# stevenlsw/reart

Hardware: AMD Instinct MI355X
Metric: relaxation-loop iterations/sec (higher is better)
Workload: dtype f32; 1 GPU; synthetic T=20 x N=4096, P=20, Chamfer+flow, full iteration, one instance/GPU; frames=20, points=4096, parts=20, flow=True, graph=True, steps_per_graph=20, graph_replays=1, eager_steps=0, parallelism=instances x1, instances_per_gpu=1

## Files before the change

include/reart_hip.h:

```cpp
#ifndef REART_HIP_H
#define REART_HIP_H

#include <stddef.h>
#include <stdint.h>

#ifdef __cplusplus
extern "C" {
#endif

typedef enum {
    REART_OK = 0,
    REART_ERR_INVALID_ARG = -1,
    REART_ERR_UNSUPPORTED = -2,
    REART_ERR_LAUNCH = -3,
    REART_ERR_NO_DEVICE = -4
} reart_status;

#define REART_MAX_K 16
#define REART_MAX_K_LIST 1024
#define REART_MAX_POSE_LEN 1024
#define REART_MAX_D 256

int reart_version(void);
int reart_device_count(void);
const char *reart_status_string(int status);


size_t reart_knn_points_workspace_bytes(int N, int P1, int P2, int K);
size_t reart_knn_points_workspace_bytes_d(int N, int P1, int P2, int D, int K);
int reart_knn_points_idx(const float *p1, const float *p2,
                         const int64_t *lengths1, const int64_t *lengths2,
                         int N, int P1, int P2, int D, int K,
                         float *dists, int64_t *idx,
                         void *workspace, size_t workspace_bytes, void *stream);

size_t reart_knn_points_workspace_bytes_f64(int N, int P1, int P2, int D, int K);
int reart_knn_points_idx_f64(const double *p1, const double *p2,
                             const int64_t *lengths1, const int64_t *lengths2,
                             int N, int P1, int P2, int D, int K,
                             double *dists, int64_t *idx,
                             void *workspace, size_t workspace_bytes, void *stream);

size_t reart_knn_points_backward_workspace_bytes(int N, int P1, int P2, int K);
int reart_knn_points_backward(const float *p1, const float *p2,
                              const int64_t *lengths1, const int64_t *lengths2,
                              const int64_t *idx, const float *grad_dists,
                              int N, int P1, int P2, int D, int K,
                              float *grad_p1, float *grad_p2,
                              void *workspace, size_t workspace_bytes, void *stream);

size_t reart_chamfer_bidir_workspace_bytes(int N, int P);
int reart_chamfer_bidir(const float *x, const float *y, int N, int P,
                        float *d_xy, int64_t *i_xy, float *d_yx, int64_t *i_yx,
                        void *workspace, size_t workspace_bytes, void *stream);

int reart_knn_cuda(const float *ref, const float *query, int B, int nr, int nq,
                   int D, int k, int euclidean, float *dist, int64_t *idx,
                   void *workspace, size_t workspace_bytes, void *stream);


size_t reart_blend_anchor_motion_workspace_bytes(int nq, int nr, int k);
int reart_blend_anchor_motion(const float *query, const float *ref, const float *ref_flow,
                              int nq, int nr, int k, int euclidean,
                              float *flow, uint8_t *mask,
                              void *workspace, size_t workspace_bytes, void *stream);

size_t reart_blend_anchor_motion_batch_workspace_bytes(int B, int nq, int nr_max, int k);
int reart_blend_anchor_motion_batch(const float *query, const float *ref, const float *ref_flow, const int64_t *ref_len,
                                    int B, int nq, int nr_max, int k, int euclidean, float *flow, uint8_t *mask,
                                    void *workspace, size_t workspace_bytes, void *stream);

size_t reart_kin_post_workspace_bytes(int B, int N, int nr_max, int k);
int reart_kin_post(const float *pc_trans, const float *cano, int B, int N, int cano_idx, const float *pc_src, const float *tgt,
                   const int32_t *cols, const int32_t *slot_of_point, int n, float lambda_assign, const float *ref,
                   const float *ref_flow, const int64_t *ref_len, int nr_max, int k, int euclidean, float lambda_flow, int robust,
                   float smooth_weight, float *G, float *matched, float *losses, void *workspace, size_t workspace_bytes,
                   void *stream);

size_t reart_flow_loss_workspace_bytes(void);
int reart_flow_loss(const float *gt, const float *pred, const uint8_t *mask, int B, int N,
                    int robust, float smooth_weight, float *loss, float *grad_pred,
                    void *workspace, size_t workspace_bytes, void *stream);


int reart_base_forward(const float *cano, int N, int P, int B,
                       const float *W1, const float *b1, const float *W2, int H,
                       const float *prop6d, const float *propt,
                       const float *gumbel, float tau,
                       float *out, int64_t *seg_part, float *trans_list,
                       float *yT, float *hT, int32_t *hard_idx, void *stream);

int reart_gumbel_noise(uint64_t seed, int64_t iter, int N, int P, float *out, void *stream);

size_t reart_base_backward_workspace_bytes(int N, int P, int B, int H);
int reart_base_path(int P, int B, int H, int backward);
int reart_base_backward(const float *cano, int N, int P, int B,
                        const float *W1, const float *b1, const float *W2, int H,
                        const float *prop6d, const float *propt,
                        const float *yT, const float *hT, const int32_t *hard_idx, float tau,
                        const float *G,
                        float *gW1, float *gb1, float *gW2, float *g6d, float *gt,
                        void *workspace, size_t workspace_bytes, void *stream);

int reart_compute_pc_transform(const float *cano, const float *pose, const int64_t *part,
                               int N, int P, int B, float *out, void *stream);

int reart_rotation_6d_to_matrix(const float *d6, int n, float *R, void *stream);

int reart_adam_step(float *param, const float *grad, float *exp_avg, float *exp_avg_sq,
                    int n, int step, float lr, float beta1, float beta2, float eps,
                    void *stream);

int reart_adam_step_multi(int count, float *const *param, const float *const *grad, float *const *exp_avg,
                          float *const *exp_avg_sq, const int *n, const float *lr, int step, float beta1, float beta2,
                          float eps, void *stream);


typedef struct reart_relax_config {
    int N, P, B, H;
    int cano_idx;
    int use_flow;
    int robust;
    int euclidean;
    int flow_k;
    int M_max;
    int M_total;
    int n_iter;
    int ring;
    float lambda_flow;
    float smooth_weight;
    float trans_lr, seg_lr;
    float beta1, beta2, eps;
    float start_tau, end_tau;
    float fixed_tau;
    uint64_t seed;
    int use_grid;
    int use_boxes;
    int use_assign;
    float lambda_assign;
    float weight_decay;
    int search_mode;
    int tune_slices;
    int tune_slices_flow;
    int tune_sparse;
    int tune_fwd_pts;
    int tune_bwd_pts;
    int tune_reorder;
    int tune_cloud;
    int tune_xcd;
    int profile;
    int tune_share;
    int tune_long;
} reart_relax_config;

typedef struct reart_relax_buffers {
    const float *cano;
    const float *pc_list;
    const float *ref_loc;
    const float *ref_flow;
    const int *ref_off;
    const float *gumbel;
    float *W1, *b1, *W2;
    float *p6d, *pt;
    float *adam_m, *adam_v;
    int64_t *iter;
    float *tau;
    float *losses;
    float *pc_trans;
    int64_t *seg_part;
    float *trans_list;
    void *aux_stream, *ev_fork, *ev_join;
    const int *assign_map;
} reart_relax_buffers;

size_t reart_relax_workspace_bytes(const reart_relax_config *cfg);
int reart_relax_prepare(const reart_relax_config *cfg, const reart_relax_buffers *bufs,
                        void *workspace, size_t workspace_bytes, void *stream);
int reart_relax_forward(const reart_relax_config *cfg, const reart_relax_buffers *bufs,
                        void *workspace, size_t workspace_bytes, void *stream);
int reart_relax_step(const reart_relax_config *cfg, const reart_relax_buffers *bufs,
                     void *workspace, size_t workspace_bytes, void *stream);
int reart_relax_step_batch(const reart_relax_config *cfgs, const reart_relax_buffers *bufs, void *const *workspaces,
                           size_t workspace_bytes, int K, void *stream);
#define REART_RELAX_PHASES 8
int reart_relax_step_timed(const reart_relax_config *cfg, const reart_relax_buffers *bufs,
                           void *workspace, size_t workspace_bytes, void *stream, float *h_ms);
int reart_relax_profile(const reart_relax_config *cfg, void *workspace, size_t workspace_bytes, void *stream,
                        double *h_out, int reset);


#define REART_FPS_MAX_N_LDS 12288
#define REART_FPS_MAX_N (1 << 21)
int reart_fps(const float *xyz, int B, int N, int npoint, const int32_t *start, int cuda_mode,
              int32_t *idx32, int64_t *idx64, void *stream);

int reart_fps_temp(const float *xyz, int B, int N, int npoint, const int32_t *start, int cuda_mode,
                   float *temp, int32_t *idx32, int64_t *idx64, void *stream);

int reart_ball_query(const float *xyz, const float *new_xyz, int B, int N, int S,
                     double radius, int nsample, int cuda_mode,
                     int32_t *idx32, int64_t *idx64, void *stream);

int reart_pn2_gather_points(const float *points, const int32_t *idx, int B, int C, int N, int M, float *out, void *stream);
int reart_pn2_gather_points_grad(const float *grad_out, const int32_t *idx, int B, int C, int N, int M, float *grad_points,
                                 void *stream);
int reart_pn2_three_interpolate(const float *points, const int32_t *idx, const float *weight, int B, int C, int M, int N,
                                float *out, void *stream);
int reart_pn2_three_interpolate_grad(const float *grad_out, const int32_t *idx, const float *weight, int B, int C, int N, int M,
                                     float *grad_points, void *stream);


int reart_fk_forward(const int32_t *parent, const int32_t *edge_of_part, const int32_t *order,
                     int P, const float *axis, const float *moment, const float *theta,
                     const float *distance, int B, int E, float *trans, void *stream);

size_t reart_fk_backward_workspace_bytes(int P, int B, int E);
int reart_fk_backward(const float *x, const int64_t *part, const float *G, int N,
                      const int32_t *parent, const int32_t *edge_of_part, const int32_t *order,
                      int P, const float *axis, const float *moment, const float *theta,
                      const float *distance, int B, int E, const float *trans,
                      float *g_axis, float *g_moment, float *g_theta, float *g_distance,
                      void *workspace, size_t workspace_bytes, void *stream);

#define REART_IK_MAX_POINTS 1024
int reart_ik_fit(const int32_t *parent, const int32_t *edge_of_part, const int32_t *order, int P,
                 const float *axis, const float *moment, int E, const float *src, const int64_t *part, int n,
                 const float *tgt, int M, const float *theta_init, int n_iter, float lr, float beta1, float beta2,
                 float eps, float *theta, float *loss, void *stream);


int reart_mlp_layer(const float *X, int ldx, const int64_t *gather_idx, int K, int S, int Npts,
                    const float *F, int D, const float *Q, const float *C, int xyz_first,
                    const float *Wt, const float *bias, int rows, int Cin, int Cout, int relu,
                    int pool_k, float *Y, int ldy, int ycol0, void *stream);

int reart_mlp_chain3(const int64_t *gather_idx, int K, int S, int Npts, const float *F, const float *Q, const float *C,
                     const float *W1t, const float *b1, int C1, const float *W2t, const float *b2, int C2,
                     const float *W3t, const float *b3, int C3, int rows, float *Y, int ldy, int ycol0, void *stream);

size_t reart_mlp_chain3_wide_workspace_bytes(int D, int C1, int C2, int C3);
int reart_mlp_chain3_wide(const int64_t *gather_idx, int K, int S, int Npts, const float *F, int D, const float *Q,
                          const float *C, const float *W1t, const float *b1, int C1, const float *W2t, const float *b2,
                          int C2, const float *W3t, const float *b3, int C3, int rows, float *Y, int ldy, int ycol0,
                          void *workspace, size_t workspace_bytes, void *stream);

int reart_mlp_chain_serves(int D, int K, int C1, int C2, int C3, int rows, int xyz_first);
size_t reart_mlp_chain_workspace_bytes(int D, int C1, int C2, int C3);
int reart_mlp_chain(const int64_t *gather_idx, int K, int S, int Npts, const float *F, int D, const float *Q, const float *C,
                    int xyz_first, const float *W1t, const float *b1, int C1, const float *W2t, const float *b2, int C2,
                    const float *W3t, const float *b3, int C3, int rows, float *Y, int ldy, int ycol0, void *workspace,
                    size_t workspace_bytes, void *stream);

int reart_square_distance(const float *src, const float *dst, int B, int N, int M, float *out, void *stream);

int reart_three_nn(const float *xyz1, const float *xyz2, int B, int N, int S2, float *dist3,
                   int64_t *idx3, void *stream);
size_t reart_three_interpolate_workspace_bytes(int B, int N, int S2);
int reart_three_interpolate(const float *xyz1, const float *xyz2, const float *points2, int B,
                            int N, int S2, int D, float *out, int ldo, int col0,
                            void *workspace, size_t workspace_bytes, void *stream);


size_t reart_grid_knn_workspace_bytes(int E, int Nt_max);
int reart_grid_knn(const float *targets, const int32_t *offsets, int E, int Nt_max,
                   const float *queries, int nq, int K, float *dists, int32_t *idx,
                   void *workspace, size_t workspace_bytes, void *stream);

size_t reart_knn_points_warm_workspace_bytes(int N, int P1, int P2, int K);
int reart_knn_points_idx_warm(const float *p1, const float *p2, int N, int P1, int P2, int K,
                              int32_t *seed, float *dists, int64_t *idx, void *workspace,
                              size_t workspace_bytes, void *stream);

size_t reart_chamfer_loss_workspace_bytes(int N, int P1, int P2);
int reart_chamfer_loss(const float *x, const float *y, int N, int P1, int P2, int32_t *seed_xy, int32_t *seed_yx,
                       int y_unchanged, float *d_xy, int64_t *i_xy, float *d_yx, int64_t *i_yx, float *loss,
                       float *grad_x, float *grad_y, int32_t *fx_bits, void *workspace, size_t workspace_bytes,
                       void *stream);

size_t reart_flow_term_workspace_bytes(int B, int N, int nr_max);
int reart_flow_term_prepare(const float *ref, const float *ref_flow, const int64_t *ref_len, int B, int nr_max, void *workspace,
                            size_t workspace_bytes, void *stream);
int reart_flow_term(const float *pc_trans, const float *cano, const int32_t *order, int B, int N, int cano_idx, int euclidean,
                    int robust, float smooth_weight, float weight, int32_t *seed, float *gt_flow, uint8_t *mask, float *dists,
                    int64_t *idx, float *loss, float *G, int accumulate, void *workspace, size_t workspace_bytes, void *stream);


size_t reart_lap_workspace_bytes(int B, int n);
int reart_lap_auction(const float *cost, int B, int n, int32_t *col4row, int32_t *certified,
                      const double *price_in, double *price_out, void *workspace, size_t workspace_bytes,
                      void *stream);

int reart_lap_auction_points(const float *cost, const float *src, const float *tgt, int B, int n, int32_t *col4row,
                             int32_t *certified, const double *price_in, double *price_out, void *workspace,
                             size_t workspace_bytes, void *stream);

size_t reart_lap_race_workspace_bytes(int B, int n, int racers);
int reart_lap_auction_race(const float *cost, const float *src, const float *tgt, int B, int n, int racers,
                           int32_t *col4row, int32_t *certified, double *price_out, void *workspace,
                           size_t workspace_bytes, void *stream);

int reart_lap_auction_race_warm(const float *cost, const float *src, const float *tgt, int B, int n, int racers,
                                const int32_t *col4row_in, const double *price_in, int32_t *col4row, int32_t *certified,
                                double *price_out, void *workspace, size_t workspace_bytes, void *stream);

#define REART_LAP_LARGE_MAX_N 8192
size_t reart_lap_large_workspace_bytes(int B, int n);
int reart_lap_auction_large(const float *cost, const float *src, const float *tgt, int B, int n,
                            int32_t *col4row, int32_t *certified, double *price_out,
                            void *workspace, size_t workspace_bytes, void *stream);

int reart_lap_auction_warm(const float *cost, int B, int n, int32_t *col4row, int32_t *certified,
                           const double *price_in, double *price_out, void *workspace, size_t workspace_bytes,
                           void *stream);

int reart_lap_resolve(const float *cost, int B, int n, int32_t *col4row, int32_t *certified,
                      const double *price_in, double *price_out, void *workspace, size_t workspace_bytes,
                      void *stream);

size_t reart_lap_resolve_large_workspace_bytes(int B, int n);
int reart_lap_resolve_large(const float *cost, int B, int n, int max_steps, int32_t *col4row, int32_t *certified,
                            const double *price_in, double *price_out, void *workspace, size_t workspace_bytes,
                            void *stream);

int reart_lap_step_floor(int B, int n, int steps, void *workspace, size_t workspace_bytes, double *h_us_per_step, void *stream);

int reart_relax_step_floor(const int *shape, int nk, int iters, void *workspace, size_t workspace_bytes, void *stream);

int reart_lap_resolve_points(const float *src, const float *tgt, int B, int n, int32_t *col4row,
                             int32_t *certified, const double *price_in, double *price_out, void *workspace,
                             size_t workspace_bytes, void *stream);
// ... 53 lines not shown
```

reart_amd/_lib.py:

```python
import ctypes
import os
import threading

import torch

_HERE = os.path.dirname(os.path.abspath(__file__))
LIB_PATH = os.environ.get("REART_LIB") or os.path.join(_HERE, "csrc", "libreart_hip.so")

c_int, c_float, c_size_t, c_void_p = ctypes.c_int, ctypes.c_float, ctypes.c_size_t, ctypes.c_void_p
P = c_void_p

MAX_K = 16
MAX_K_LIST = 1024
MAX_D = 256
MAX_POSE_LEN = 1024
IK_MAX_POINTS = 1024
LAP_LARGE_MAX_N = 8192
FPS_MAX_N_LDS = 12288
FPS_MAX_N = 1 << 21

PROTOTYPES = {
    "reart_version": (c_int, []),
    "reart_device_count": (c_int, []),
    "reart_status_string": (ctypes.c_char_p, [c_int]),
    "reart_knn_points_workspace_bytes": (c_size_t, [c_int] * 4),
    "reart_knn_points_workspace_bytes_d": (c_size_t, [c_int] * 5),
    "reart_knn_points_idx": (c_int, [P, P, P, P, c_int, c_int, c_int, c_int, c_int, P, P, P, c_size_t, P]),
    "reart_knn_points_workspace_bytes_f64": (c_size_t, [c_int] * 5),
    "reart_knn_points_idx_f64": (c_int, [P, P, P, P, c_int, c_int, c_int, c_int, c_int, P, P, P, c_size_t, P]),
    "reart_knn_points_backward_workspace_bytes": (c_size_t, [c_int] * 4),
    "reart_knn_points_backward": (c_int, [P, P, P, P, P, P, c_int, c_int, c_int, c_int, c_int, P, P, P, c_size_t, P]),
    "reart_chamfer_bidir_workspace_bytes": (c_size_t, [c_int] * 2),
    "reart_chamfer_bidir": (c_int, [P, P, c_int, c_int, P, P, P, P, P, c_size_t, P]),
    "reart_knn_cuda": (c_int, [P, P, c_int, c_int, c_int, c_int, c_int, c_int, P, P, P, c_size_t, P]),
    "reart_blend_anchor_motion_workspace_bytes": (c_size_t, [c_int] * 3),
    "reart_blend_anchor_motion": (c_int, [P, P, P, c_int, c_int, c_int, c_int, P, P, P, c_size_t, P]),
    "reart_kin_post_workspace_bytes": (c_size_t, [c_int] * 4),
    "reart_kin_post": (c_int, [P, P, c_int, c_int, c_int, P, P, P, P, c_int, c_float, P, P, P, c_int, c_int, c_int, c_float, c_int, c_float,
                               P, P, P, P, c_size_t, P]),
    "reart_blend_anchor_motion_batch_workspace_bytes": (c_size_t, [c_int] * 4),
    "reart_blend_anchor_motion_batch": (c_int, [P, P, P, P, c_int, c_int, c_int, c_int, c_int, P, P, P, c_size_t, P]),
    "reart_flow_loss_workspace_bytes": (c_size_t, []),
    "reart_flow_loss": (c_int, [P, P, P, c_int, c_int, c_int, c_float, P, P, P, c_size_t, P]),
    "reart_base_forward": (c_int, [P, c_int, c_int, c_int, P, P, P, c_int, P, P, P, c_float, P, P, P, P, P, P, P]),
    "reart_gumbel_noise": (c_int, [ctypes.c_uint64, ctypes.c_int64, c_int, c_int, P, P]),
    "reart_base_backward_workspace_bytes": (c_size_t, [c_int] * 4),
    "reart_base_path": (c_int, [c_int] * 4),
    "reart_base_backward": (c_int, [P, c_int, c_int, c_int, P, P, P, c_int, P, P, P, P, P, c_float, P,
                                    P, P, P, P, P, P, c_size_t, P]),
    "reart_compute_pc_transform": (c_int, [P, P, P, c_int, c_int, c_int, P, P]),
    "reart_rotation_6d_to_matrix": (c_int, [P, c_int, P, P]),
    "reart_adam_step": (c_int, [P, P, P, P, c_int, c_int, c_float, c_float, c_float, c_float, P]),
    "reart_adam_step_multi": (c_int, [c_int, P, P, P, P, P, P, c_int, c_float, c_float, c_float, P]),
    "reart_fps": (c_int, [P, c_int, c_int, c_int, P, c_int, P, P, P]),
    "reart_fps_temp": (c_int, [P, c_int, c_int, c_int, P, c_int, P, P, P, P]),
    "reart_ball_query": (c_int, [P, P, c_int, c_int, c_int, ctypes.c_double, c_int, c_int, P, P, P]),
    "reart_pn2_gather_points": (c_int, [P, P, c_int, c_int, c_int, c_int, P, P]),
    "reart_pn2_gather_points_grad": (c_int, [P, P, c_int, c_int, c_int, c_int, P, P]),
    "reart_pn2_three_interpolate": (c_int, [P, P, P, c_int, c_int, c_int, c_int, P, P]),
    "reart_pn2_three_interpolate_grad": (c_int, [P, P, P, c_int, c_int, c_int, c_int, P, P]),
    "reart_fk_forward": (c_int, [P, P, P, c_int, P, P, P, P, c_int, c_int, P, P]),
    "reart_fk_backward_workspace_bytes": (c_size_t, [c_int] * 3),
    "reart_fk_backward": (c_int, [P, P, P, c_int, P, P, P, c_int, P, P, P, P, c_int, c_int, P, P, P, P, P, P,
                                  c_size_t, P]),
    "reart_ik_fit": (c_int, [P, P, P, c_int, P, P, c_int, P, P, c_int, P, c_int, P, c_int, c_float, c_float, c_float, c_float, P, P, P]),
    "reart_mlp_layer": (c_int, [P, c_int, P, c_int, c_int, c_int, P, c_int, P, P, c_int, P, P, c_int, c_int, c_int,
                                c_int, c_int, P, c_int, c_int, P]),
    "reart_mlp_chain3": (c_int, [P, c_int, c_int, c_int, P, P, P, P, P, c_int, P, P, c_int, P, P, c_int, c_int, P, c_int, c_int, P]),
    "reart_mlp_chain3_wide_workspace_bytes": (c_size_t, [c_int] * 4),
    "reart_mlp_chain3_wide": (c_int, [P, c_int, c_int, c_int, P, c_int, P, P, P, P, c_int, P, P, c_int, P, P, c_int, c_int, P, c_int,
                                      c_int, P, c_size_t, P]),
    "reart_mlp_chain_serves": (c_int, [c_int] * 7),
    "reart_mlp_chain_workspace_bytes": (c_size_t, [c_int] * 4),
    "reart_mlp_chain": (c_int, [P, c_int, c_int, c_int, P, c_int, P, P, c_int, P, P, c_int, P, P, c_int, P, P, c_int, c_int, P, c_int,
                                c_int, P, c_size_t, P]),
    "reart_square_distance": (c_int, [P, P, c_int, c_int, c_int, P, P]),
    "reart_three_nn": (c_int, [P, P, c_int, c_int, c_int, P, P, P]),
    "reart_three_interpolate_workspace_bytes": (c_size_t, [c_int] * 3),
    "reart_three_interpolate": (c_int, [P, P, P, c_int, c_int, c_int, c_int, P, c_int, c_int, P, c_size_t, P]),
    "reart_grid_knn_workspace_bytes": (c_size_t, [c_int] * 2),
    "reart_grid_knn": (c_int, [P, P, c_int, c_int, P, c_int, c_int, P, P, P, c_size_t, P]),
    "reart_knn_points_warm_workspace_bytes": (c_size_t, [c_int] * 4),
    "reart_knn_points_idx_warm": (c_int, [P, P, c_int, c_int, c_int, c_int, P, P, P, P, c_size_t, P]),
    "reart_chamfer_loss_workspace_bytes": (c_size_t, [c_int] * 3),
    "reart_chamfer_loss": (c_int, [P, P, c_int, c_int, c_int, P, P, c_int, P, P, P, P, P, P, P, P, P, c_size_t, P]),
    "reart_flow_term_workspace_bytes": (c_size_t, [c_int] * 3),
    "reart_flow_term_prepare": (c_int, [P, P, P, c_int, c_int, P, c_size_t, P]),
    "reart_flow_term": (c_int, [P, P, P, c_int, c_int, c_int, c_int, c_int, c_float, c_float, P, P, P, P, P, P, P, c_int, P, c_size_t, P]),
    "reart_lap_workspace_bytes": (c_size_t, [c_int] * 2),
    "reart_lap_auction": (c_int, [P, c_int, c_int, P, P, P, P, P, c_size_t, P]),
    "reart_lap_auction_warm": (c_int, [P, c_int, c_int, P, P, P, P, P, c_size_t, P]),
    "reart_lap_auction_points": (c_int, [P, P, P, c_int, c_int, P, P, P, P, P, c_size_t, P]),
    "reart_lap_race_workspace_bytes": (c_size_t, [c_int] * 3),
    "reart_lap_auction_race": (c_int, [P, P, P, c_int, c_int, c_int, P, P, P, P, c_size_t, P]),
    "reart_lap_auction_race_warm": (c_int, [P, P, P, c_int, c_int, c_int, P, P, P, P, P, P, c_size_t, P]),
    "reart_lap_large_workspace_bytes": (c_size_t, [c_int] * 2),
    "reart_lap_auction_large": (c_int, [P, P, P, c_int, c_int, P, P, P, P, c_size_t, P]),
    "reart_lap_resolve": (c_int, [P, c_int, c_int, P, P, P, P, P, c_size_t, P]),
    "reart_lap_resolve_large_workspace_bytes": (c_size_t, [c_int] * 2),
    "reart_lap_resolve_large": (c_int, [P, c_int, c_int, c_int, P, P, P, P, P, c_size_t, P]),
    "reart_lap_resolve_points": (c_int, [P, P, c_int, c_int, P, P, P, P, P, c_size_t, P]),
    "reart_lap_resolve_points_race": (c_int, [P, P, c_int, c_int, c_int, P, P, P, P, P, c_size_t, P]),
    "reart_lap_resolve_points_mw": (c_int, [P, P, c_int, c_int, c_int, P, P, P, P, P, c_size_t, P]),
    "reart_lap_mc_workspace_bytes": (c_size_t, [c_int] * 3),
    "reart_lap_resolve_points_mc": (c_int, [P, P, c_int, c_int, c_int, c_int, P, P, P, P, P, c_size_t, P]),
    "reart_gather_points": (c_int, [P, P, c_int, c_int, c_int, P, P]),
    "reart_publish_words": (c_int, [P, c_int, P, c_int, P, c_int, P, P]),
    "reart_assign_pairs": (c_int, [P, P, P, c_int, c_int, c_int, P, P]),
    "reart_lap_ties": (c_int, [P, P, c_int, c_int, P, P, P, P, P, c_int, P]),
    "reart_lap_resolve_points_mc_ties": (c_int, [P, P, c_int, c_int, c_int, c_int, P, P, P, P, P, P, P, c_int, P, c_size_t, P]),
    "reart_lap_step_floor": (c_int, [c_int, c_int, c_int, P, c_size_t, ctypes.POINTER(ctypes.c_double), P]),
    "reart_relax_step_floor": (c_int, [ctypes.POINTER(c_int), c_int, c_int, P, c_size_t, P]),
    "reart_cdist": (c_int, [P, P, c_int, c_int, c_int, P, P]),
    "reart_match_smnn_workspace_bytes": (c_size_t, [c_int] * 3),
    "reart_match_smnn": (c_int, [P, P, c_int, c_int, c_int, c_int, c_float, P, P, P, c_size_t, P]),
    "reart_screw_fit_workspace_bytes": (c_size_t, [c_int] * 2),
    "reart_screw_fit": (c_int, [P, c_int, c_int, P, c_int, c_int, P, P, P, P, P, P, P, c_size_t, P]),
    "reart_part_fps": (c_int, [P, P, c_int, P, c_int, c_int, c_int, P, P, P]),
    "reart_part_pair_cost": (c_int, [P, P, c_int, c_int, c_int, P, P, P, P]),
    "reart_group_temporal_err": (c_int, [P, c_int, c_int, P, P, c_int, P, P, P]),
    "reart_relax_workspace_bytes": (c_size_t, None),
    "reart_relax_prepare": (c_int, None),
    "reart_relax_step": (c_int, None),
    "reart_relax_step_batch": (c_int, None),
    "reart_relax_forward": (c_int, None),
    "reart_relax_step_timed": (c_int, None),
    "reart_relax_profile": (c_int, None),
}

_lib = None
_lock = threading.Lock()


class ReartHipError(RuntimeError):
    """A libreart_hip.so entry point returned a negative reart_status."""


def lib():
    global _lib
    if _lib is None:
        with _lock:
            if _lib is None:
                if not os.path.exists(LIB_PATH):
                    raise ImportError(
                        f"{LIB_PATH} is missing: build it with `make -C reart_amd/csrc -j8` "
                        "(or `python -c 'import __graft_entry__ as g; g.build()'`). "
                        "reart_amd has no CPU / PyTorch fallback."
                    )
                handle = ctypes.CDLL(LIB_PATH)
                for name, (res, args) in PROTOTYPES.items():
                    fn = getattr(handle, name)
                    fn.restype = res
                    if args is not None:
                        fn.argtypes = args
                _lib = handle
    return _lib


def check(rc, what):
    if rc != 0:
        msg = lib().reart_status_string(rc).decode()
        raise ReartHipError(f"{what} failed: {msg} (status {rc})")


def require_gpu(*tensors):
    for t in tensors:
        if t is not None and not t.is_cuda:
            raise RuntimeError(
                "reart_amd operators run on an AMD GPU only (tensor is on "
                f"{t.device}); there is no CPU fallback."
            )


def ptr(t):
    return None if t is None else c_void_p(t.data_ptr())


def stream():
    return c_void_p(torch.cuda.current_stream().cuda_stream)


_ws_cache = {}


def workspace(nbytes, device):
    key = (device.index if device.index is not None else torch.cuda.current_device(),
           torch.cuda.current_stream(device).cuda_stream)
    buf = _ws_cache.get(key)
    if buf is None or buf.numel() < nbytes:
        buf = torch.empty(max(int(nbytes), 1 << 20), dtype=torch.uint8, device=device)
        _ws_cache[key] = buf
    return buf
```

reart_amd/csrc/internal.h:

```cpp
#pragma once
#include "common.h"

struct BaseFwdArgs {
    const float *cano;
    const float *W1, *b1, *W2, *p6d, *pt;
    const float *gumbel;
    const float *tau_ptr;
    const int64_t *iter_ptr;
    uint64_t seed;
    float tau;
    int N, P, B, H, Npad;
    float *out;
    float *out_soa;
    int64_t *seg_part;
    float *trans_list;
    float *yT;
    float *hT;
    int *hard_idx;
    float *rt_table;
    float *boxes;
    int pts;
};

struct BaseBwdArgs {
    const float *cano, *W2, *p6d, *pt;
    const float *yT, *hT;
    const int *hard_idx;
    const float *tau_ptr;
    float tau;
    const float *G;
    const float *rt_table;
    const float *gpf;
    int cano_idx;
    int N, P, B, H;
    int nchunk;
    int cpts;
    int dp_sep;
    float *partial;
    float *gW1, *gb1, *gW2, *g6d, *gt;
};

struct AdamSeg { float *p; const float *g; float *m; float *v; int n; float lr; };
struct AdamArgs { AdamSeg seg[8]; int nseg; float beta1, beta2, eps; const int64_t *step_ptr; int step; };

#define REART_BATCH_MAX 6
template <class A>
struct Batched { A a[REART_BATCH_MAX]; };
template <class A>
static inline Batched<A> reart_batched(const A *a, int K) {
    Batched<A> b = {};
    for (int k = 0; k < K && k < REART_BATCH_MAX; ++k) b.a[k] = a[k];
    return b;
}
int reart_base_forward_launch(const BaseFwdArgs *a, int K, hipStream_t st, int force_long);
struct FinalizeAdam {
    int enabled;
    float *W1, *b1, *W2, *p6d, *pt;
    float *m, *v;
    float seg_lr, trans_lr, beta1, beta2, eps;
    float weight_decay;
    const int64_t *step_ptr;
    const double *bias_corr;
};

struct StepBook {
    int enabled;
    const double *frame_loss; int n_frame_part;
    const double *flow_part; int n_flow_part;
    int64_t *iter; float *tau; float *losses; double *bias_corr;
    unsigned int *ticket;
    int ring, n_iter;
    float lambda_flow, fixed_tau, end_tau, start_tau, beta1, beta2;
};
int reart_base_backward_launch(const BaseBwdArgs *args, const FinalizeAdam *adam, const StepBook *book, void *const *workspaces,
                               size_t workspace_bytes, int K, hipStream_t st, int force_long);
int reart_base_forward_long_launch(const BaseFwdArgs *a, int K, hipStream_t st);
int reart_base_backward_long_launch(const BaseBwdArgs *a, int K, hipStream_t st);
int reart_base_bwd_long_tile(int P, int B, int H, int cpts, int *dp_sep, size_t *lds);
#ifdef __HIPCC__
__device__ __forceinline__ float reart_tau_schedule(long cur_iter, int n_iter, float end_t, float start_t) {
    const double c = cos(3.14159265358979323846 * (double)cur_iter / (double)n_iter);
    return (float)((double)end_t + ((double)start_t - (double)end_t) * (c + 1.0) * 0.5);
}
#endif
int reart_adam_ex(const AdamArgs &a, hipStream_t st);

int reart_knn_run(int njobs, const float *const *q, const float *const *t,
                  const int64_t *const *lenq, const int64_t *const *lent, int N, const int *P1,
                  const int *P2, int K, int euclidean, float *const *dists, int64_t *const *idx,
                  void *workspace, size_t workspace_bytes, hipStream_t st);

#define NN_BS 64
#define NN_UB 16
struct SoaJob {
    const float *src;
    const int64_t *len;
    float *dst;
    int P, Ppad;
};
struct SoaArgs {
    SoaJob job[2];
};

struct KnnJob {
    const float *q;
    const float *tsoa;
    const int64_t *lenq;
    const int64_t *lent;
    const float *q_alt;
    const int *qmap;
    const int *tlen;
    const float *boxes;
    const int *seed;
    const int *border;
    unsigned int *cost;
    int P1, P2, Ppad, L;
    int nqg;
    float *pd;
    int *pi;
    float *dists;
    int64_t *idx;
};
struct KnnArgs {
    KnnJob job[2];
    int N, S, K, euclidean;
    int items0;
    int items;
};

int reart_knn_launch_slices(const KnnArgs &a, int KK, hipStream_t st);
int reart_soa_launch(const SoaArgs &sa, int maxPpad, int N, int njobs, hipStream_t st);
int reart_knn_pick_split(long waves, int P2, int K);

size_t reart_knn_list_workspace_bytes(int N, int P1, int P2, int K);
int reart_knn_list_run(const float *q, const float *t, const int64_t *lenq, const int64_t *lent, int N, int P1,
                       int P2, int K, int euclidean, float *dists, int64_t *idx, void *workspace,
                       size_t workspace_bytes, hipStream_t st);
template <class T>
int reart_knn_anyd_run(const T *q, const T *t, const int64_t *lenq, const int64_t *lent, int N, int P1, int P2, int D,
                       int K, int euclidean, T *dists, int64_t *idx, void *workspace, size_t workspace_bytes,
                       hipStream_t st);
#ifndef NN_BOX
#define NN_BOX 16
#endif
int reart_boxes_launch(const float *soa, int N, int Ppad, float *boxes, hipStream_t st);
struct SearchArgs {
    KnnJob k1[2]; int n1;
    KnnJob k3;    int n3;
    int G;
    int per;
    int S1, S3;
    int sparse;
    int share;
    int interleave;
    int cloud_resident;
    int cloud_slices;
    int k_nqg;
    unsigned long long *prof;
    unsigned int *prof_pairs;
};
int reart_search_launch(const SearchArgs &a, hipStream_t st);
int reart_search_launch_batch(const SearchArgs *a, int K, hipStream_t st);
int reart_search_grid(int n1, int n3, int G);
int reart_search_grid_cloud(int n1, int n3, int G, int nqg, int slices);
int reart_search_workgroups(const SearchArgs &a);

#ifdef __HIPCC__
__device__ __forceinline__ void reart_top3_insert(float (&kd)[3], int (&ki)[3], float d, int j) {
    const bool l0 = (d < kd[0]) | ((d == kd[0]) & (j < ki[0]));
    const bool l1 = (d < kd[1]) | ((d == kd[1]) & (j < ki[1]));
    const bool l2 = (d < kd[2]) | ((d == kd[2]) & (j < ki[2]));
    kd[2] = l1 ? kd[1] : (l2 ? d : kd[2]);
    ki[2] = l1 ? ki[1] : (l2 ? j : ki[2]);
    kd[1] = l0 ? kd[0] : (l1 ? d : kd[1]);
    ki[1] = l0 ? ki[0] : (l1 ? j : ki[1]);
    kd[0] = l0 ? d : kd[0];
    ki[0] = l0 ? j : ki[0];
}
#endif

struct GridBuildArgs {
    const float *pts;
    const int *offsets;
    int N;
    int stride;
    float *gx, *gy, *gz;
    int *gorig;
    int *cell_start;
    float *meta;
    int *scratch;
};

struct GridQueryArgs {
    const float *q;
    const float *q_alt;
    const int *qmap;
    int nq, E, stride, euclid_unused;
    const float *gx, *gy, *gz;
    const int *gorig, *cell_start;
    const float *meta;
    float *od;
    int *oi;
};

size_t reart_grid_bytes(int E, int stride);
void reart_grid_layout(void *mem, int E, int stride, GridBuildArgs *b);
int reart_grid_build_launch(const GridBuildArgs &b, int E, hipStream_t st);
int reart_grid_query_launch(const GridQueryArgs &q, int K, hipStream_t st);
```

reart_amd/csrc/model.hip:

```cpp
#include "common.h"
#include "internal.h"
#include "model_dev.h"
#include <math.h>


#ifdef REART_PHASE_CLOCK
__device__ unsigned long long g_phase_ts[2][16];
extern "C" int reart_debug_phase_clock(unsigned long long *out) {
    return hipMemcpyFromSymbol(out, HIP_SYMBOL(g_phase_ts), sizeof(g_phase_ts)) == hipSuccess ? REART_OK : REART_ERR_LAUNCH;
}
#define PHASE_TS(which, k) do { if (blockIdx.x == 1 && threadIdx.x == 0) { g_phase_ts[which][k] = __builtin_amdgcn_s_memtime(); \
    g_phase_ts[which][(k) == 0 ? 12 : 13] = wall_clock64(); } } while (0)
#else
#define PHASE_TS(which, k) do { } while (0)
#endif
#ifdef REART_PHASE_CLOCK
#define PHASE_SYNC_TS(which, k) do { __syncthreads(); PHASE_TS(which, k); } while (0)
#else
#define PHASE_SYNC_TS(which, k) do { } while (0)
#endif


template <int PP, bool HALF, bool BATCH>
__global__ __launch_bounds__(64 * (HALF ? (((PP > 0 ? PP : 32) + 2 * FW_PG - 1) / (2 * FW_PG)) : (((PP > 0 ? PP : 32) + FW_PG - 1) / FW_PG)))
void base_fwd_kernel(Batched<BaseFwdArgs> ab) {
    const BaseFwdArgs &a = ab.a[BATCH ? blockIdx.y : 0];
    extern __shared__ __attribute__((aligned(16))) float smem[];
    constexpr int PMAX = (PP > 0) ? PP : 32;
    constexpr int W = HALF ? (PMAX + 2 * FW_PG - 1) / (2 * FW_PG) : (PMAX + FW_PG - 1) / FW_PG;
    constexpr int NS = HALF ? 2 * W : W;
    constexpr int PTS = HALF ? FW_PTS / 2 : FW_PTS;
    constexpr int BS = 64 * W;
    float *s_rt = smem;
    float *s_wb = s_rt + 12 * (size_t)a.B * a.P;
    float *s_w2T = s_wb + 4 * (size_t)a.H;
    float *s_a = s_w2T + (size_t)a.H * PMAX;
    float *s_e = s_a + PMAX * PTS;
    float *s_hh = s_e + PMAX * PTS;
    const int HS = a.H + 4;
    const int tid = threadIdx.x, lane = tid & 63, grp = tid >> 6;
    const int pl = HALF ? (lane & 31) : lane;
    const int sid = HALF ? 2 * grp + (lane >> 5) : grp;
    PHASE_TS(0, 0);
    const int P = (PP > 0) ? PP : a.P;
    const int nRT = a.B * a.P;
    auto put_rt = [&](int e, const float (&d6)[6], const float (&tv)[3]) {
        float R[9];
        r6d_to_matrix(d6, R);
#pragma unroll
        for (int c = 0; c < 9; ++c) s_rt[12 * e + c] = R[c];
#pragma unroll
        for (int c = 0; c < 3; ++c) s_rt[12 * e + 9 + c] = tv[c];
        if (blockIdx.x == 0) {
            if (a.trans_list) {
                float *T = a.trans_list + 16 * (size_t)e;
#pragma unroll
                for (int r = 0; r < 3; ++r) {
#pragma unroll
                    for (int c = 0; c < 3; ++c) T[4 * r + c] = R[3 * r + c];
                    T[4 * r + 3] = tv[r];
                }
                T[12] = 0.f; T[13] = 0.f; T[14] = 0.f; T[15] = 1.f;
            }
            if (a.rt_table) {
#pragma unroll
                for (int c = 0; c < 9; ++c) a.rt_table[12 * (size_t)e + c] = R[c];
#pragma unroll
                for (int c = 0; c < 3; ++c) a.rt_table[12 * (size_t)e + 9 + c] = tv[c];
            }
        }
    };
    {
        float d6[6], tv[3], vw[PMAX];
        const int e0 = tid < nRT ? tid : 0;
#pragma unroll
        for (int c = 0; c < 6; ++c) d6[c] = a.p6d[6 * (size_t)e0 + c];
#pragma unroll
        for (int c = 0; c < 3; ++c) tv[c] = a.pt[3 * (size_t)e0 + c];
        const int ew = tid < 4 * a.H ? tid : 0;
        const float wbv = (ew & 3) < 3 ? a.W1[3 * (ew >> 2) + (ew & 3)] : a.b1[ew >> 2];
        const int jw = tid < a.H ? tid : 0;
#pragma unroll
        for (int p = 0; p < PMAX; ++p) vw[p] = a.W2[(size_t)(p < P ? p : 0) * a.H + jw];
        if (tid < nRT) put_rt(tid, d6, tv);
        if (tid < 4 * a.H) s_wb[tid] = wbv;
        if (tid < a.H) {
#pragma unroll
            for (int p = 0; p < PMAX; ++p) s_w2T[((p >> 1) * a.H + tid) * 2 + (p & 1)] = p < P ? vw[p] : 0.f;
        }
    }
    for (int e = tid + BS; e < nRT; e += BS) {
        float d6[6], tv[3];
#pragma unroll
        for (int c = 0; c < 6; ++c) d6[c] = a.p6d[6 * (size_t)e + c];
#pragma unroll
        for (int c = 0; c < 3; ++c) tv[c] = a.pt[3 * (size_t)e + c];
        put_rt(e, d6, tv);
    }
    for (int e = tid + BS; e < 4 * a.H; e += BS) {
        const int j = e >> 2, c = e & 3;
        s_wb[e] = c < 3 ? a.W1[3 * j + c] : a.b1[j];
    }
    for (int j = tid + BS; j < a.H; j += BS)
        for (int p = 0; p < PMAX; ++p) s_w2T[((p >> 1) * a.H + j) * 2 + (p & 1)] = p < P ? a.W2[(size_t)p * a.H + j] : 0.f;

    const int n = blockIdx.x * PTS + pl;
    const bool live = n < a.N;
    const int nc = live ? n : a.N - 1;
    const float x0 = a.cano[3 * (size_t)nc], x1 = a.cano[3 * (size_t)nc + 1], x2 = a.cano[3 * (size_t)nc + 2];
    const int p0 = sid * FW_PG;
    const bool has1 = p0 + 1 < P;
    const float tau = a.tau_ptr ? a.tau_ptr[0] : a.tau;
    float g0, g1 = 0.f;
    if (a.gumbel) {
        g0 = a.gumbel[(size_t)nc * P + (p0 < P ? p0 : 0)];
        if (has1) g1 = a.gumbel[(size_t)nc * P + p0 + 1];
    } else {
        const uint64_t it = a.iter_ptr ? (uint64_t)a.iter_ptr[0] : 0ull;
        uint32_t r[4];
        philox4x32((uint32_t)n, (uint32_t)(p0 >> 2), (uint32_t)it, (uint32_t)(it >> 32), (uint32_t)a.seed,
                   (uint32_t)(a.seed >> 32), r);
        g0 = gumbel_from_bits(r[p0 & 3]);
        g1 = gumbel_from_bits(r[(p0 & 3) + 1]);
    }
    __syncthreads();
    PHASE_TS(0, 1);
    {
        const int jq = (a.H + NS - 1) / NS, j0 = sid * jq, j1 = (j0 + jq < a.H) ? j0 + jq : a.H;
        for (int j = j0; j < j1; ++j) {
            const float4 wb = *(const float4 *)(s_wb + 4 * j);
            float acc = wb.x * x0;
            acc = fmaf(wb.y, x1, acc);
            acc = fmaf(wb.z, x2, acc);
            acc = acc + wb.w;
            const float h = acc > 0.f ? acc : 0.f;
            s_hh[pl * HS + j] = h;
            if (a.hT && live) a.hT[(size_t)j * a.N + n] = h;
        }
    }
    __syncthreads();
    float sp0 = 0.f, sp1 = 0.f;
    {
        const float *hrow = s_hh + pl * HS, *wrow = s_w2T + (size_t)(sid < PMAX / 2 ? sid : PMAX / 2 - 1) * a.H * 2;
        int j = 0;
        const int H4 = (a.H & 3) == 0 ? a.H : 0;
#pragma unroll 2
        for (; j + 4 <= H4; j += 4) {
            const float4 h4 = *(const float4 *)(hrow + j);
            const float4 wa = *(const float4 *)(wrow + 2 * j), wb2 = *(const float4 *)(wrow + 2 * j + 4);
            sp0 = fmaf(wa.x, h4.x, sp0); sp1 = fmaf(wa.y, h4.x, sp1);
            sp0 = fmaf(wa.z, h4.y, sp0); sp1 = fmaf(wa.w, h4.y, sp1);
            sp0 = fmaf(wb2.x, h4.z, sp0); sp1 = fmaf(wb2.y, h4.z, sp1);
            sp0 = fmaf(wb2.z, h4.w, sp0); sp1 = fmaf(wb2.w, h4.w, sp1);
        }
        for (; j < a.H; ++j) {
            const float h = hrow[j];
            sp0 = fmaf(wrow[2 * j], h, sp0);
            sp1 = fmaf(wrow[2 * j + 1], h, sp1);
        }
    }
    PHASE_TS(0, 2);
    const float z0 = (sp0 + g0) / tau, z1 = has1 ? (sp1 + g1) / tau : -INFINITY;
    if (p0 < P) { s_a[p0 * PTS + pl] = sp0; s_e[p0 * PTS + pl] = z0; }
    if (has1) { s_a[(p0 + 1) * PTS + pl] = sp1; s_e[(p0 + 1) * PTS + pl] = z1; }
    __syncthreads();
    float m = -INFINITY;
    int am = 0;
    float sm = -INFINITY;
#pragma unroll
    for (int p = 0; p < PMAX; ++p)
        if (PP > 0 || p < P) {
            m = fmaxf(m, s_e[p * PTS + pl]);
            if (sid == 0) {
                const float sv = s_a[p * PTS + pl];
                if (sv > sm) { sm = sv; am = p; }
            }
        }
    __syncthreads();
    const float e0 = expf(z0 - m), e1 = has1 ? expf(z1 - m) : 0.f;
    if (p0 < P) s_e[p0 * PTS + pl] = e0;
    if (has1) s_e[(p0 + 1) * PTS + pl] = e1;
    __syncthreads();
    float sum = 0.f;
#pragma unroll
    for (int p = 0; p < PMAX; ++p)
        if (PP > 0 || p < P) sum += s_e[p * PTS + pl];
    const float y0 = e0 / sum, y1 = e1 / sum;
    if (p0 < P) { s_a[p0 * PTS + pl] = y0; if (a.yT && live) a.yT[(size_t)p0 * a.N + n] = y0; }
    if (has1) { s_a[(p0 + 1) * PTS + pl] = y1; if (a.yT && live) a.yT[(size_t)(p0 + 1) * a.N + n] = y1; }
    __syncthreads();
    PHASE_TS(0, 3);
    int k = 0;
    float yk = -1.f;
#pragma unroll
    for (int p = 0; p < PMAX; ++p)
        if (PP > 0 || p < P) {
            const float yv = s_a[p * PTS + pl];
            if (yv > yk) { yk = yv; k = p; }
        }
    const float w = (1.0f - yk) + yk;
    if (live && sid == 0) {
        if (a.seg_part) a.seg_part[n] = am;
        if (a.hard_idx) a.hard_idx[n] = k;
    }
    PHASE_TS(0, 4);
    for (int t = sid; t < a.B; t += NS) {
        float v[3];
        apply_rt(s_rt + 12 * (t * a.P + k), x0, x1, x2, v);
        v[0] = w * v[0]; v[1] = w * v[1]; v[2] = w * v[2];
        if (live) {
            float *o = a.out + 3 * ((size_t)t * a.N + n);
            o[0] = v[0]; o[1] = v[1]; o[2] = v[2];
        }
        if (a.out_soa && n < a.Npad) {
            float *o = a.out_soa + (size_t)t * 3 * a.Npad;
            o[n] = live ? v[0] : INFINITY;
            o[a.Npad + n] = live ? v[1] : INFINITY;
            o[2 * (size_t)a.Npad + n] = live ? v[2] : INFINITY;
        }
        if (a.boxes && blockIdx.x * PTS < a.Npad) {
            float lo[3], hi[3];
#pragma unroll
            for (int c = 0; c < 3; ++c) {
                static_assert(NN_BOX == 16, "a box is one DPP row");
                lo[c] = reart_row16_min(live ? v[c] : INFINITY);
                hi[c] = reart_row16_max(live ? v[c] : -INFINITY);
                if (hi[c] == -INFINITY) hi[c] = INFINITY;
            }
            const int pos = blockIdx.x * PTS + pl;
            if ((pl & (NN_BOX - 1)) == 0 && pos < a.Npad) {
                float *o = a.boxes + ((size_t)t * (a.Npad / NN_BOX) + pos / NN_BOX) * 8;
                o[0] = lo[0]; o[1] = lo[1]; o[2] = lo[2]; o[3] = hi[0]; o[4] = hi[1]; o[5] = hi[2];
            }
        }
    }
    PHASE_TS(0, 5);
}

template <int PP, bool HALF>
static void launch_base_fwd_t(const BaseFwdArgs *ak, int K, hipStream_t st) {
    const BaseFwdArgs &a = ak[0];
    constexpr int PMAX = (PP > 0) ? PP : 32;
    constexpr int W = HALF ? (PMAX + 2 * FW_PG - 1) / (2 * FW_PG) : (PMAX + FW_PG - 1) / FW_PG;
    constexpr int PTS = HALF ? FW_PTS / 2 : FW_PTS;
    const int cover = a.out_soa ? (a.Npad > a.N ? a.Npad : a.N) : a.N;
    const size_t lds = sizeof(float) * (12 * (size_t)a.B * a.P + (size_t)a.H * (4 + PMAX) + 2 * (size_t)PTS * PMAX +
                                        (size_t)(a.H + 4) * PTS);
    if (lds > REART_LDS_DEFAULT_CAP) {
        (void)hipFuncSetAttribute((const void *)base_fwd_kernel<PP, HALF, false>, hipFuncAttributeMaxDynamicSharedMemorySize, 152 * 1024);
        (void)hipFuncSetAttribute((const void *)base_fwd_kernel<PP, HALF, true>, hipFuncAttributeMaxDynamicSharedMemorySize, 152 * 1024);
    }
    if (K == 1) hipLaunchKernelGGL((base_fwd_kernel<PP, HALF, false>), dim3(reart_div_up(cover, PTS)), dim3(64 * W), lds, st, reart_batched(ak, 1));
    else hipLaunchKernelGGL((base_fwd_kernel<PP, HALF, true>), dim3(reart_div_up(cover, PTS), K), dim3(64 * W), lds, st, reart_batched(ak, K));
}
template <int PP>
static void launch_base_fwd(const BaseFwdArgs *a, int K, hipStream_t st) {
    if (a[0].pts == 64) launch_base_fwd_t<PP, false>(a, K, st);
    else launch_base_fwd_t<PP, true>(a, K, st);
}

static size_t base_fwd_lds_bound(int P, int B, int H) {
    return ((size_t)B * P * 12 + 2 * FW_PTS * 32 + (size_t)H * (36 + FW_PTS) + 4 * FW_PTS) * sizeof(float);
}
static size_t base_bwd_lds(int P, int B, int H) {
    const int PMAX = (P == 20 || P == 10 || P == 8) ? P : 32;
    return sizeof(float) * ((size_t)(H + PMAX) * BW_LD + RED_CHUNK * 5 + PMAX + 4 +
                            (size_t)B * RED_CHUNK * 3 + (size_t)H * PMAX + 12 * (size_t)B * P +
                            (size_t)PMAX * BW_LD);
}

extern "C" int reart_base_path(int P, int B, int H, int backward) {
    if (P < 1 || B < 1 || H < 1) return REART_ERR_INVALID_ARG;
    if (P > 32) return REART_ERR_UNSUPPORTED;
    if ((backward ? base_bwd_lds(P, B, H) : base_fwd_lds_bound(P, B, H)) <= REART_MODEL_LDS_CAP) return 0;
    if (B > REART_MAX_POSE_LEN) return REART_ERR_UNSUPPORTED;
    if (backward) return reart_base_bwd_long_tile(P, B, H, 0, nullptr, nullptr) >= 1 ? 1 : REART_ERR_UNSUPPORTED;
    return base_fwd_lds_bound(P, 0, H) <= REART_MODEL_LDS_CAP ? 1 : REART_ERR_UNSUPPORTED;
}

int reart_base_forward_launch(const BaseFwdArgs *ak, int K, hipStream_t st, int force_long) {
    if (K < 1 || K > REART_BATCH_MAX) return REART_ERR_INVALID_ARG;
    const BaseFwdArgs &a = ak[0];
    for (int k = 1; k < K; ++k)
        if (ak[k].N != a.N || ak[k].P != a.P || ak[k].B != a.B || ak[k].H != a.H || ak[k].Npad != a.Npad || ak[k].pts != a.pts ||
            !ak[k].out_soa != !a.out_soa)
            return REART_ERR_INVALID_ARG;
    if (a.P < 1 || a.P > 32) return REART_ERR_UNSUPPORTED;
    const int path = reart_base_path(a.P, a.B, a.H, 0);
    if (path < 0) return path;
    if (path == 1 || force_long) return reart_base_forward_long_launch(ak, K, st);
    switch (a.P) {
        case 20: launch_base_fwd<20>(ak, K, st); break;
        case 10: launch_base_fwd<10>(ak, K, st); break;
        case 8: launch_base_fwd<8>(ak, K, st); break;
        default: launch_base_fwd<0>(ak, K, st); break;
    }
    REART_CHECK_LAUNCH();
    return REART_OK;
}

extern "C" int reart_base_forward(const float *cano, int N, int P, int B, const float *W1,
                                  const float *b1, const float *W2, int H, const float *prop6d,
                                  const float *propt, const float *gumbel, float tau, float *out,
                                  int64_t *seg_part, float *trans_list, float *yT, float *hT,
                                  int32_t *hard_idx, void *stream) {
    if (N < 0 || P < 1 || B < 0 || H < 1) return REART_ERR_INVALID_ARG;
    if (N == 0 || B == 0) return REART_OK;
    if (!cano || !W1 || !b1 || !W2 || !prop6d || !propt || !gumbel || !out) return REART_ERR_INVALID_ARG;
    if (!(tau > 0.f)) return REART_ERR_INVALID_ARG;
    BaseFwdArgs a = {};
    a.cano = cano; a.W1 = W1; a.b1 = b1; a.W2 = W2; a.p6d = prop6d; a.pt = propt;
    a.gumbel = gumbel; a.tau = tau; a.N = N; a.P = P; a.B = B; a.H = H; a.Npad = 0;
    a.out = out; a.seg_part = seg_part; a.trans_list = trans_list; a.yT = yT; a.hT = hT;
    a.hard_idx = hard_idx;
    return reart_base_forward_launch(&a, 1, (hipStream_t)stream, 0);
}

__global__ __launch_bounds__(256) void gumbel_noise_kernel(uint64_t seed, uint64_t it, int N, int P, float *__restrict__ out) {
    const int Q = (P + 3) >> 2;
    const size_t e = (size_t)blockIdx.x * 256 + threadIdx.x;
    if (e >= (size_t)N * Q) return;
    const int n = (int)(e / Q), q = (int)(e % Q);
    uint32_t r[4];
    philox4x32((uint32_t)n, (uint32_t)q, (uint32_t)it, (uint32_t)(it >> 32), (uint32_t)seed, (uint32_t)(seed >> 32), r);
#pragma unroll
    for (int w = 0; w < 4; ++w)
        if (4 * q + w < P) out[(size_t)n * P + 4 * q + w] = gumbel_from_bits(r[w]);
}

extern "C" int reart_gumbel_noise(uint64_t seed, int64_t iter, int N, int P, float *out, void *stream) {
    if (N < 0 || P < 1 || iter < 0) return REART_ERR_INVALID_ARG;
    if (N == 0) return REART_OK;
    if (!out) return REART_ERR_INVALID_ARG;
    const size_t total = (size_t)N * ((P + 3) >> 2);
    gumbel_noise_kernel<<<(unsigned)((total + 255) / 256), 256, 0, (hipStream_t)stream>>>(seed, (uint64_t)iter, N, P, out);
    REART_CHECK_LAUNCH();
    return REART_OK;
}


__global__ __launch_bounds__(256) void rt_table_kernel(const float *__restrict__ p6d,
                                                       const float *__restrict__ pt, int n,
                                                       float *__restrict__ table) {
    const int e = blockIdx.x * 256 + threadIdx.x;
    if (e >= n) return;
    float R[9];
    r6d_to_matrix(p6d + 6 * (size_t)e, R);
#pragma unroll
    for (int c = 0; c < 9; ++c) table[12 * (size_t)e + c] = R[c];
#pragma unroll
    for (int c = 0; c < 3; ++c) table[12 * (size_t)e + 9 + c] = pt[3 * (size_t)e + c];
}

#ifdef REART_PHASE_CLOCK
#define PHASE_TS_WAVE(which, k, wave) do { if (blockIdx.x == 1 && (int)threadIdx.x == 64 * (wave)) g_phase_ts[which][k] = __builtin_amdgcn_s_memtime(); } while (0)
#else
#define PHASE_TS_WAVE(which, k, wave) do { } while (0)
#endif

template <int V> struct BwPiece { float v[V]; };
template <int V> __device__ __forceinline__ BwPiece<V> bw_load(const float *p) {
    BwPiece<V> r;
    if constexpr (V == 4) {
        const float4 q = *(const float4 *)p;
        r.v[0] = q.x; r.v[1] = q.y; r.v[2] = q.z; r.v[3] = q.w;
    } else {
        r.v[0] = *p;
    }
    return r;
}
template <int PP, int V, bool FAST, class LoadPoint>
__device__ __forceinline__ void bwd_stage_tiles(const BaseBwdArgs &a, int n0, int cn, float *s_h, float *s_G, float *s_w2T,
                                                float *s_rt, float *s_y, LoadPoint load_point) {
    typedef BwPiece<V> Pc;
    constexpr int PMAX = (PP > 0) ? PP : 32, BS = 64 * BW_WAVES;
    const int P = (PP > 0) ? PP : a.P;
    const int H = FAST ? 128 : a.H, B = FAST ? 19 : a.B, cw = FAST ? 32 : a.cpts;
    const int rsh = (cw == 64 ? 6 : (cw == 32 ? 5 : 4)) - (V == 4 ? 2 : 0);
    const int rp = 1 << rsh, gpc = 3 * rp;
    const int nH = H << rsh, nY = P << rsh, nG = B * gpc, nR = B * P * 12 / V, nW = P * (H / V);
    constexpr int UH = FAST ? 1 : 128 * RED_CHUNK / V / BS, UG = FAST ? 1 : (19 * RED_CHUNK * 3 / V + BS - 1) / BS,
                  UY = FAST ? 1 : (PMAX * RED_CHUNK / V + BS - 1) / BS, UR = (19 * 20 * 12 / V + BS - 1) / BS,
                  UW = FAST ? 1 : (PMAX * 128 / V + BS - 1) / BS;
    const int tid = threadIdx.x, tw = (tid + BS - 384) & (BS - 1), ty = BS - 1 - tid;
    const bool flow = a.gpf != nullptr;
    auto load_g = [&](int e, Pc &g, Pc &gh, Pc &gl) {
// ... 176 lines not shown
                    }
                }
#pragma unroll
                for (int u = 0; u < TU; ++u) {
                    const bool tok = t0 + u < a.B;
#pragma unroll
                    for (int r = 0; r < 3; ++r)
                        c = __builtin_amdgcn_mfma_f32_16x16x4f32(tok ? av[u][r] * xt : 0.f, (pok && tok) ? bv[u][r] : 0.f, c, 0, 0, 0);
                }
            }
#pragma unroll
            for (int reg = 0; reg < 4; ++reg)
                if (pok) s_ds[pc * BW_LD + 16 * mt + 4 * kq + reg] = c[reg];
        }
    }
    __syncthreads();
    PHASE_TS(1, 2);
    const int bl = lane < cn16 ? lane : 0;
    if (grp == 0) {
        const float yk = s_y[(kn < 0 ? 0 : kn) * BW_LD + bl];
        s_w[lane] = (1.0f - yk) + yk;
    }
    float ds0 = 0.f, ds1 = 0.f;
    if (has0) {
        const float dw0 = s_ds[p0 * BW_LD + bl];
        const float dw1 = has1 ? s_ds[(p0 + 1) * BW_LD + bl] : 0.f;
        const float tau = a.tau_ptr ? a.tau_ptr[0] : a.tau;
        float dot = 0.f;
#pragma unroll
        for (int p = 0; p < PMAX; ++p)
            if (PP > 0 || p < P) dot = fmaf(s_y[p * BW_LD + bl], s_ds[p * BW_LD + bl], dot);
        ds0 = (s_y[p0 * BW_LD + bl] * (dw0 - dot)) / tau;
        if (has1) ds1 = (s_y[(p0 + 1) * BW_LD + bl] * (dw1 - dot)) / tau;
    }
    __syncthreads();
    if (has0) s_ds[p0 * BW_LD + lane] = live ? ds0 : 0.f;
    if (has1) s_ds[(p0 + 1) * BW_LD + lane] = live ? ds1 : 0.f;
    __syncthreads();
    PHASE_TS(1, 3);
    const int n2 = (a.B * 12 + 31) >> 5, n1 = (a.H + 31) >> 5;
    if (grp < BW_MFMA) {
        typedef float f16v __attribute__((ext_vector_type(16)));
        for (int g = grp; g < n2 + n1; g += BW_MFMA) {
            f16v c = {0.f, 0.f, 0.f, 0.f, 0.f, 0.f, 0.f, 0.f, 0.f, 0.f, 0.f, 0.f, 0.f, 0.f, 0.f, 0.f};
            const int pr = lane & 31, kh = lane >> 5;
            if (g >= n2) {
                const int jc = (g - n2) * 32 + (lane & 31);
                const float *ap = s_ds + (pr < P ? pr : 0) * BW_LD + kh;
                const float *bp = s_h + (jc < a.H ? jc : 0) * BW_LD + kh;
                const bool aok = pr < P, bok = jc < a.H;
                for (int kb = 0; kb < cn16; kb += 16) {
#pragma unroll
                    for (int kk = kb; kk < kb + 16; kk += 2) {
                        const float av = aok ? ap[kk] : 0.f;
                        const float bv = bok ? bp[kk] : 0.f;
                        c = __builtin_amdgcn_mfma_f32_32x32x2f32(av, bv, c, 0, 0, 0);
                    }
                }
#pragma unroll
                for (int reg = 0; reg < 16; ++reg) {
                    const int prow_p = (reg & 3) + 8 * (reg >> 2) + 4 * kh;
                    if (prow_p < P && bok) prow[off_gW2() + prow_p * a.H + jc] = c[reg];
                }
                PHASE_TS_WAVE(1, 5, n2 % BW_MFMA);
            } else {
                const int col = g * 32 + (lane & 31);
                const bool cok = col < a.B * 12;
                const int t = cok ? col / 12 : 0, e = cok ? col - t * 12 : 0;
                const int gr = e < 9 ? e / 3 : e - 9, xc = e < 9 ? e - 3 * (e / 3) : 0;
                const float *gcol = s_G + t * (RED_CHUNK * 3) + gr;
                for (int kb = 0; kb < cn16; kb += 16) {
#pragma unroll
                    for (int kk = kb; kk < kb + 16; kk += 2) {
                        const int n = kk + kh;
                        const float av = (s_kn[n] == pr) ? 1.f : 0.f;
                        float bv = s_w[n] * gcol[3 * n];
                        if (e < 9) bv = bv * s_x[3 * n + xc];
                        c = __builtin_amdgcn_mfma_f32_32x32x2f32(av, cok ? bv : 0.f, c, 0, 0, 0);
                    }
                }
#pragma unroll
                for (int reg = 0; reg < 16; ++reg) {
                    const int prow_p = (reg & 3) + 8 * (reg >> 2) + 4 * kh;
                    if (prow_p < P && cok) prow[off_gRt(a.P, a.H) + (t * a.P + prow_p) * 12 + e] = c[reg];
                }
                PHASE_TS_WAVE(1, 4, 0);
            }
        }
    }
    if (!a.dp_sep) __syncthreads();
    if (grp >= BW_MFMA) {
        typedef float f16v __attribute__((ext_vector_type(16)));
        for (int jt = grp - BW_MFMA; jt < n1; jt += BW_HID) {
            const int j0 = 32 * jt, j1 = (j0 + 32 < a.H) ? j0 + 32 : a.H;
            const int jc = j0 + (lane & 31), kh = lane >> 5;
            const bool jok = jc < a.H;
            const float *bp = s_w2T + (jok ? jc : 0) * PMAX + kh;
            for (int nb = 0; nb < cn16; nb += 32) {
                f16v c = {0.f, 0.f, 0.f, 0.f, 0.f, 0.f, 0.f, 0.f, 0.f, 0.f, 0.f, 0.f, 0.f, 0.f, 0.f, 0.f};
                const float *ap = s_ds + kh * BW_LD + nb + (lane & 31);
#pragma unroll
                for (int p = 0; p < PMAX; p += 2) {
                    const bool pok = PP > 0 || p + kh < P;
                    const float av = pok ? ap[p * BW_LD] : 0.f;
                    const float bv = (pok && jok) ? bp[p] : 0.f;
                    c = __builtin_amdgcn_mfma_f32_32x32x2f32(av, bv, c, 0, 0, 0);
                }
#pragma unroll
                for (int reg = 0; reg < 16; ++reg) {
                    const int nn = nb + (reg & 3) + 8 * (reg >> 2) + 4 * kh;
                    if (jok && nn < a.cpts) {
                        const float h = s_h[jc * BW_LD + nn];
                        s_dp[jc * dp_ld + nn] = (nn < cn && h > 0.f) ? c[reg] : 0.f;
                    }
                }
            }
            __builtin_amdgcn_fence(__ATOMIC_ACQ_REL, "wavefront");
            __builtin_amdgcn_wave_barrier();
            PHASE_TS_WAVE(1, 6, BW_MFMA);
            {
                const int ob = 4 * j0 + lane;
                const bool ok0 = ob < 4 * j1, ok1 = ob + 64 < 4 * j1;
                const int ja = ok0 ? ob >> 2 : j0, jb = ok1 ? (ob + 64) >> 2 : ja, c = ob & 3, xo = c < 3 ? c : 0;
                float acc0 = 0.f, acc1 = 0.f;
                for (int ib = 0; ib < cn16; ib += 16) {
#pragma unroll
                    for (int i = ib; i < ib + 16; ++i) {
                        const float xs = s_x[3 * i + xo], xv = c < 3 ? xs : 1.0f;
                        acc0 = fmaf(s_dp[ja * dp_ld + i], xv, acc0);
                        acc1 = fmaf(s_dp[jb * dp_ld + i], xv, acc1);
                    }
                }
                if (c < 3) {
                    if (ok0) prow[off_gW1(a.P, a.H) + 3 * ja + c] = acc0;
                    if (ok1) prow[off_gW1(a.P, a.H) + 3 * jb + c] = acc1;
                } else {
                    if (ok0) prow[off_gb1(a.P, a.H) + ja] = acc0;
                    if (ok1) prow[off_gb1(a.P, a.H) + jb] = acc1;
                }
            }
            PHASE_TS_WAVE(1, 7, BW_MFMA);
        }
    }
    PHASE_SYNC_TS(1, 8);
}


struct AdamLoaded { float p, m, v; };
__device__ __forceinline__ AdamLoaded adam_load(const float *p, const float *m, const float *v) {
    AdamLoaded r;
    r.p = *p; r.m = *m; r.v = *v;
    return r;
}
__device__ __forceinline__ void adam_update(float *p, float g, float *m, float *v, const AdamLoaded &ld, float lr,
                                            float step_size_base, float bc2s, float beta1, float beta2,
                                            float eps, float weight_decay = 0.f) {
    (void)lr;
    if (weight_decay != 0.f) g = g + weight_decay * ld.p;
    float mm = ld.m, vv = ld.v;
    mm = mm + (g - mm) * (1.0f - beta1);
    vv = vv * beta2 + ((1.0f - beta2) * g) * g;
    const float denom = sqrtf(vv) / bc2s + eps;
    *m = mm; *v = vv;
    *p = ld.p - step_size_base * (mm / denom);
}

__device__ __forceinline__ void base_bwd_finalize_body(const BaseBwdArgs &a, const FinalizeAdam &ad) {
    const int og = blockIdx.x * 256 + threadIdx.x;
    const int nWr = a.P * a.H + 4 * a.H;
    const int nW = (4 * nWr + 63) & ~63;
    const int RQ = (a.nchunk + 3) >> 2;
    const int o = og >> 2;
    const int no = n_out(a.P, a.H, a.B);
    double bc1 = 1.0, bc2 = 1.0;
    if (ad.enabled) { bc1 = ad.bias_corr[0]; bc2 = ad.bias_corr[1]; }
    if (og < nW) {
        if (o >= nWr) return;
        const int nW2 = a.P * a.H, nW1 = 3 * a.H;
        const int kind = o < nW2 ? 0 : (o < nW2 + nW1 ? 1 : 2);
        const int q = kind == 0 ? o : (kind == 1 ? o - nW2 : o - nW2 - nW1);
        const int mo = kind == 0 ? nW1 + a.H + q : (kind == 1 ? q : nW1 + q);
        AdamLoaded ld = {0.f, 0.f, 0.f};
        if (ad.enabled) {
            if (kind == 0) ld.p = ad.W2[q];
            else if (kind == 1) ld.p = ad.W1[q];
            else ld.p = ad.b1[q];
            ld.m = ad.m[mo]; ld.v = ad.v[mo];
        }
        float acc = 0.f;
        int c = (og & 3) * RQ;
        const int cend = c + RQ < a.nchunk ? c + RQ : a.nchunk;
        for (; c + 32 <= cend; c += 32) {
            float v[32];
#pragma unroll
            for (int u = 0; u < 32; ++u) v[u] = a.partial[(size_t)(c + u) * no + o];
#pragma unroll
            for (int u = 0; u < 32; ++u) acc += v[u];
        }
        for (; c + 8 <= cend; c += 8) {
            float v[8];
#pragma unroll
            for (int u = 0; u < 8; ++u) v[u] = a.partial[(size_t)(c + u) * no + o];
#pragma unroll
            for (int u = 0; u < 8; ++u) acc += v[u];
        }
        for (; c < cend; ++c) acc += a.partial[(size_t)c * no + o];
        acc = acc + __shfl_xor(acc, 1, 64);
        acc = acc + __shfl_xor(acc, 2, 64);
        if (og & 3) return;
        const float ss_seg = (float)((double)ad.seg_lr / bc1), bc2s = (float)bc2;
        if (kind == 0) {
            a.gW2[q] = acc;
            if (ad.enabled) adam_update(ad.W2 + q, acc, ad.m + mo, ad.v + mo, ld, ad.seg_lr, ss_seg, bc2s, ad.beta1, ad.beta2, ad.eps, ad.weight_decay);
        } else if (kind == 1) {
            a.gW1[q] = acc;
            if (ad.enabled) adam_update(ad.W1 + q, acc, ad.m + mo, ad.v + mo, ld, ad.seg_lr, ss_seg, bc2s, ad.beta1, ad.beta2, ad.eps, ad.weight_decay);
        } else {
            a.gb1[q] = acc;
            if (ad.enabled) adam_update(ad.b1 + q, acc, ad.m + mo, ad.v + mo, ld, ad.seg_lr, ss_seg, bc2s, ad.beta1, ad.beta2, ad.eps, ad.weight_decay);
        }
    } else if (og < nW + 64 * a.B * a.P) {
        const int q = og - nW, e = q >> 6, tq = (q >> 4) & 3, c = q & 15;
        const int base6 = 3 * a.H + a.H + a.P * a.H, baset = base6 + 6 * a.B * a.P;
        const int k = c < 6 ? c : (c < 9 ? c - 6 : 2);
        const int mo = c < 6 ? base6 + 6 * e + k : baset + 3 * e + k;
        float *const pp = c < 6 ? ad.p6d + 6 * (size_t)e + k : ad.pt + 3 * (size_t)e + k;
        float d6[6];
#pragma unroll
        for (int u = 0; u < 6; ++u) d6[u] = a.p6d[6 * (size_t)e + u];
        AdamLoaded ld = {0.f, 0.f, 0.f};
        if (ad.enabled) ld = adam_load(pp, ad.m + mo, ad.v + mo);
        float acc = 0.f;
        if (c < 12) {
            const float *pr = a.partial + off_gRt(a.P, a.H) + 12 * (size_t)e + c;
            int ch = tq * RQ;
            const int chend = ch + RQ < a.nchunk ? ch + RQ : a.nchunk;
            for (; ch + 32 <= chend; ch += 32) {
                float v[32];
#pragma unroll
                for (int u = 0; u < 32; ++u) v[u] = pr[(size_t)(ch + u) * no];
#pragma unroll
                for (int u = 0; u < 32; ++u) acc += v[u];
            }
            for (; ch < chend; ++ch) acc += pr[(size_t)ch * no];
        }
        acc = acc + __shfl_xor(acc, 16, 64);
        acc = acc + __shfl_xor(acc, 32, 64);
        float gRt[12];
        const int lane0 = (threadIdx.x & 63) & ~15;
#pragma unroll
        for (int u = 0; u < 12; ++u) gRt[u] = __shfl(acc, lane0 + u, 64);
        if (c >= 9 || tq != 0) return;
        float g6[6];
        r6d_backward(d6, gRt, g6);
        const float ss_tr = (float)((double)ad.trans_lr / bc1), bc2s = (float)bc2;
        float g;
        if (c < 6) {
            g = g6[0];
#pragma unroll
            for (int u = 1; u < 6; ++u) g = (c == u) ? g6[u] : g;
            a.g6d[6 * (size_t)e + c] = g;
        } else {
            g = k == 0 ? gRt[9] : (k == 1 ? gRt[10] : gRt[11]);
            a.gt[3 * (size_t)e + k] = g;
        }
        if (ad.enabled) adam_update(pp, g, ad.m + mo, ad.v + mo, ld, ad.trans_lr, ss_tr, bc2s, ad.beta1, ad.beta2, ad.eps, ad.weight_decay);
    }
}

template <bool BATCH>
__global__ __launch_bounds__(384) void base_bwd_finalize_kernel(Batched<BaseBwdArgs> ab, Batched<FinalizeAdam> adb, Batched<StepBook> bkb) {
    const BaseBwdArgs &a = ab.a[BATCH ? blockIdx.y : 0];
    const FinalizeAdam &ad = adb.a[BATCH ? blockIdx.y : 0];
    const StepBook &bk = bkb.a[BATCH ? blockIdx.y : 0];
    __shared__ int s_last;
    __shared__ double s_book[4];
    __shared__ float s_tau;
    __shared__ long s_it;
    const int tid = threadIdx.x;
#ifdef REART_PHASE_CLOCK
    if (blockIdx.x == 1 && blockIdx.y == 0 && threadIdx.x == 0) { g_phase_ts[0][14] = __builtin_amdgcn_s_memtime(); g_phase_ts[0][8] = g_phase_ts[0][14]; }
#endif
    if (tid >= 320) {
        if (!bk.enabled) return;
        if (tid == 320) {
            const long it = (long)bk.iter[0];
            s_it = it;
            s_book[2] = 1.0 - pow((double)bk.beta1, (double)(it + 2));
            s_book[3] = sqrt(1.0 - pow((double)bk.beta2, (double)(it + 2)));
            s_tau = bk.fixed_tau > 0.f ? bk.fixed_tau : reart_tau_schedule(it + 2, bk.n_iter, bk.end_tau, bk.start_tau);
        }
    } else if (tid >= 256) {
        if (!bk.enabled) return;
        const int l = tid - 256;
        double recon = 0.0, flow = 0.0;
        for (int b = l; b < bk.n_frame_part; b += 64) recon += bk.frame_loss[b];
        for (int i = l; i < bk.n_flow_part; i += 64) flow += bk.flow_part[i];
        recon = reart_wave_sum_d(recon);
        flow = reart_wave_sum_d(flow);
        if (l == 0) { s_book[0] = recon; s_book[1] = flow * (double)bk.lambda_flow; }
    } else base_bwd_finalize_body(a, ad);
#ifdef REART_PHASE_CLOCK
    if (blockIdx.x == 1 && blockIdx.y == 0 && threadIdx.x == 0) g_phase_ts[0][9] = __builtin_amdgcn_s_memtime();
#endif
    if (!bk.enabled) return;
    __syncthreads();
    if (tid == 0) s_last = (atomicAdd(bk.ticket, 1u) == gridDim.x - 1) ? 1 : 0;
    __syncthreads();
#ifdef REART_PHASE_CLOCK
    if (blockIdx.x == 1 && blockIdx.y == 0 && threadIdx.x == 0) g_phase_ts[0][10] = __builtin_amdgcn_s_memtime();
#endif
    if (!s_last || tid != 0) return;
    const long it = s_it;
    if (bk.losses && bk.ring > 0) {
        float *row = bk.losses + 4 * (size_t)(it % bk.ring);
        row[0] = (float)s_book[0]; row[1] = (float)s_book[1]; row[2] = (float)(s_book[0] + s_book[1]); row[3] = bk.tau[0];
    }
    bk.iter[0] = it + 1;
    bk.bias_corr[0] = s_book[2];
    bk.bias_corr[1] = s_book[3];
    bk.tau[0] = s_tau;
    *bk.ticket = 0u;
}

static size_t base_bwd_ws_layout(int N, int P, int B, int H, size_t *o_rt, size_t *o_part) {
    const int nchunk = reart_div_up(N, 16);
    size_t off = 0;
    *o_rt = off; off += reart_align_up(sizeof(float) * 12 * (size_t)B * P, 256);
    *o_part = off; off += reart_align_up(sizeof(float) * (size_t)nchunk * n_out(P, H, B), 256);
    return off;
}

extern "C" size_t reart_base_backward_workspace_bytes(int N, int P, int B, int H) {
    if (N <= 0 || P <= 0 || B <= 0 || H <= 0) return 0;
    size_t a, b;
    return base_bwd_ws_layout(N, P, B, H, &a, &b);
}

template <int PP>
static int launch_bwd_block(const BaseBwdArgs *ak, int K, size_t lds, hipStream_t st) {
    if (lds > REART_LDS_DEFAULT_CAP &&
        (hipFuncSetAttribute((const void *)base_bwd_block_kernel<PP, false>, hipFuncAttributeMaxDynamicSharedMemorySize, 152 * 1024) != hipSuccess ||
         hipFuncSetAttribute((const void *)base_bwd_block_kernel<PP, true>, hipFuncAttributeMaxDynamicSharedMemorySize, 152 * 1024) != hipSuccess))
        return REART_ERR_LAUNCH;
    if (K == 1) hipLaunchKernelGGL((base_bwd_block_kernel<PP, false>), dim3(ak[0].nchunk), dim3(64 * BW_WAVES), lds, st, reart_batched(ak, 1));
    else hipLaunchKernelGGL((base_bwd_block_kernel<PP, true>), dim3(ak[0].nchunk, K), dim3(64 * BW_WAVES), lds, st, reart_batched(ak, K));
    return REART_OK;
}

int reart_base_backward_launch(const BaseBwdArgs *args, const FinalizeAdam *adam, const StepBook *book, void *const *workspaces,
                               size_t workspace_bytes, int K, hipStream_t st, int force_long) {
    if (K < 1 || K > REART_BATCH_MAX) return REART_ERR_INVALID_ARG;
    BaseBwdArgs ak[REART_BATCH_MAX];
    for (int k = 0; k < K; ++k) ak[k] = args[k];
    const BaseBwdArgs &a0 = ak[0];
    if (a0.P > 32) return REART_ERR_UNSUPPORTED;
    size_t o_rt, o_part;
    const size_t need = base_bwd_ws_layout(a0.N, a0.P, a0.B, a0.H, &o_rt, &o_part);
    if (!workspaces || workspace_bytes < need) return REART_ERR_INVALID_ARG;
    for (int k = 0; k < K; ++k) {
        BaseBwdArgs &a = ak[k];
        a.cpts = (a.cpts == 64 || a.cpts == 32 || a.cpts == 16) ? a.cpts : 32;
        a.nchunk = reart_div_up(a.N, a.cpts);
        if (a.N != a0.N || a.P != a0.P || a.B != a0.B || a.H != a0.H || a.cpts != a0.cpts || !workspaces[k]) return REART_ERR_INVALID_ARG;
        char *ws = (char *)workspaces[k];
        a.partial = (float *)(ws + o_part);
        if (!a.rt_table) {
            float *table = (float *)(ws + o_rt);
            hipLaunchKernelGGL(rt_table_kernel, dim3(reart_div_up(a.B * a.P, 256)), dim3(256), 0, st, a.p6d, a.pt,
                               a.B * a.P, table);
            a.rt_table = table;
        }
    }
    const int path = reart_base_path(a0.P, a0.B, a0.H, 1);
    if (path < 0) return path;
    int rc;
    if (path == 1 || force_long) rc = reart_base_backward_long_launch(ak, K, st);
    else {
        size_t lds = base_bwd_lds(a0.P, a0.B, a0.H);
        const size_t lds_dp = sizeof(float) * (size_t)a0.H * (a0.cpts + 1);
        const int dp_sep = lds + lds_dp <= 152 * 1024;
        if (dp_sep) lds += lds_dp;
        for (int k = 0; k < K; ++k) ak[k].dp_sep = dp_sep;
        switch (a0.P) {
            case 20: rc = launch_bwd_block<20>(ak, K, lds, st); break;
            case 10: rc = launch_bwd_block<10>(ak, K, lds, st); break;
            case 8: rc = launch_bwd_block<8>(ak, K, lds, st); break;
            default: rc = launch_bwd_block<0>(ak, K, lds, st); break;
        }
    }
    if (rc != REART_OK) return rc;
    Batched<FinalizeAdam> adb = {};
    Batched<StepBook> bkb = {};
    for (int k = 0; k < K; ++k) {
        if (adam) adb.a[k] = adam[k];
        if (book) bkb.a[k] = book[k];
    }
    const int nfin = (int)reart_align_up((size_t)4 * (a0.P * a0.H + 4 * a0.H), 64) + 64 * a0.B * a0.P;
    if (K == 1) hipLaunchKernelGGL(base_bwd_finalize_kernel<false>, dim3(reart_div_up(nfin, 256)), dim3(384), 0, st, reart_batched(ak, 1), adb, bkb);
    else hipLaunchKernelGGL(base_bwd_finalize_kernel<true>, dim3(reart_div_up(nfin, 256), K), dim3(384), 0, st, reart_batched(ak, K), adb, bkb);
    REART_CHECK_LAUNCH();
    return REART_OK;
}

extern "C" int reart_base_backward(const float *cano, int N, int P, int B, const float *W1,
                                   const float *b1, const float *W2, int H, const float *prop6d,
                                   const float *propt, const float *yT, const float *hT,
                                   const int32_t *hard_idx, float tau, const float *G, float *gW1,
                                   float *gb1, float *gW2, float *g6d, float *gt, void *workspace,
                                   size_t workspace_bytes, void *stream) {
    (void)W1; (void)b1;
    if (N <= 0 || P < 1 || B <= 0 || H < 1) return REART_ERR_INVALID_ARG;
    if (!cano || !W2 || !prop6d || !propt || !yT || !hT || !hard_idx || !G || !gW1 || !gb1 || !gW2 ||
        !g6d || !gt)
        return REART_ERR_INVALID_ARG;
    BaseBwdArgs a = {};
    a.cano = cano; a.W2 = W2; a.p6d = prop6d; a.pt = propt; a.yT = yT; a.hT = hT;
    a.hard_idx = hard_idx; a.tau = tau; a.G = G; a.N = N; a.P = P; a.B = B; a.H = H;
    a.gW1 = gW1; a.gb1 = gb1; a.gW2 = gW2; a.g6d = g6d; a.gt = gt;
    return reart_base_backward_launch(&a, nullptr, nullptr, &workspace, workspace_bytes, 1, (hipStream_t)stream, 0);
}

__global__ __launch_bounds__(256) void pc_transform_kernel(const float *__restrict__ cano,
                                                           const float *__restrict__ pose,
                                                           const int64_t *__restrict__ part, int N,
                                                           int P, int B, float *__restrict__ out) {
    const int n = blockIdx.x * 256 + threadIdx.x, t = blockIdx.y;
    if (n >= N) return;
    const float *T = pose + 16 * ((size_t)t * P + part[n]);
    const float x0 = cano[3 * (size_t)n], x1 = cano[3 * (size_t)n + 1], x2 = cano[3 * (size_t)n + 2];
    float *o = out + 3 * ((size_t)t * N + n);
#pragma unroll
    for (int c = 0; c < 3; ++c) {
        float acc = x0 * T[4 * c];
        acc = fmaf(x1, T[4 * c + 1], acc);
        acc = fmaf(x2, T[4 * c + 2], acc);
        o[c] = acc + T[4 * c + 3];
    }
}

extern "C" int reart_compute_pc_transform(const float *cano, const float *pose, const int64_t *part,
                                          int N, int P, int B, float *out, void *stream) {
    if (N < 0 || P < 1 || B < 0) return REART_ERR_INVALID_ARG;
    if (N == 0 || B == 0) return REART_OK;
    if (!cano || !pose || !part || !out) return REART_ERR_INVALID_ARG;
    hipLaunchKernelGGL(pc_transform_kernel, dim3(reart_div_up(N, 256), B), dim3(256), 0,
                       (hipStream_t)stream, cano, pose, part, N, P, B, out);
    REART_CHECK_LAUNCH();
    return REART_OK;
}

extern "C" int reart_rotation_6d_to_matrix(const float *d6, int n, float *R, void *stream);
__global__ __launch_bounds__(256) void r6d_kernel(const float *__restrict__ d6, int n, float *__restrict__ R) {
    const int i = blockIdx.x * 256 + threadIdx.x;
    if (i >= n) return;
    float r[9];
    r6d_to_matrix(d6 + 6 * (size_t)i, r);
#pragma unroll
    for (int c = 0; c < 9; ++c) R[9 * (size_t)i + c] = r[c];
}
extern "C" int reart_rotation_6d_to_matrix(const float *d6, int n, float *R, void *stream) {
    if (n < 0) return REART_ERR_INVALID_ARG;
    if (n == 0) return REART_OK;
    if (!d6 || !R) return REART_ERR_INVALID_ARG;
    hipLaunchKernelGGL(r6d_kernel, dim3(reart_div_up(n, 256)), dim3(256), 0, (hipStream_t)stream, d6, n, R);
    REART_CHECK_LAUNCH();
    return REART_OK;
}


__global__ __launch_bounds__(256) void adam_kernel(AdamArgs a) {
    const AdamSeg s = a.seg[blockIdx.y];
    const int i = blockIdx.x * 256 + threadIdx.x;
    if (i >= s.n) return;
// ... 51 lines not shown
```

reart_amd/csrc/step.hip:

```cpp
#include "common.h"
#include "internal.h"
#include "blocksort.h"
#include <math.h>
#include <string.h>

struct StepPlan {
    int S1, L1, Npad;
    int S3, Mpad;
    int nchunk, nparams;
    size_t o_ysoa, o_xsoa, o_rsoa, o_rlen, o_qmap;
    size_t o_pd0, o_pi0, o_pd1, o_pi1, o_pd3, o_pi3;
    size_t o_yT, o_hT, o_hard, o_rt, o_G, o_gpf, o_fx, o_floss, o_fpart, o_grads, o_bwd;
    size_t o_bc;
    size_t o_ticket;
    size_t o_boxY, o_boxX, o_boxR;
    int pruned;
    int W1, W3;
    int sparse;
    size_t o_seed3;
    size_t o_border;
    size_t o_cost;
    size_t o_prof, o_prof_pairs, o_prof_acc;
    size_t o_gridY, o_gridR;
    int gstrideY, gstrideR;
    size_t bwd_bytes, total;
};

static size_t take(size_t &off, size_t bytes) {
    const size_t o = off;
    off += reart_align_up(bytes, 256);
    return o;
}

#define FLOW_BS 256
#define CG_BS 1024
#define POST_FBS 512
#define CG_RANGE 1024
static_assert(CG_BS == CG_RANGE, "chamfer_grad_kernel: thread tid owns target r0 + tid");

static int step_plan(const reart_relax_config *c, StepPlan *p) {
    if (c->N <= 0 || c->P <= 0 || c->P > 32 || c->B <= 0 || c->H <= 0) return REART_ERR_INVALID_ARG;
    if (c->use_flow && (c->flow_k != 3 || c->M_max < 3)) return REART_ERR_UNSUPPORTED;
    const long waves1 = 2L * c->B * reart_div_up(c->N, NN_BS);
    p->pruned = (c->use_boxes && !c->use_grid && c->search_mode != 1) ? 1 : 0;
    p->W1 = (c->tune_slices >= 1 && c->tune_slices <= 4) ? c->tune_slices : 3;
    p->W3 = (c->tune_slices_flow >= 1 && c->tune_slices_flow <= 4) ? c->tune_slices_flow : p->W1;
    p->sparse = c->tune_sparse < 0 ? 0 : (c->tune_sparse == 0 ? 40 : (c->tune_sparse > 64 ? 64 : c->tune_sparse));
    p->S1 = p->pruned ? 1 : reart_knn_pick_split(waves1, c->N, 1);
    p->L1 = (int)reart_align_up((size_t)reart_div_up(c->N, p->S1), NN_BOX);
    p->Npad = p->L1 * p->S1;
    p->S3 = 1; p->Mpad = 0;
    if (c->use_flow) {
        const long waves3 = (long)c->B * reart_div_up(c->N, NN_BS);
        p->S3 = p->pruned ? 1 : reart_knn_pick_split(waves3, c->M_max, 3);
        p->Mpad = (int)reart_align_up((size_t)reart_div_up(c->M_max, p->S3), NN_BOX) * p->S3;
    }
    p->nchunk = reart_div_up(c->N, 64);
    p->nparams = 3 * c->H + c->H + c->P * c->H + 6 * c->B * c->P + 3 * c->B * c->P;
    size_t off = 0;
    const size_t BN = (size_t)c->B * c->N;
    p->o_ysoa = take(off, sizeof(float) * 3 * c->B * (size_t)p->Npad);
    p->o_xsoa = take(off, sizeof(float) * 3 * c->B * (size_t)p->Npad);
    p->o_rsoa = take(off, sizeof(float) * 3 * c->B * (size_t)p->Mpad);
    p->o_rlen = take(off, sizeof(int) * c->B);
    p->o_qmap = take(off, sizeof(int) * (c->B + 1));
    p->o_pd0 = take(off, sizeof(float) * p->S1 * BN);
    p->o_pi0 = take(off, sizeof(int) * p->S1 * BN);
    p->o_pd1 = take(off, sizeof(float) * p->S1 * BN);
    p->o_pi1 = take(off, sizeof(int) * p->S1 * BN);
    p->o_pd3 = take(off, c->use_flow ? sizeof(float) * p->S3 * BN * 3 : 0);
    p->o_pi3 = take(off, c->use_flow ? sizeof(int) * p->S3 * BN * 3 : 0);
    p->o_yT = take(off, sizeof(float) * (size_t)c->P * c->N);
    p->o_hT = take(off, sizeof(float) * (size_t)c->H * c->N);
    p->o_hard = take(off, sizeof(int) * (size_t)c->N);
    p->o_rt = take(off, sizeof(float) * 12 * (size_t)c->B * c->P);
    p->o_G = take(off, sizeof(float) * 3 * BN);
    p->o_gpf = take(off, sizeof(float) * 3 * BN);
    p->o_fx = take(off, sizeof(double));
    p->o_floss = take(off, sizeof(double) * (size_t)c->B * reart_div_up(c->N, CG_RANGE));
    p->o_fpart = take(off, sizeof(double) * (size_t)c->B * reart_div_up(c->N, FLOW_BS));
    p->o_grads = take(off, sizeof(float) * p->nparams);
    p->bwd_bytes = reart_base_backward_workspace_bytes(c->N, c->P, c->B, c->H);
    p->o_bwd = take(off, p->bwd_bytes);
    p->o_bc = take(off, 2 * sizeof(double));
    p->o_ticket = take(off, 4 * sizeof(unsigned int));
    p->o_boxY = take(off, sizeof(float) * 8 * (size_t)c->B * (p->Npad / NN_BOX));
    p->o_boxX = take(off, sizeof(float) * 8 * (size_t)c->B * (p->Npad / NN_BOX));
    p->o_boxR = take(off, sizeof(float) * 8 * (size_t)c->B * (p->Mpad / NN_BOX + 1));
    p->o_seed3 = take(off, (p->pruned && c->use_flow) ? sizeof(int) * BN * 3 : 0);
    const size_t G = (size_t)c->B * reart_div_up(c->N, NN_BS);
    p->o_border = take(off, sizeof(int) * 3 * G);
    p->o_cost = take(off, sizeof(unsigned int) * 3 * G);
    const size_t nprof = (c->profile && p->pruned) ? (size_t)reart_search_grid(2, 1, (int)G) : 0;
    p->o_prof = take(off, sizeof(unsigned long long) * 2 * nprof);
    p->o_prof_pairs = take(off, sizeof(unsigned int) * nprof);
    p->o_prof_acc = take(off, sizeof(unsigned long long) * 4);
    p->gstrideY = (int)reart_align_up((size_t)c->N, 64);
    p->gstrideR = (int)reart_align_up((size_t)(c->M_max > 0 ? c->M_max : 1), 64);
    p->o_gridY = take(off, c->use_grid ? reart_grid_bytes(c->B, p->gstrideY) : 0);
    p->o_gridR = take(off, (c->use_grid && c->use_flow) ? reart_grid_bytes(c->B, p->gstrideR) : 0);
    p->total = off;
    return REART_OK;
}

extern "C" size_t reart_relax_workspace_bytes(const reart_relax_config *cfg) {
    StepPlan p;
    if (!cfg || step_plan(cfg, &p) != REART_OK) return 0;
    return p.total;
}

__global__ void relax_init_kernel(reart_relax_config c, const int *__restrict__ ref_off,
                                  int *__restrict__ rlen, int *__restrict__ qmap,
                                  int64_t *__restrict__ iter, float *__restrict__ tau,
                                  const float *__restrict__ pc_list, int *__restrict__ fx_bits,
                                  double *__restrict__ bias_corr, int *__restrict__ seed3, int *__restrict__ border) {
    __shared__ float s_max[1024];
    const int t = threadIdx.x;
    if (seed3)
        for (size_t e = t; e < (size_t)c.B * c.N * 3; e += 1024) seed3[e] = (int)(e % 3);
    float mx = 0.f;
    for (size_t e = t; e < (size_t)c.B * c.N * 3; e += 1024) mx = fmaxf(mx, fabsf(pc_list[e]));
    s_max[t] = mx;
    __syncthreads();
    for (int o = 512; o >= 1; o >>= 1) {
        if (t < o) s_max[t] = fmaxf(s_max[t], s_max[t + o]);
        __syncthreads();
    }
    if (t == 0) {
        const double bound = 8.0 * (double)c.N * fmax((double)s_max[0], 1e-30);
        int bits = (int)floor(61.0 - log2(bound));
        fx_bits[0] = bits > 39 ? 39 : (bits < 0 ? 0 : bits);
    }
    if (t < c.B) {
        {
            const int nqg = (c.N + NN_BS - 1) / NN_BS, ng = c.B * nqg;
            for (int g = 0; g < nqg; ++g)
                for (int j = 0; j < 3; ++j) border[j * ng + t * nqg + g] = t * nqg + g;
        }
        qmap[t] = (t < c.cano_idx) ? t : (t == c.cano_idx ? -1 : t - 1);
        if (c.use_flow) rlen[t] = ref_off[t + 1] - ref_off[t];
    }
    if (t == 0) {
        const long it = (long)iter[0];
        tau[0] = c.fixed_tau > 0.f ? c.fixed_tau : reart_tau_schedule(it + 1, c.n_iter, c.end_tau, c.start_tau);
        bias_corr[0] = 1.0 - pow((double)c.beta1, (double)(it + 1));
        bias_corr[1] = sqrt(1.0 - pow((double)c.beta2, (double)(it + 1)));
    }
}

__global__ __launch_bounds__(256) void ref_soa_kernel(const float *__restrict__ ref_loc,
                                                      const int *__restrict__ ref_off, int Mpad,
                                                      float *__restrict__ soa) {
    const int f = blockIdx.y, j = blockIdx.x * 256 + threadIdx.x;
    if (j >= Mpad) return;
    const int o = ref_off[f], m = ref_off[f + 1] - o;
    float x = INFINITY, y = INFINITY, z = INFINITY;
    if (j < m) {
        const float *p = ref_loc + 3 * ((size_t)o + j);
        x = p[0]; y = p[1]; z = p[2];
    }
    float *d = soa + (size_t)f * 3 * Mpad;
    d[j] = x; d[Mpad + j] = y; d[2 * (size_t)Mpad + j] = z;
}

extern "C" int reart_relax_prepare(const reart_relax_config *cfg, const reart_relax_buffers *bufs,
                                   void *workspace, size_t workspace_bytes, void *stream) {
    StepPlan p;
    if (!cfg || !bufs) return REART_ERR_INVALID_ARG;
    int rc = step_plan(cfg, &p);
    if (rc != REART_OK) return rc;
    if (!workspace || workspace_bytes < p.total) return REART_ERR_INVALID_ARG;
    if (!bufs->cano || !bufs->pc_list || !bufs->iter || !bufs->tau) return REART_ERR_INVALID_ARG;
    if (cfg->use_flow && (!bufs->ref_loc || !bufs->ref_flow || !bufs->ref_off)) return REART_ERR_INVALID_ARG;
    static_assert(REART_MAX_POSE_LEN <= 1024, "relax_init_kernel: one thread per frame");
    if (cfg->B > REART_MAX_POSE_LEN) return REART_ERR_UNSUPPORTED;
    char *ws = (char *)workspace;
    hipStream_t st = (hipStream_t)stream;
    SoaArgs sa = {};
    for (int j = 0; j < 2; ++j) {
        sa.job[j].src = bufs->pc_list; sa.job[j].len = nullptr;
        sa.job[j].dst = (float *)(ws + p.o_ysoa); sa.job[j].P = cfg->N; sa.job[j].Ppad = p.Npad;
    }
    rc = reart_soa_launch(sa, p.Npad, cfg->B, 1, st);
    if (rc != REART_OK) return rc;
    hipLaunchKernelGGL(relax_init_kernel, dim3(1), dim3(1024), 0, st, *cfg, bufs->ref_off,
                       (int *)(ws + p.o_rlen), (int *)(ws + p.o_qmap), bufs->iter, bufs->tau, bufs->pc_list,
                       (int *)(ws + p.o_fx), (double *)(ws + p.o_bc),
                       (p.pruned && cfg->use_flow) ? (int *)(ws + p.o_seed3) : nullptr, (int *)(ws + p.o_border));
    if (hipMemsetAsync(ws + p.o_ticket, 0, 4 * sizeof(unsigned int), st) != hipSuccess) return REART_ERR_LAUNCH;
    if (hipMemsetAsync(ws + p.o_prof_acc, 0, 4 * sizeof(unsigned long long), st) != hipSuccess) return REART_ERR_LAUNCH;
    if (p.pruned) {
        if (hipMemsetAsync(ws + p.o_pi0, 0, sizeof(int) * (size_t)cfg->B * cfg->N, st) != hipSuccess) return REART_ERR_LAUNCH;
        if (hipMemsetAsync(ws + p.o_pi1, 0, sizeof(int) * (size_t)cfg->B * cfg->N, st) != hipSuccess) return REART_ERR_LAUNCH;
    }
    rc = reart_boxes_launch((const float *)(ws + p.o_ysoa), cfg->B, p.Npad, (float *)(ws + p.o_boxY), st);
    if (rc != REART_OK) return rc;
    if (cfg->use_grid) {
        GridBuildArgs gb = {};
        reart_grid_layout(ws + p.o_gridY, cfg->B, p.gstrideY, &gb);
        gb.pts = bufs->pc_list; gb.offsets = nullptr; gb.N = cfg->N;
        rc = reart_grid_build_launch(gb, cfg->B, st);
        if (rc != REART_OK) return rc;
        if (cfg->use_flow) {
            GridBuildArgs gr = {};
            reart_grid_layout(ws + p.o_gridR, cfg->B, p.gstrideR, &gr);
            gr.pts = bufs->ref_loc; gr.offsets = bufs->ref_off; gr.N = cfg->M_max;
            rc = reart_grid_build_launch(gr, cfg->B, st);
            if (rc != REART_OK) return rc;
        }
    }
    if (cfg->use_flow)
    {
        hipLaunchKernelGGL(ref_soa_kernel, dim3(reart_div_up(p.Mpad, 256), cfg->B), dim3(256), 0, st,
                           bufs->ref_loc, bufs->ref_off, p.Mpad, (float *)(ws + p.o_rsoa));
        rc = reart_boxes_launch((const float *)(ws + p.o_rsoa), cfg->B, p.Mpad, (float *)(ws + p.o_boxR), st);
        if (rc != REART_OK) return rc;
    }
    REART_CHECK_LAUNCH();
    return REART_OK;
}

struct FlowArgs {
    const float *pd; const int *pi;
    const float *ref_flow; const int *ref_off; const int *qmap;
    const float *X; const float *cano;
    int N, B, S, euclidean, robust, cano_idx;
    int blocks;
    const float *rsoa; int Mpad;
    float smooth, lambda;
    float *gpf;
    double *part;
    int *seed_out;
};

__device__ __forceinline__ const float *complete_frame(const FlowArgs &a, int f) {
    return f < a.cano_idx ? a.X + (size_t)f * a.N * 3
                          : (f == a.cano_idx ? a.cano : a.X + (size_t)(f - 1) * a.N * 3);
}

__device__ __forceinline__ float huber1s(float x) {
    const float ax = fabsf(x);
    return ax <= 1.0f ? 0.5f * x * x : (ax - 0.5f);
}
__device__ __forceinline__ float huber1s_grad(float x) {
    return fabsf(x) <= 1.0f ? x : (x > 0.f ? 1.0f : -1.0f);
}

template <int SL, int FBS>
__device__ __forceinline__ void flow_blend_body(const FlowArgs &a, const int bx, const int f, const int nbx) {
    __shared__ double s_red[FBS / REART_WAVE];
    const int n = bx * FBS + threadIdx.x;
    double term = 0.0;
    if (n < a.N) {
        constexpr int NU = SL == 1 ? 1 : 4;
        float kd[3] = {INFINITY, INFINITY, INFINITY};
        int ki[3] = {0x7fffffff, 0x7fffffff, 0x7fffffff};
        const size_t stride = (size_t)a.B * a.N * 3, o0 = ((size_t)f * a.N + n) * 3;
        const float *c0 = complete_frame(a, f) + 3 * (size_t)n;
        const float *c1 = complete_frame(a, f + 1) + 3 * (size_t)n;
        const float c0v[3] = {c0[0], c0[1], c0[2]}, c1v[3] = {c1[0], c1[1], c1[2]};
        const int roff = a.ref_off[f];
        for (int s0 = 0; s0 < (SL ? 1 : a.S); s0 += 4) {
            float e[NU][3];
            int q[NU][3];
#pragma unroll
            for (int u = 0; u < NU; ++u) {
                const bool ok = s0 + u < a.S;
                const size_t o = o0 + (size_t)(ok ? s0 + u : 0) * stride;
#pragma unroll
                for (int k = 0; k < 3; ++k) { e[u][k] = a.pd[o + k]; q[u][k] = a.pi[o + k]; }
                if (!ok) { e[u][0] = INFINITY; e[u][1] = INFINITY; e[u][2] = INFINITY; }
            }
#pragma unroll
            for (int u = 0; u < NU; ++u)
#pragma unroll
                for (int k = 0; k < 3; ++k)
                    reart_top3_insert(kd, ki, e[u][k], e[u][k] < INFINITY ? q[u][k] : 0x7fffffff);
        }
        if (a.blocks) {
            const float qx = c0v[0], qy = c0v[1], qz = c0v[2];
            const float *tx = a.rsoa + (size_t)f * 3 * a.Mpad, *ty = tx + a.Mpad, *tz = ty + a.Mpad;
            int bb[3];
            float4 X[3][2], Y[3][2], Z[3][2];
#pragma unroll
            for (int cb = 0; cb < 3; ++cb) {
                bb[cb] = (kd[cb] < INFINITY) ? ki[cb] : -1;
                const int blk = bb[cb] < 0 ? 0 : bb[cb];
#pragma unroll
                for (int h = 0; h < 2; ++h) {
                    X[cb][h] = *(const float4 *)(tx + blk + 4 * h);
                    Y[cb][h] = *(const float4 *)(ty + blk + 4 * h);
                    Z[cb][h] = *(const float4 *)(tz + blk + 4 * h);
                }
            }
            __builtin_amdgcn_sched_barrier(0);
#pragma unroll
            for (int k = 0; k < 3; ++k) { kd[k] = INFINITY; ki[k] = 0x7fffffff; }
#pragma unroll
            for (int cb = 0; cb < 3; ++cb) {
#pragma unroll
                for (int u = 0; u < 8; ++u) {
                    const float4 vx = X[cb][u >> 2], vy = Y[cb][u >> 2], vz = Z[cb][u >> 2];
                    const int c = u & 3;
                    const float px = c == 0 ? vx.x : (c == 1 ? vx.y : (c == 2 ? vx.z : vx.w));
                    const float py = c == 0 ? vy.x : (c == 1 ? vy.y : (c == 2 ? vy.z : vy.w));
                    const float pz = c == 0 ? vz.x : (c == 1 ? vz.y : (c == 2 ? vz.z : vz.w));
                    float d = reart_sqdist3(qx, qy, qz, px, py, pz);
                    if (bb[cb] < 0) d = INFINITY;
                    reart_top3_insert(kd, ki, d, d < INFINITY ? bb[cb] + u : 0x7fffffff);
                }
            }
        }
#pragma unroll
        for (int k = 0; k < 3; ++k) ki[k] = ki[k] == 0x7fffffff ? 0 : ki[k];
        if (a.seed_out) {
            int *so = a.seed_out + 3 * ((size_t)f * a.N + n);
            so[0] = ki[0]; so[1] = ki[1]; so[2] = ki[2];
        }
        const float *rf = a.ref_flow + 3 * (size_t)roff;
        float rfl[3][3];
#pragma unroll
        for (int k = 0; k < 3; ++k)
#pragma unroll
            for (int c = 0; c < 3; ++c) rfl[k][c] = rf[3 * (size_t)ki[k] + c];
        float w[3], wsum = 0.f, dmin = INFINITY, fmx = -INFINITY;
#pragma unroll
        for (int k = 0; k < 3; ++k) {
            float d = a.euclidean ? sqrtf(kd[k]) : kd[k];
            if (d < 1e-10f) d = 1e-10f;
            w[k] = 1.0f / d;
            wsum += w[k];
            dmin = fminf(dmin, d);
            fmx = fmaxf(fmx, (rfl[k][0] * rfl[k][0] + rfl[k][1] * rfl[k][1]) + rfl[k][2] * rfl[k][2]);
        }
        float gtf[3] = {0.f, 0.f, 0.f};
#pragma unroll
        for (int k = 0; k < 3; ++k) {
            const float wn = w[k] / wsum;
            gtf[0] += rfl[k][0] * wn; gtf[1] += rfl[k][1] * wn; gtf[2] += rfl[k][2] * wn;
        }
        const bool m = (dmin <= fmx) || (dmin <= 0.05f);
        float fl = 0.f, sm = 0.f;
// ... 190 lines not shown
}
__device__ __forceinline__ void prof_body(const OrderArgs &o) {
    __shared__ unsigned long long s_lo[CG_BS / 64], s_hi[CG_BS / 64], s_sum[CG_BS / 64], s_busy[CG_BS / 64];
    const int tid = threadIdx.x;
    unsigned long long lo = ~0ull, hi = 0ull, sum = 0ull, busy = 0ull;
    for (int k = tid; k < o.nprof; k += CG_BS) {
        const unsigned long long a = o.prof[2 * (size_t)k], b = o.prof[2 * (size_t)k + 1];
        lo = a < lo ? a : lo; hi = b > hi ? b : hi; sum += o.prof_pairs[k]; busy += b - a;
    }
#pragma unroll
    for (int off = 32; off >= 1; off >>= 1) {
        const unsigned long long l2 = __shfl_xor(lo, off, 64), h2 = __shfl_xor(hi, off, 64), s2 = __shfl_xor(sum, off, 64);
        const unsigned long long b2 = __shfl_xor(busy, off, 64);
        lo = l2 < lo ? l2 : lo; hi = h2 > hi ? h2 : hi; sum += s2; busy += b2;
    }
    if ((tid & 63) == 0) { s_lo[tid >> 6] = lo; s_hi[tid >> 6] = hi; s_sum[tid >> 6] = sum; s_busy[tid >> 6] = busy; }
    __syncthreads();
    if (tid == 0) {
        for (int w = 1; w < CG_BS / 64; ++w) {
            lo = s_lo[w] < lo ? s_lo[w] : lo; hi = s_hi[w] > hi ? s_hi[w] : hi; sum += s_sum[w]; busy += s_busy[w];
        }
        o.prof_acc[0] += 1ull; o.prof_acc[1] += hi - lo; o.prof_acc[2] += sum; o.prof_acc[3] += busy;
    }
}
struct PostArgs { int nfx, nflow, ncx, nwork, norder; FlowArgs fl; CGradArgs cg; OrderArgs od; };
#ifdef REART_PHASE_CLOCK
__device__ unsigned long long g_post_ts[8];
extern "C" int reart_debug_post_clock(unsigned long long *out) {
    return hipMemcpyFromSymbol(out, HIP_SYMBOL(g_post_ts), sizeof(g_post_ts)) == hipSuccess ? REART_OK : REART_ERR_LAUNCH;
}
#define POST_TS(k) do { __syncthreads(); if (threadIdx.x == 0 && blockIdx.y == 0) g_post_ts[k] = __builtin_amdgcn_s_memtime(); } while (0)
#else
#define POST_TS(k) do { } while (0)
#endif
template <bool BATCH>
__global__ __launch_bounds__(CG_BS) void post_kernel(Batched<PostArgs> ab) {
    const PostArgs &a = ab.a[BATCH ? blockIdx.y : 0];
    const int w = blockIdx.x;
    if (w < a.nflow) {
        if (threadIdx.x >= POST_FBS) return;
        if (w == 1) POST_TS(0);
        flow_blend_body<1, POST_FBS>(a.fl, w % a.nfx, w / a.nfx, a.nfx);
        if (w == 1) POST_TS(1);
    } else if (w < a.nwork) {
        if (w == a.nflow + 1) POST_TS(2);
        chamfer_grad_body<1>(a.cg, (w - a.nflow) % a.ncx, (w - a.nflow) / a.ncx, a.ncx);
        if (w == a.nflow + 1) POST_TS(3);
    } else if (w < a.nwork + a.norder) {
        if (w == a.nwork) POST_TS(4);
        order_body(a.od, w - a.nwork);
        if (w == a.nwork) POST_TS(5);
    } else {
        POST_TS(6);
        prof_body(a.od);
        POST_TS(7);
    }
}

struct AssignArgs {
    const float *X, *Y;
    const int *map;
    int N, B;
    float lambda;
    float *G;
    double *loss_part;
};
__device__ __forceinline__ void assign_grad_body(const AssignArgs &a, int bx, int b, int gx) {
    __shared__ double s_red[CG_BS / REART_WAVE];
    const int i = bx * CG_BS + threadIdx.x, tid = threadIdx.x;
    double term = 0.0;
    if (i < a.N) {
        const size_t o = (size_t)b * a.N + i;
        const int m = a.map[o];
        float g[3] = {0.f, 0.f, 0.f};
        if (m >= 0 && m < a.N) {
            float sq = 0.f;
#pragma unroll
            for (int k = 0; k < 3; ++k) {
                const float d = a.X[3 * o + k] - a.Y[3 * ((size_t)b * a.N + m) + k];
                sq += d * d;
                g[k] = a.lambda * (2.0f * d);
            }
            term = (double)sq;
        }
#pragma unroll
        for (int k = 0; k < 3; ++k) a.G[3 * o + k] = g[k];
    }
    term = reart_wave_sum_d(term);
    if ((tid & 63) == 0) s_red[tid >> 6] = term;
    __syncthreads();
    if (tid == 0) {
        double t = 0.0;
        for (int w = 0; w < CG_BS / REART_WAVE; ++w) t += s_red[w];
        a.loss_part[(size_t)b * gx + bx] = t * (double)a.lambda;
    }
}
template <bool BATCH>
__global__ __launch_bounds__(CG_BS) void assign_grad_kernel(Batched<AssignArgs> ab) {
    assign_grad_body(ab.a[BATCH ? blockIdx.z : 0], blockIdx.x, blockIdx.y, gridDim.x);
}

#define MARK(k) do { if (ev) (void)hipEventRecord(ev[k], st); } while (0)

struct StepGeom {
    int pruned, grid;
    int flow;
    int merged;
    int has_search;
    int static_order;
    int has_fl, has_aa, has_cg;
    int fl_sl, cg_sl;
    int fgx, fgy, ncg, post_blocks, N, B;
    int long_model;
};
struct StepLaunch {
    StepGeom g;
    BaseFwdArgs fa; SearchArgs sa; KnnArgs ka, k3; GridQueryArgs gq3, gq1; PostArgs pa;
    FlowArgs fl; AssignArgs aa; CGradArgs cg;
    BaseBwdArgs ba; FinalizeAdam ad; StepBook bk; void *ws_bwd; size_t bwd_bytes;
    int auto_s1, auto_s3;
    void *aux_stream, *ev_fork, *ev_join;
};

static int step_describe(const reart_relax_config *cfg, const reart_relax_buffers *bufs, void *workspace, size_t workspace_bytes,
                         bool forward_only, StepLaunch *out) {
    StepPlan p;
    if (!cfg || !bufs) return REART_ERR_INVALID_ARG;
    int rc = step_plan(cfg, &p);
    if (rc != REART_OK) return rc;
    if (!workspace || workspace_bytes < p.total) return REART_ERR_INVALID_ARG;
    if (!bufs->W1 || !bufs->b1 || !bufs->W2 || !bufs->p6d || !bufs->pt || !bufs->adam_m || !bufs->adam_v ||
        !bufs->pc_trans || !bufs->iter || !bufs->tau)
        return REART_ERR_INVALID_ARG;
    const reart_relax_config &c = *cfg;
    StepLaunch &L = *out;
    L = StepLaunch{};
    StepGeom &g = L.g;
    char *ws = (char *)workspace;
    const int N = c.N, B = c.B, P = c.P, H = c.H;
    float *G = (float *)(ws + p.o_G);
    g.N = N; g.B = B; g.pruned = p.pruned; g.grid = c.use_grid ? 1 : 0; g.flow = c.use_flow ? 1 : 0;
    g.long_model = c.tune_long > 0 ? 1 : 0;

    BaseFwdArgs &fa = L.fa;
    fa.cano = bufs->cano; fa.W1 = bufs->W1; fa.b1 = bufs->b1; fa.W2 = bufs->W2; fa.p6d = bufs->p6d;
    fa.pt = bufs->pt; fa.gumbel = bufs->gumbel; fa.tau_ptr = bufs->tau; fa.iter_ptr = bufs->iter;
    fa.seed = c.seed; fa.tau = 1.0f; fa.N = N; fa.P = P; fa.B = B; fa.H = H; fa.Npad = p.Npad;
    fa.out = bufs->pc_trans; fa.out_soa = (float *)(ws + p.o_xsoa); fa.seg_part = bufs->seg_part;
    fa.trans_list = bufs->trans_list; fa.yT = (float *)(ws + p.o_yT); fa.hT = (float *)(ws + p.o_hT);
    fa.hard_idx = (int *)(ws + p.o_hard);
    fa.rt_table = (float *)(ws + p.o_rt);
    fa.boxes = c.use_boxes ? (float *)(ws + p.o_boxX) : nullptr;
    fa.pts = c.tune_fwd_pts;
    if (forward_only) return REART_OK;
    if (c.use_assign && !bufs->assign_map) return REART_ERR_INVALID_ARG;

    const int nqg = reart_div_up(N, NN_BS);
    const int *qmap = (const int *)(ws + p.o_qmap);
    KnnArgs &ka = L.ka, &k3 = L.k3;
    ka.N = B; ka.S = p.S1; ka.K = 1; ka.euclidean = 0;
    for (int j = 0; j < 2; ++j) {
        KnnJob &kj = ka.job[j];
        kj.q = j == 0 ? bufs->pc_trans : bufs->pc_list;
        kj.tsoa = (const float *)(ws + (j == 0 ? p.o_ysoa : p.o_xsoa));
        kj.P1 = N; kj.P2 = N; kj.Ppad = p.Npad; kj.L = p.L1; kj.nqg = nqg;
        kj.pd = (float *)(ws + (j == 0 ? p.o_pd0 : p.o_pd1));
        kj.pi = (int *)(ws + (j == 0 ? p.o_pi0 : p.o_pi1));
        kj.boxes = c.use_boxes ? (const float *)(ws + (j == 0 ? p.o_boxY : p.o_boxX)) : nullptr;
        kj.seed = p.pruned ? kj.pi : nullptr;
        kj.border = (const int *)(ws + p.o_border) + (size_t)j * B * nqg;
        kj.cost = p.pruned ? (unsigned int *)(ws + p.o_cost) + (size_t)j * B * nqg : nullptr;
    }
    ka.items0 = B * nqg * p.S1; ka.items = 2 * ka.items0;
    if (c.use_flow) {
        k3.N = B; k3.S = p.S3; k3.K = 3; k3.euclidean = 0;
        KnnJob &kj = k3.job[0];
        kj.q = bufs->pc_trans; kj.q_alt = bufs->cano; kj.qmap = qmap;
        kj.tsoa = (const float *)(ws + p.o_rsoa); kj.tlen = (const int *)(ws + p.o_rlen);
        kj.boxes = c.use_boxes ? (const float *)(ws + p.o_boxR) : nullptr;
        kj.P1 = N; kj.P2 = c.M_max; kj.Ppad = p.Mpad; kj.L = p.Mpad / p.S3; kj.nqg = nqg;
        kj.pd = (float *)(ws + p.o_pd3); kj.pi = (int *)(ws + p.o_pi3);
        kj.seed = p.pruned ? (const int *)(ws + p.o_seed3) : nullptr;
        kj.border = (const int *)(ws + p.o_border) + 2 * (size_t)B * nqg;
        kj.cost = p.pruned ? (unsigned int *)(ws + p.o_cost) + 2 * (size_t)B * nqg : nullptr;
        k3.job[1] = kj;
        k3.items0 = B * nqg * p.S3; k3.items = k3.items0;
    }
    const bool chamfer = !c.use_assign;
    const bool merged = p.pruned && c.use_flow && chamfer;
    g.merged = merged ? 1 : 0;
    L.aux_stream = bufs->aux_stream; L.ev_fork = bufs->ev_fork; L.ev_join = bufs->ev_join;

    int search_wgs = 0, S3 = p.S3, S0 = p.S1;
    if (p.pruned) {
        SearchArgs &sa = L.sa;
        sa.G = B * nqg; sa.S1 = p.W1; sa.S3 = p.W3; sa.sparse = p.sparse; sa.share = c.tune_share < 0 ? 0 : (c.tune_share == 1 ? 1 : 2); sa.interleave = c.tune_xcd > 0 ? 0 : 1;
        sa.cloud_resident = c.tune_cloud > 0 ? 1 : 0; sa.cloud_slices = c.tune_cloud > 0 ? c.tune_cloud : 0;
        if (chamfer) { sa.k1[0] = ka.job[0]; sa.k1[1] = ka.job[1]; sa.n1 = 2; }
        if (c.use_flow) { sa.k3 = k3.job[0]; sa.n3 = 1; }
        if (c.profile && merged) {
            sa.prof = (unsigned long long *)(ws + p.o_prof); sa.prof_pairs = (unsigned int *)(ws + p.o_prof_pairs);
        }
        L.auto_s1 = c.tune_slices == 0; L.auto_s3 = c.tune_slices_flow == 0;
        if (sa.n1 + sa.n3 > 0) {
            search_wgs = reart_search_workgroups(sa);
            g.static_order = search_wgs != reart_search_grid(sa.n1, sa.n3, sa.G);
            g.has_search = 1;
        }
    } else if (c.use_grid) {
        if (c.use_flow) {
            GridBuildArgs gr = {};
            reart_grid_layout(ws + p.o_gridR, B, p.gstrideR, &gr);
            GridQueryArgs &gq = L.gq3;
            gq.q = bufs->pc_trans; gq.q_alt = bufs->cano; gq.qmap = qmap; gq.nq = N; gq.E = B; gq.stride = p.gstrideR;
            gq.gx = gr.gx; gq.gy = gr.gy; gq.gz = gr.gz; gq.gorig = gr.gorig; gq.cell_start = gr.cell_start;
            gq.meta = gr.meta; gq.od = (float *)(ws + p.o_pd3); gq.oi = (int *)(ws + p.o_pi3);
            S3 = 1;
        }
        if (chamfer) {
            GridBuildArgs gy = {};
            reart_grid_layout(ws + p.o_gridY, B, p.gstrideY, &gy);
            GridQueryArgs &gq = L.gq1;
            gq.q = bufs->pc_trans; gq.nq = N; gq.E = B; gq.stride = p.gstrideY; gq.gx = gy.gx; gq.gy = gy.gy; gq.gz = gy.gz;
            gq.gorig = gy.gorig; gq.cell_start = gy.cell_start; gq.meta = gy.meta;
            gq.od = (float *)(ws + p.o_pd0); gq.oi = (int *)(ws + p.o_pi0);
            S0 = 1;
            ka.job[0] = ka.job[1];
            ka.items = ka.items0;
        }
    }
    int nfp = 0;
    FlowArgs &fl = L.fl;
    if (c.use_flow) {
        fl.pd = (const float *)(ws + p.o_pd3); fl.pi = (const int *)(ws + p.o_pi3); fl.ref_flow = bufs->ref_flow;
        fl.ref_off = bufs->ref_off; fl.qmap = qmap; fl.X = bufs->pc_trans; fl.cano = bufs->cano; fl.N = N; fl.B = B;
        fl.blocks = c.use_grid ? 0 : 1; fl.rsoa = (const float *)(ws + p.o_rsoa); fl.Mpad = p.Mpad;
        fl.S = S3; fl.euclidean = c.euclidean; fl.robust = c.robust; fl.cano_idx = c.cano_idx;
        fl.smooth = c.smooth_weight; fl.lambda = c.lambda_flow;
        fl.gpf = (float *)(ws + p.o_gpf); fl.part = (double *)(ws + p.o_fpart);
        fl.seed_out = p.pruned ? (int *)(ws + p.o_seed3) : nullptr;
        g.fgx = reart_div_up(N, merged ? POST_FBS : FLOW_BS); g.fgy = B;
        nfp = g.fgx * g.fgy;
        g.has_fl = merged ? 0 : 1; g.fl_sl = fl.S == 1 ? 1 : (fl.S <= 4 ? 4 : 0);
    }
    g.ncg = reart_div_up(N, CG_RANGE);
    if (c.use_assign) {
        AssignArgs &aa = L.aa;
        aa.X = bufs->pc_trans; aa.Y = bufs->pc_list; aa.map = bufs->assign_map; aa.N = N; aa.B = B;
        aa.lambda = c.lambda_assign; aa.G = G; aa.loss_part = (double *)(ws + p.o_floss);
        g.has_aa = 1;
    } else {
        CGradArgs &cg = L.cg;
        cg.X = bufs->pc_trans; cg.Y = bufs->pc_list;
        cg.pd0 = (const float *)(ws + p.o_pd0); cg.pi0 = (const int *)(ws + p.o_pi0);
        cg.pd1 = (const float *)(ws + p.o_pd1); cg.pi1 = (const int *)(ws + p.o_pi1);
        cg.fx_bits = (const int *)(ws + p.o_fx);
        cg.N = N; cg.B = B; cg.S0 = S0; cg.S1 = p.S1; cg.G = G;
        cg.loss_part = (double *)(ws + p.o_floss);
        g.has_cg = merged ? 0 : 1; g.cg_sl = (cg.S0 == 1 && cg.S1 == 1) ? 1 : ((cg.S0 <= 4 && cg.S1 <= 4) ? 4 : 0);
        if (merged) {
            PostArgs &pa = L.pa;
            pa.fl = fl; pa.cg = cg; pa.nfx = g.fgx; pa.nflow = pa.nfx * B; pa.ncx = g.ncg;
            pa.nwork = pa.nflow + g.ncg * B;
            const bool reorder = c.tune_reorder >= 0 && !g.static_order;
            for (int j = 0; j < 3; ++j) {
                const KnnJob &kj = j < 2 ? ka.job[j] : k3.job[0];
                pa.od.cost[j] = reorder ? kj.cost : nullptr;
                pa.od.border[j] = (int *)(ws + p.o_border) + (size_t)j * B * nqg;
            }
            pa.od.groups = B * nqg; pa.od.per = c.tune_xcd > 0 ? reart_div_up(B * nqg, 8) : B * nqg;
            pa.norder = reorder ? 3 : 0;
            g.post_blocks = pa.nwork + pa.norder;
            if (c.profile) {
                pa.od.prof = (const unsigned long long *)(ws + p.o_prof);
                pa.od.prof_pairs = (const unsigned int *)(ws + p.o_prof_pairs);
                pa.od.prof_acc = (unsigned long long *)(ws + p.o_prof_acc);
                pa.od.nprof = search_wgs;
                g.post_blocks += 1;
            }
        }
    }
    float *grads = (float *)(ws + p.o_grads);
    float *gW1 = grads, *gb1 = gW1 + 3 * H, *gW2 = gb1 + H, *g6d = gW2 + P * H, *gt = g6d + 6 * B * P;
    BaseBwdArgs &ba = L.ba;
    ba.cano = bufs->cano; ba.W2 = bufs->W2; ba.p6d = bufs->p6d; ba.pt = bufs->pt; ba.yT = fa.yT; ba.hT = fa.hT;
    ba.hard_idx = fa.hard_idx; ba.tau_ptr = bufs->tau; ba.tau = 1.0f; ba.G = G; ba.rt_table = fa.rt_table;
    ba.cano_idx = c.cano_idx;
    ba.gpf = c.use_flow ? (const float *)(ws + p.o_gpf) : nullptr;
    ba.cpts = c.tune_bwd_pts;
    ba.N = N; ba.P = P; ba.B = B; ba.H = H; ba.gW1 = gW1; ba.gb1 = gb1; ba.gW2 = gW2; ba.g6d = g6d; ba.gt = gt;
    FinalizeAdam &ad = L.ad;
    ad.enabled = 1; ad.W1 = bufs->W1; ad.b1 = bufs->b1; ad.W2 = bufs->W2; ad.p6d = bufs->p6d; ad.pt = bufs->pt;
    ad.m = bufs->adam_m; ad.v = bufs->adam_v; ad.seg_lr = c.seg_lr; ad.trans_lr = c.trans_lr;
    ad.beta1 = c.beta1; ad.beta2 = c.beta2; ad.eps = c.eps; ad.step_ptr = bufs->iter;
    ad.weight_decay = c.weight_decay;
    ad.bias_corr = (const double *)(ws + p.o_bc);
    StepBook &bk = L.bk;
    bk.enabled = 1; bk.frame_loss = (const double *)(ws + p.o_floss); bk.n_frame_part = B * g.ncg;
    bk.flow_part = (const double *)(ws + p.o_fpart); bk.n_flow_part = nfp;
    bk.iter = bufs->iter; bk.tau = bufs->tau; bk.losses = bufs->losses; bk.bias_corr = (double *)(ws + p.o_bc);
    bk.ticket = (unsigned int *)(ws + p.o_ticket);
    bk.ring = c.ring; bk.n_iter = c.n_iter; bk.lambda_flow = c.lambda_flow; bk.fixed_tau = c.fixed_tau;
    bk.end_tau = c.end_tau; bk.start_tau = c.start_tau; bk.beta1 = c.beta1; bk.beta2 = c.beta2;
    L.ws_bwd = ws + p.o_bwd; L.bwd_bytes = p.bwd_bytes;
    return REART_OK;
}

static bool step_batchable(const StepGeom &g) {
    return g.pruned && !g.static_order;
}

template <class A>
static Batched<A> gather(const StepLaunch *L, int K, A StepLaunch::*m) {
    Batched<A> b = {};
    for (int k = 0; k < K; ++k) b.a[k] = L[k].*m;
    return b;
}

static int step_launch(const StepLaunch *L, int K, hipStream_t st, hipEvent_t *ev, bool forward_only) {
    const StepGeom &g = L[0].g;
    if (K > 1 && !step_batchable(g)) return REART_ERR_UNSUPPORTED;
    MARK(0);
    int rc = reart_base_forward_launch(gather(L, K, &StepLaunch::fa).a, K, st, g.long_model);
    if (rc != REART_OK) return rc;
    MARK(1);
    if (forward_only) return REART_OK;
    const bool forked = !g.pruned && !ev && L[0].aux_stream && L[0].ev_fork && L[0].ev_join && g.flow;
    hipStream_t fst = forked ? (hipStream_t)L[0].aux_stream : st;
    if (forked) {
        if (hipEventRecord((hipEvent_t)L[0].ev_fork, st) != hipSuccess) return REART_ERR_LAUNCH;
        if (hipStreamWaitEvent(fst, (hipEvent_t)L[0].ev_fork, 0) != hipSuccess) return REART_ERR_LAUNCH;
    }
    if (g.has_search) {
        Batched<SearchArgs> sa = gather(L, K, &StepLaunch::sa);
        const int auto_s = K >= 3 ? 1 : (K == 2 ? 2 : 3);
        for (int k = 0; k < K; ++k) {
            if (L[k].auto_s1) sa.a[k].S1 = auto_s;
            if (L[k].auto_s3) sa.a[k].S3 = L[k].auto_s1 ? auto_s : sa.a[k].S1;
        }
        rc = K == 1 ? reart_search_launch(sa.a[0], st) : reart_search_launch_batch(sa.a, K, st);
        if (rc != REART_OK) return rc;
    } else if (!g.pruned && g.flow) {
        rc = g.grid ? reart_grid_query_launch(L[0].gq3, 3, fst) : reart_knn_launch_slices(L[0].k3, 3, fst);
        if (rc != REART_OK) return rc;
    }
    MARK(2);
    if (g.has_fl) {
        const dim3 fg(g.fgx, g.fgy, K);
        const Batched<FlowArgs> fb = gather(L, K, &StepLaunch::fl);
        if (K > 1) hipLaunchKernelGGL((flow_blend_kernel<1, true>), fg, dim3(FLOW_BS), 0, fst, fb);
        else if (g.fl_sl == 1) hipLaunchKernelGGL((flow_blend_kernel<1, false>), fg, dim3(FLOW_BS), 0, fst, fb);
        else if (g.fl_sl) hipLaunchKernelGGL((flow_blend_kernel<4, false>), fg, dim3(FLOW_BS), 0, fst, fb);
        else hipLaunchKernelGGL((flow_blend_kernel<0, false>), fg, dim3(FLOW_BS), 0, fst, fb);
        REART_CHECK_LAUNCH();
    }
    if (forked && hipEventRecord((hipEvent_t)L[0].ev_join, fst) != hipSuccess) return REART_ERR_LAUNCH;
    MARK(3);
    if (g.has_aa) {
        MARK(4);
        const dim3 ag(reart_div_up(g.N, CG_BS), g.B, K);
        const Batched<AssignArgs> ab = gather(L, K, &StepLaunch::aa);
        if (K > 1) hipLaunchKernelGGL(assign_grad_kernel<true>, ag, dim3(CG_BS), 0, st, ab);
        else hipLaunchKernelGGL(assign_grad_kernel<false>, ag, dim3(CG_BS), 0, st, ab);
    } else {
        if (!g.pruned) {
            if (g.grid) {
                rc = reart_grid_query_launch(L[0].gq1, 1, st);
                if (rc != REART_OK) return rc;
            }
            rc = reart_knn_launch_slices(L[0].ka, 1, st);
            if (rc != REART_OK) return rc;
        }
        MARK(4);
        if (g.merged) {
            const Batched<PostArgs> pb = gather(L, K, &StepLaunch::pa);
            if (K > 1) hipLaunchKernelGGL((post_kernel<true>), dim3(g.post_blocks, K), dim3(CG_BS), 0, st, pb);
            else hipLaunchKernelGGL((post_kernel<false>), dim3(g.post_blocks), dim3(CG_BS), 0, st, pb);
        } else {
            const dim3 cgd(g.ncg, g.B, K);
            const Batched<CGradArgs> cb = gather(L, K, &StepLaunch::cg);
            if (K > 1) hipLaunchKernelGGL((chamfer_grad_kernel<1, true>), cgd, dim3(CG_BS), 0, st, cb);
            else if (g.cg_sl == 1) hipLaunchKernelGGL((chamfer_grad_kernel<1, false>), cgd, dim3(CG_BS), 0, st, cb);
            else if (g.cg_sl) hipLaunchKernelGGL((chamfer_grad_kernel<4, false>), cgd, dim3(CG_BS), 0, st, cb);
            else hipLaunchKernelGGL((chamfer_grad_kernel<0, false>), cgd, dim3(CG_BS), 0, st, cb);
        }
    }
    REART_CHECK_LAUNCH();
    MARK(5);
    if (forked && hipStreamWaitEvent(st, (hipEvent_t)L[0].ev_join, 0) != hipSuccess) return REART_ERR_LAUNCH;
    const Batched<BaseBwdArgs> ba = gather(L, K, &StepLaunch::ba);
    const Batched<FinalizeAdam> ad = gather(L, K, &StepLaunch::ad);
    const Batched<StepBook> bk = gather(L, K, &StepLaunch::bk);
    const Batched<void *> wb = gather(L, K, &StepLaunch::ws_bwd);
    rc = reart_base_backward_launch(ba.a, ad.a, bk.a, wb.a, L[0].bwd_bytes, K, st, g.long_model);
    if (rc != REART_OK) return rc;
    MARK(6);
    MARK(7);
    MARK(8);
    return REART_OK;
}

static int relax_step_one(const reart_relax_config *cfg, const reart_relax_buffers *bufs, void *workspace, size_t workspace_bytes,
                          void *stream, hipEvent_t *ev, bool forward_only) {
    StepLaunch L;
    const int rc = step_describe(cfg, bufs, workspace, workspace_bytes, forward_only, &L);
    return rc != REART_OK ? rc : step_launch(&L, 1, (hipStream_t)stream, ev, forward_only);
}

extern "C" int reart_relax_step(const reart_relax_config *cfg, const reart_relax_buffers *bufs,
                                void *workspace, size_t workspace_bytes, void *stream) {
    return relax_step_one(cfg, bufs, workspace, workspace_bytes, stream, nullptr, false);
}

extern "C" int reart_relax_step_batch(const reart_relax_config *cfgs, const reart_relax_buffers *bufs, void *const *workspaces,
                                      size_t workspace_bytes, int K, void *stream) {
    if (!cfgs || !bufs || !workspaces || K < 1 || K > REART_BATCH_MAX) return REART_ERR_INVALID_ARG;
    static_assert(sizeof(Batched<SearchArgs>) <= 3584, "kernel-argument segment");
    StepLaunch L[REART_BATCH_MAX];
    for (int k = 0; k < K; ++k) {
        const int rc = step_describe(&cfgs[k], &bufs[k], workspaces[k], workspace_bytes, false, &L[k]);
        if (rc != REART_OK) return rc;
        if (!step_batchable(L[k].g)) return REART_ERR_UNSUPPORTED;
        if (memcmp(&L[k].g, &L[0].g, sizeof(StepGeom)) != 0 || L[k].bwd_bytes != L[0].bwd_bytes) return REART_ERR_INVALID_ARG;
    }
    return step_launch(L, K, (hipStream_t)stream, nullptr, false);
}

extern "C" int reart_relax_step_timed(const reart_relax_config *cfg, const reart_relax_buffers *bufs,
                                      void *workspace, size_t workspace_bytes, void *stream,
                                      float *h_ms) {
    if (!h_ms) return REART_ERR_INVALID_ARG;
    hipEvent_t ev[REART_RELAX_PHASES + 1];
    for (int k = 0; k <= REART_RELAX_PHASES; ++k)
        if (hipEventCreate(&ev[k]) != hipSuccess) return REART_ERR_LAUNCH;
    int rc = relax_step_one(cfg, bufs, workspace, workspace_bytes, stream, ev, false);
    if (rc == REART_OK) {
        if (hipEventSynchronize(ev[REART_RELAX_PHASES]) != hipSuccess) rc = REART_ERR_LAUNCH;
        for (int k = 0; k < REART_RELAX_PHASES && rc == REART_OK; ++k) {
            float ms = 0.f;
            if (hipEventElapsedTime(&ms, ev[k], ev[k + 1]) != hipSuccess) rc = REART_ERR_LAUNCH;
            h_ms[k] += ms;
        }
    }
    for (int k = 0; k <= REART_RELAX_PHASES; ++k) (void)hipEventDestroy(ev[k]);
    return rc;
}

extern "C" int reart_relax_profile(const reart_relax_config *cfg, void *workspace, size_t workspace_bytes,
                                   void *stream, double *h_out, int reset) {
    StepPlan p;
    if (!cfg || !h_out) return REART_ERR_INVALID_ARG;
    int rc = step_plan(cfg, &p);
    if (rc != REART_OK) return rc;
    if (!workspace || workspace_bytes < p.total) return REART_ERR_INVALID_ARG;
// ... 51 lines not shown
```

reart_amd/relax.py:

```python
import ctypes
import os

import torch

from . import _lib

c_int, c_float, c_void_p = ctypes.c_int, ctypes.c_float, ctypes.c_void_p


class RelaxConfig(ctypes.Structure):
    _fields_ = [(n, c_int) for n in ("N", "P", "B", "H", "cano_idx", "use_flow", "robust", "euclidean", "flow_k",
                                     "M_max", "M_total", "n_iter", "ring")] + \
               [(n, c_float) for n in ("lambda_flow", "smooth_weight", "trans_lr", "seg_lr", "beta1", "beta2", "eps",
                                       "start_tau", "end_tau", "fixed_tau")] + [("seed", ctypes.c_uint64),
                                                                                 ("use_grid", c_int), ("use_boxes", c_int),
                                                                                 ("use_assign", c_int), ("lambda_assign", c_float),
                                                                                 ("weight_decay", c_float)] + \
               [(n, c_int) for n in ("search_mode", "tune_slices", "tune_slices_flow", "tune_sparse", "tune_fwd_pts",
                                     "tune_bwd_pts", "tune_reorder", "tune_cloud", "tune_xcd", "profile", "tune_share",
                                     "tune_long")]


def tuning_from_env(env=None):
    env = os.environ if env is None else env
    geti = lambda k: int(env[k]) if env.get(k, "") != "" else None
    t = {}
    if env.get("REART_SEARCH") == "brute":
        t["search_mode"] = 1
    for key, field in (("REART_PRUNE_SPLIT", "tune_slices"), ("REART_PRUNE_SPLIT3", "tune_slices_flow"),
                       ("REART_FWD_PTS", "tune_fwd_pts"), ("REART_BWD_PTS", "tune_bwd_pts")):
        if geti(key) is not None:
            t[field] = geti(key)
    if geti("REART_SPARSE") is not None:
        t["tune_sparse"] = -1 if geti("REART_SPARSE") <= 0 else geti("REART_SPARSE")
    if env.get("REART_REORDER") == "0":
        t["tune_reorder"] = -1
    if geti("REART_CLOUD") is not None:
        t["tune_cloud"] = max(0, geti("REART_CLOUD"))
    if env.get("REART_XCD") == "1":
        t["tune_xcd"] = 1
    if env.get("REART_LONG") == "1":
        t["tune_long"] = 1
    if env.get("REART_SHARE") in ("0", "1"):
        t["tune_share"] = -1 if env["REART_SHARE"] == "0" else 1
    return t


class RelaxBuffers(ctypes.Structure):
    _fields_ = [(n, c_void_p) for n in ("cano", "pc_list", "ref_loc", "ref_flow", "ref_off", "gumbel", "W1", "b1", "W2",
                                        "p6d", "pt", "adam_m", "adam_v", "iter", "tau", "losses", "pc_trans",
                                        "seg_part", "trans_list", "aux_stream", "ev_fork", "ev_join", "assign_map")]


def morton_order(points):
    p = points.detach().float()
    lo, hi = p.min(dim=0).values, p.max(dim=0).values
    q = ((p - lo) / (hi - lo).clamp_min(1e-20).max() * 1023.0).clamp(0, 1023).long()

    def spread(v):
        v = (v | (v << 16)) & 0x030000FF
        v = (v | (v << 8)) & 0x0300F00F
        v = (v | (v << 4)) & 0x030C30C3
        v = (v | (v << 2)) & 0x09249249
        return v

    code = spread(q[:, 0]) | (spread(q[:, 1]) << 1) | (spread(q[:, 2]) << 2)
    return torch.sort(code, stable=True).indices


def kd_order(points, leaf=16):
    import numpy as np

    p = points.detach().float().cpu().numpy()
    out, stack = [], [np.arange(p.shape[0])]
    while stack:
        ids = stack.pop()
        if ids.shape[0] <= leaf:
            out.append(ids)
            continue
        pts = p[ids]
        ax = int(np.argmax(pts.max(0) - pts.min(0)))
        o = ids[np.argsort(pts[:, ax], kind="stable")]
        half = (o.shape[0] // 2 + leaf - 1) // leaf * leaf
        stack.append(o[half:])
        stack.append(o[:half])
    return torch.from_numpy(np.concatenate(out)).to(points.device)


_L = None


def _lib_fns():
    global _L
    if _L is None:
        L = _lib.lib()
        L.reart_relax_workspace_bytes.restype = ctypes.c_size_t
        L.reart_relax_workspace_bytes.argtypes = [ctypes.POINTER(RelaxConfig)]
        for fn in (L.reart_relax_prepare, L.reart_relax_step, L.reart_relax_forward):
            fn.restype = c_int
            fn.argtypes = [ctypes.POINTER(RelaxConfig), ctypes.POINTER(RelaxBuffers), c_void_p, ctypes.c_size_t, c_void_p]
        L.reart_relax_step_timed.restype = c_int
        L.reart_relax_step_timed.argtypes = [ctypes.POINTER(RelaxConfig), ctypes.POINTER(RelaxBuffers), c_void_p,
                                             ctypes.c_size_t, c_void_p, ctypes.POINTER(c_float)]
        L.reart_relax_step_batch.restype = c_int
        L.reart_relax_step_batch.argtypes = [ctypes.POINTER(RelaxConfig), ctypes.POINTER(RelaxBuffers), ctypes.POINTER(c_void_p),
                                             ctypes.c_size_t, c_int, c_void_p]
        L.reart_relax_profile.restype = c_int
        L.reart_relax_profile.argtypes = [ctypes.POINTER(RelaxConfig), c_void_p, ctypes.c_size_t, c_void_p,
                                          ctypes.POINTER(ctypes.c_double), c_int]
        _L = L
    return _L


def gumbel_noise(seed, iteration, N, P, device):
    out = torch.empty((N, P), dtype=torch.float32, device=device)
    with torch.cuda.device(device):
        rc = _lib.lib().reart_gumbel_noise(int(seed), int(iteration), N, P, _lib.ptr(out), _lib.stream())
    _lib.check(rc, "reart_gumbel_noise")
    return out


class RelaxEngine:

    def __init__(self, cano_pc, pc_list, model, cano_idx, pc_ref_list=None, flow_ref_list=None, n_iter=15000,
                 start_tau=5.0, end_tau=1.0, trans_lr=1e-2, seg_lr=1e-3, lambda_flow=1.0, use_robust_loss=False,
                 smooth_weight=1e-2, fixed_tau=0.0, seed=2, ring=1024, knn_squared=False, start_iter=0, use_grid=False,
                 overlap_flow=True, spatial_sort=True, weight_decay=0.0, profile=False, tuning=None):
        _lib.require_gpu(cano_pc, pc_list)
        dev = cano_pc.device
        self.device, self.model = dev, model
        cano_pc, pc_list = cano_pc.float(), pc_list.float()
        order = {"kd": kd_order, "morton": morton_order}[os.environ.get("REART_ORDER", "kd")]
        self._perm = order(cano_pc) if spatial_sort else None
        self._perm_frames = None
        if spatial_sort:
            cano_pc = cano_pc[self._perm]
            self._perm_frames = torch.stack([order(f) for f in pc_list])
            pc_list = torch.stack([f[o] for f, o in zip(pc_list, self._perm_frames)])
            if pc_ref_list is not None:
                orders = [order(r.reshape(-1, 3)) for r in pc_ref_list]
                pc_ref_list = [r.reshape(-1, 3)[o] for r, o in zip(pc_ref_list, orders)]
                flow_ref_list = [f.reshape(-1, 3)[o] for f, o in zip(flow_ref_list, orders)]
            self._inv = torch.empty_like(self._perm)
            self._inv[self._perm] = torch.arange(self._perm.numel(), device=dev)
        self.cano = cano_pc.contiguous()
        self.pc_list = pc_list.contiguous()
        B, N, _ = self.pc_list.shape
        if B > _lib.MAX_POSE_LEN:
            raise NotImplementedError(f"a sequence of {B + 1} frames: the relaxation step takes at most "
                                      f"REART_MAX_POSE_LEN = {_lib.MAX_POSE_LEN} frames beside the canonical one")
        c1, c2 = model.seg_head.model[0], model.seg_head.model[2]
        H, P = c1.weight.shape[0], c2.weight.shape[0]
        self.params = [c1.weight, c1.bias, c2.weight, model.proposal_6d, model.proposal_t]
        for p in self.params:
            assert p.is_cuda and p.is_contiguous() and p.dtype == torch.float32
        nparams = sum(p.numel() for p in self.params)
        self.adam_m = torch.zeros(nparams, device=dev)
        self.adam_v = torch.zeros(nparams, device=dev)
        self.iter = torch.full((1,), int(start_iter), dtype=torch.int64, device=dev)
        self.tau = torch.zeros(1, device=dev)
        self.ring = ring
        self.losses = torch.zeros((ring, 4), device=dev)
        self._pc_trans = torch.empty((B, N, 3), device=dev)
        self._assign_map = torch.full((B, N), -1, dtype=torch.int32, device=dev)
        self._seg_part = torch.empty((N,), dtype=torch.int64, device=dev)
        self.trans_list = torch.empty((B, P, 4, 4), device=dev)
        self.gumbel = None
        use_flow = pc_ref_list is not None
        if use_flow:
            assert len(pc_ref_list) == B and len(flow_ref_list) == B
            lens = [int(r.shape[0]) for r in pc_ref_list]
            self.ref_loc = torch.cat([r.reshape(-1, 3) for r in pc_ref_list]).contiguous().float().to(dev)
            self.ref_flow = torch.cat([r.reshape(-1, 3) for r in flow_ref_list]).contiguous().float().to(dev)
            off = [0]
            for m in lens:
                off.append(off[-1] + m)
            self.ref_off = torch.tensor(off, dtype=torch.int32, device=dev)
        else:
            lens, self.ref_loc, self.ref_flow, self.ref_off = [0], None, None, None
        self.cfg = RelaxConfig(N=N, P=P, B=B, H=H, cano_idx=cano_idx, use_flow=int(use_flow),
                               robust=int(bool(use_robust_loss)), euclidean=0 if knn_squared else 1, flow_k=3,
                               M_max=max(lens), M_total=sum(lens), n_iter=n_iter, ring=ring, lambda_flow=lambda_flow,
                               smooth_weight=smooth_weight, trans_lr=trans_lr, seg_lr=seg_lr, beta1=0.9, beta2=0.999,
                               eps=1e-8, start_tau=start_tau, end_tau=end_tau, fixed_tau=fixed_tau, seed=seed,
                               use_grid=int(bool(use_grid)), use_boxes=int(bool(spatial_sort)),
                               weight_decay=float(weight_decay), profile=int(bool(profile)))
        for k, v in (tuning_from_env() if tuning is None else tuning).items():
            setattr(self.cfg, k, int(v))
        L = _lib_fns()
        nbytes = L.reart_relax_workspace_bytes(ctypes.byref(self.cfg))
        if nbytes == 0:
            raise _lib.ReartHipError("reart_relax_workspace_bytes: unsupported configuration")
        self.workspace = torch.empty(nbytes, dtype=torch.uint8, device=dev)
        self._graph = None
        self._bufs = None
        self.graph_replays = self.eager_steps = 0
        self._aux = None
        if use_flow and overlap_flow:
            self._aux = torch.cuda.Stream(device=dev)
            self._ev = (torch.cuda.Event(), torch.cuda.Event())
            for ev in self._ev:
                ev.record()
        self._refresh_buffers()
        rc = L.reart_relax_prepare(ctypes.byref(self.cfg), ctypes.byref(self._bufs), _lib.ptr(self.workspace),
                                   self.workspace.numel(), _lib.stream())
        _lib.check(rc, "reart_relax_prepare")

    def _refresh_buffers(self):
        p = _lib.ptr
        v = lambda t: None if t is None else t.data_ptr()
        W1, b1, W2, p6d, pt = self.params
        self._bufs = RelaxBuffers(cano=v(self.cano), pc_list=v(self.pc_list), ref_loc=v(self.ref_loc),
                                  ref_flow=v(self.ref_flow), ref_off=v(self.ref_off), gumbel=v(self.gumbel),
                                  W1=v(W1), b1=v(b1), W2=v(W2), p6d=v(p6d), pt=v(pt), adam_m=v(self.adam_m),
                                  adam_v=v(self.adam_v), iter=v(self.iter), tau=v(self.tau), losses=v(self.losses),
                                  pc_trans=v(self._pc_trans), seg_part=v(self._seg_part), trans_list=v(self.trans_list),
                                  aux_stream=None if self._aux is None else self._aux.cuda_stream,
                                  ev_fork=None if self._aux is None else self._ev[0].cuda_event,
                                  ev_join=None if self._aux is None else self._ev[1].cuda_event,
                                  assign_map=v(self._assign_map))

    @property
    def pc_trans(self):
        return self._pc_trans if self._perm is None else self._pc_trans[:, self._inv]

    @property
    def seg_part(self):
        return self._seg_part if self._perm is None else self._seg_part[self._inv]

    def caller_clouds(self):
        if self._perm is None:
            return self.cano, self.pc_list
        B, N = self._perm_frames.shape
        inv_f = torch.empty_like(self._perm_frames)
        inv_f.scatter_(1, self._perm_frames, torch.arange(N, device=self.device).expand(B, N))
        return self.cano[self._inv], torch.gather(self.pc_list, 1, inv_f[..., None].expand(-1, -1, 3))

    def set_gumbel(self, noise):
        assert self._graph is None, "noise injection is an eager-mode (test) feature"
        if noise is not None and self._perm is not None:
            noise = noise[self._perm]
        self.gumbel = None if noise is None else noise.contiguous().float()
        self._refresh_buffers()

    def peek_forward(self):
        rc = _lib_fns().reart_relax_forward(ctypes.byref(self.cfg), ctypes.byref(self._bufs), _lib.ptr(self.workspace),
                                            self.workspace.numel(), _lib.stream())
        _lib.check(rc, "reart_relax_forward")

    def set_assignment(self, src_idx, tgt_idx, lambda_assign):
        B, N = self._assign_map.shape
        src = src_idx.to(self.device).long().reshape(-1)
        tgt = tgt_idx.to(self.device).long().reshape(B, -1)
        if self._perm is not None:
            src = self._inv[src]
            if getattr(self, "_inv_frames", None) is None:
                inv_f = torch.empty_like(self._perm_frames)
                inv_f.scatter_(1, self._perm_frames, torch.arange(N, device=self.device).expand(B, N))
                self._inv_frames = inv_f
            tgt = self._inv_frames.gather(1, tgt)
        self._assign_map.fill_(-1)
        self._assign_map[:, src] = tgt.to(torch.int32)
        lam32 = ctypes.c_float(lambda_assign).value
        if not self.cfg.use_assign or self.cfg.lambda_assign != lam32:
            self.cfg.use_assign, self.cfg.lambda_assign = 1, float(lambda_assign)
            self._graph = None

    def clear_assignment(self):
        if self.cfg.use_assign:
            self.cfg.use_assign = 0
            self._graph = None

    def _enqueue(self):
        rc = _lib_fns().reart_relax_step(ctypes.byref(self.cfg), ctypes.byref(self._bufs), _lib.ptr(self.workspace),
                                         self.workspace.numel(), _lib.stream())
        _lib.check(rc, "reart_relax_step")

    def capture(self, steps_per_graph=1):
        self._enqueue()
        torch.cuda.synchronize()
        g = torch.cuda.CUDAGraph()
        with torch.cuda.graph(g, capture_error_mode="thread_local"):
            for _ in range(steps_per_graph):
                self._enqueue()
        self._graph, self._steps_per_graph = g, steps_per_graph
        return 1

    def step(self, n=1):
        if self._graph is not None:
            for _ in range(n // self._steps_per_graph):
                self._graph.replay()
            self.graph_replays += n // self._steps_per_graph
            n %= self._steps_per_graph
        for _ in range(n):
            self._enqueue()
        self.eager_steps += n

    PHASES = ("forward", "flow_knn3", "flow_blend", "chamfer_nn", "chamfer_grad", "backward", "adam", "bookkeep")

    def step_timed(self, n=1):
        acc = (c_float * len(self.PHASES))()
        for _ in range(n):
            rc = _lib_fns().reart_relax_step_timed(ctypes.byref(self.cfg), ctypes.byref(self._bufs),
                                                   _lib.ptr(self.workspace), self.workspace.numel(), _lib.stream(), acc)
            _lib.check(rc, "reart_relax_step_timed")
        return {k: acc[i] / n for i, k in enumerate(self.PHASES)}

    def search_profile(self, reset=False):
        out = (ctypes.c_double * 5)()
        rc = _lib_fns().reart_relax_profile(ctypes.byref(self.cfg), _lib.ptr(self.workspace), self.workspace.numel(),
                                            _lib.stream(), out, int(bool(reset)))
        _lib.check(rc, "reart_relax_profile")
        return {"launches": int(out[0]), "seconds": float(out[1]), "pairs": int(out[2]), "clock_hz": float(out[3]),
                "workgroup_seconds": float(out[4])}

    def loss_log(self):
        it = int(self.iter.item())
        rows = self.losses[: min(it, self.ring)] if it <= self.ring else torch.roll(self.losses, -(it % self.ring), 0)
        return it, rows.clone()

    def last_losses(self):
        it = int(self.iter.item())
        return self.losses[(it - 1) % self.ring].clone()


class RelaxBatch:

    MAX = 6

    def __init__(self, engines):
        engines = list(engines)
        if not 1 <= len(engines) <= self.MAX:
            raise ValueError(f"RelaxBatch takes 1..{self.MAX} engines")
        nb = {e.workspace.numel() for e in engines}
        if len(nb) != 1:
            raise ValueError("RelaxBatch: the engines must share one shape")
        for f in self.SAME:
            vals = {getattr(e.cfg, f) for e in engines}
            if len(vals) != 1:
                raise ValueError(f"RelaxBatch: the engines differ in cfg.{f} ({sorted(vals)})")
        if len({e.device for e in engines}) != 1:
            raise ValueError("RelaxBatch: the engines live on different devices")
        self.engines = engines
        self._nbytes = nb.pop()
        self._graph = None
        self.graph_replays = self.eager_steps = 0
        self._refresh()

    SAME = ("N", "P", "B", "H", "M_max", "use_flow", "robust", "euclidean", "flow_k", "use_grid", "use_boxes", "use_assign",
            "search_mode", "tune_slices", "tune_slices_flow", "tune_sparse", "tune_fwd_pts", "tune_bwd_pts", "tune_reorder",
            "tune_cloud", "tune_xcd", "tune_share", "tune_long")

    def _refresh(self):
        K = len(self.engines)
        self._cfgs = (RelaxConfig * K)(*[e.cfg for e in self.engines])
        self._bufs = (RelaxBuffers * K)(*[e._bufs for e in self.engines])
        self._ws = (c_void_p * K)(*[e.workspace.data_ptr() for e in self.engines])

    def _enqueue(self):
        if len({(e.cfg.use_assign, e.cfg.use_flow) for e in self.engines}) != 1:
            raise RuntimeError("RelaxBatch: the engines must be in the same loss mode (all Chamfer or all assignment loss)")
        self._refresh()
        rc = _lib_fns().reart_relax_step_batch(self._cfgs, self._bufs, self._ws, self._nbytes, len(self.engines), _lib.stream())
        _lib.check(rc, "reart_relax_step_batch")

    def capture(self, steps_per_graph=1):
        self._enqueue()
        torch.cuda.synchronize()
        g = torch.cuda.CUDAGraph()
        with torch.cuda.graph(g, capture_error_mode="thread_local"):
            for _ in range(steps_per_graph):
                self._enqueue()
        self._graph, self._steps_per_graph = g, steps_per_graph
        self._graph_mode = self._mode()
        return 1

    def _mode(self):
        return tuple((e.cfg.use_assign, e.cfg.use_flow, e.cfg.lambda_assign) for e in self.engines)

    def step(self, n=1):
        if self._graph is not None and self._graph_mode != self._mode():
            self._graph = None
        if self._graph is not None:
            for _ in range(n // self._steps_per_graph):
                self._graph.replay()
            self.graph_replays += n // self._steps_per_graph
            n %= self._steps_per_graph
        for _ in range(n):
            self._enqueue()
        self.eager_steps += n
```

reart_amd/run_robot.py:

```python
#!/usr/bin/env python3
import argparse
import contextlib
import ctypes
import functools
import glob
import os
import pickle
import random

import numpy as np
import torch

from reart_amd.knn_cuda import KNN
from reart_amd.networks.loss import flow_loss, recon_loss
from reart_amd.networks.model import BaseModel, KinematicModel
from reart_amd.networks.pointnet2_utils import farthest_point_sample, index_points
from reart_amd.relax import RelaxEngine
from reart_amd.utils.chamfer import ChamferDistance, ChamferLoss
from reart_amd.utils.flow_utils import FlowTerm, blend_anchor_motion, blend_anchor_motion_batch, pad_reference_sets
from reart_amd.utils.model_utils import tau_cosine


def load_sequence(seq_path, num_points, cano_idx):
    from reart_amd.dataset import Sequence
# ... 510 lines not shown
        return m

    def _metrics(self, seg_part, trans_list):
        from reart_amd import tail

        c = self.args.cano_idx
        if not self.graph or self.count < 2:
            return tail.snapshot_metrics(self.cano_pc, self.pc_list, seg_part, trans_list, c, self.sample, chamfer=False)
        if self._g is None:
            try:
                self._g_in = (seg_part.clone(), trans_list.clone())
                g = torch.cuda.CUDAGraph()
                torch.cuda.synchronize()
                with torch.cuda.graph(g):
                    self._g_names, self._g_out = tail.snapshot_values(self.cano_pc, self._g_in[0], self._g_in[1], c, self.sample)
                self._g = g
            except Exception:
                self.graph, self._g = False, None
                torch.cuda.synchronize()
                return tail.snapshot_metrics(self.cano_pc, self.pc_list, seg_part, trans_list, c, self.sample, chamfer=False)
        if seg_part.shape != self._g_in[0].shape or trans_list.shape != self._g_in[1].shape:
            return tail.snapshot_metrics(self.cano_pc, self.pc_list, seg_part, trans_list, c, self.sample, chamfer=False)
        self._g_in[0].copy_(seg_part)
        self._g_in[1].copy_(trans_list)
        self._g.replay()
        return tail.snapshot_scaled(self._g_names, self._g_out.cpu().tolist()) if self._g_out is not None else {}


def build_kinematic_from_base(result, cano_pc, pc_list, args):
    from reart_amd import tail

    device = cano_pc.device
    seg_part = torch.from_numpy(np.asarray(result["pred_cano_part"])).long().to(device)
    trans_list = torch.from_numpy(np.asarray(result["pred_pose_list"])).float().to(device)
    if "joint_connection" in result:
        joint_connection = torch.from_numpy(np.array(result["joint_connection"])).long().to(device)
    else:
        seg_part, trans_list, joint_connection = tail.extract_structure(
            seg_part, trans_list, cano_pc, merge_thr=args.merge_thr, cano_dist_thr=args.cano_dist_thr,
            lambda_joint=args.lambda_joint, min_num=0)
    new_seg, kin_kwargs = tail.kinematic_init(seg_part, trans_list, joint_connection)
    return KinematicModel(pose_len=pc_list.shape[0], seg_part=new_seg, cano_pc=cano_pc,
                          knn=KNN(k=1, transpose_mode=True), **kin_kwargs)


def project_from_base(args, sample, result, device, save_dir, dataset=None):
    torch.cuda.manual_seed_all(args.manual_seed)
    torch.manual_seed(args.manual_seed)
    np.random.seed(args.manual_seed)
    random.seed(args.manual_seed)
    from reart_amd.utils import lap as _lap

    _lap.CANONICAL_TIES = bool(getattr(args, "deterministic", True))
    assert args.cano_idx == result["cano_idx"]
    cano_pc = torch.from_numpy(sample["cano_pc"]).float().to(device)
    pc_list = torch.from_numpy(sample["pc_list"]).float().to(device)
    os.makedirs(save_dir, exist_ok=True)
    pc_ref_list = flow_ref_list = None
    if args.use_flow_loss:
        pc_ref_list, flow_ref_list = flow_references(args, sample, device, args.seq_path)
    tau_func = functools.partial(tau_cosine, max_iter=args.n_iter, end_temp=args.end_tau, start_temp=args.start_tau)
    model = build_kinematic_from_base(result, cano_pc, pc_list, args)
    model.to(device)
    snapshot = SnapshotPrinter(args, model, cano_pc, pc_list, None if args.synthetic and "gt_flow_list" not in sample else sample, tau_func)
    n_iter = args.n_iter
    loop = make_projection_loop(args, model, cano_pc, pc_list, pc_ref_list, flow_ref_list, tau_func)
    i = 0
    while i < n_iter:
        losses = loop.iteration(i)
        if i % args.snapshot_gap == 0 or i == n_iter - 1:
            snapshot(i, losses)
        i += 1
    lap_report = None
    if args.use_assign_loss:
        lap_report = {"assign_refreshes": loop.lap_solves, "lap_fallbacks": loop.lap_fallbacks}
    out = finish(args, model, cano_pc, pc_list, sample, save_dir, tau_func(cur_iter=n_iter), dataset, lap_report)
    out.update(lap_report or {"assign_refreshes": 0, "lap_fallbacks": 0}, iterations=i, model=model)
    return out


def main(args):
    torch.cuda.manual_seed_all(args.manual_seed)
    torch.manual_seed(args.manual_seed)
    np.random.seed(args.manual_seed)
    random.seed(args.manual_seed)
    if not torch.cuda.is_available():
        raise SystemExit("reart_amd runs on an AMD GPU only (no CPU fallback)")
    from reart_amd.utils import lap as _lap

    _lap.CANONICAL_TIES = bool(getattr(args, "deterministic", True))
    if args.evaluate and args.resume is None:
        raise ValueError("need model path to evaluate!")
    device = torch.device("cuda")
    dataset = None
    if args.synthetic:
        sample = synthetic_sequence(args.num_points, args.cano_idx, args.synthetic_frames, args.use_flow_loss)
    else:
        from reart_amd.dataset import Sequence

        dataset = Sequence(args.seq_path, num_points=args.num_points, cano_idx=args.cano_idx)
        sample = dataset[0]
    cano_pc = torch.from_numpy(sample["cano_pc"]).float().to(device)
    pc_list = torch.from_numpy(sample["pc_list"]).float().to(device)
    save_dir = os.path.join(args.save_root, "synthetic" if args.synthetic
                            else (os.path.basename(args.seq_path.rstrip("/")) or "sequence"))
    os.makedirs(save_dir, exist_ok=True)

    if args.model == "kinematic" and args.resume is None:
        assert args.base_result_path is not None, "--model kinematic needs --base_result_path or --resume"
        with open(args.base_result_path, "rb") as f:
            result = pickle.load(f)
        print(f"load base result from {args.base_result_path}")
        model = project_from_base(args, sample, result, device, save_dir, dataset)["model"]
        print("all done!")
        return model

    pc_ref_list = flow_ref_list = None
    if args.use_flow_loss:
        pc_ref_list, flow_ref_list = flow_references(args, sample, device, args.seq_path)

    tau_func = functools.partial(tau_cosine, max_iter=args.n_iter, end_temp=args.end_tau, start_temp=args.start_tau)
    fixed_tau = 0.0
    if args.model == "base":
        model = BaseModel(num_parts=args.num_parts, pose_len=pc_list.shape[0])
        if args.resume is not None:
            ckpt = torch.load(args.resume[0], map_location=device, weights_only=False)
            model.load_state_dict(ckpt["state_dict"], strict=False)
            fixed_tau = float(ckpt["tau"])
            tau_func = lambda cur_iter: fixed_tau
            assert args.cano_idx == ckpt.get("cano_idx", args.cano_idx)
    else:
        ckpt = torch.load(args.resume[0], map_location=device, weights_only=False)
        model = KinematicModel(pose_len=pc_list.shape[0], seg_part=ckpt["seg_part"].to(device),
                               cano_pc=ckpt["cano_pc"].to(device), knn=KNN(k=1, transpose_mode=True),
                               edge_index=ckpt["edge_index"], paths_to_base=ckpt["paths_to_base"],
                               reverse_topo=ckpt["reverse_topo"])
        model.load_state_dict(ckpt["state_dict"], strict=True)
    model.to(device)
    chamfer_dist = ChamferDistance()
    knn_flow = KNN(k=3, transpose_mode=True)

    snapshot = SnapshotPrinter(args, model, cano_pc, pc_list, None if args.synthetic and "gt_flow_list" not in sample else sample, tau_func)

    n_iter = 1 if args.evaluate else args.n_iter
    i = 0
    lap_report = None
    fused_until = n_iter if not args.use_assign_loss else min(args.assign_iter, n_iter)
    if args.model == "base" and not args.evaluate:
        eng = RelaxEngine(cano_pc, pc_list, model, args.cano_idx, pc_ref_list, flow_ref_list, n_iter=args.n_iter,
                          start_tau=args.start_tau, end_tau=args.end_tau, trans_lr=args.trans_lr, seg_lr=args.seg_lr,
                          lambda_flow=args.lambda_flow, use_robust_loss=args.use_robust_loss, fixed_tau=fixed_tau,
                          seed=args.manual_seed, weight_decay=args.weight_decay)
        if fused_until > 0:
            i += eng.capture()
        while i < fused_until:
            chunk = min(args.snapshot_gap, fused_until - i)
            eng.step(chunk)
            i += chunk
            row = eng.last_losses().cpu().numpy()
            snapshot(i - 1, {"recon Loss": row[0], "flow Loss": row[1], "total Loss": row[2]})
        if i < n_iter and args.use_assign_loss:
            phase = AssignmentPhase(eng, cano_pc, pc_list, args.downsample, args.assign_gap, args.lambda_assign)

            def on_snapshot(k):
                row = eng.last_losses().cpu().numpy()
                snapshot(k - 1, {"opt assignment loss": row[0], "flow Loss": row[1], "total Loss": row[2]})

            i = phase.run(i, n_iter, args.snapshot_gap, on_snapshot)
            lap_report = phase.report()
            print(f"assignment phase: {lap_report['assign_refreshes']} refreshes, {lap_report['lap_fallbacks']} host fallbacks")
    if i < n_iter and not args.evaluate:
        loop = make_projection_loop(args, model, cano_pc, pc_list, pc_ref_list, flow_ref_list, tau_func)
        while i < n_iter:
            losses = loop.iteration(i)
            if i % args.snapshot_gap == 0 or i == n_iter - 1:
                snapshot(i, losses)
            i += 1
        if args.use_assign_loss:
            lap_report = {"assign_refreshes": loop.lap_solves, "lap_fallbacks": loop.lap_fallbacks}
    if args.evaluate:
        snapshot(0, {})
    finish(args, model, cano_pc, pc_list, sample, save_dir, tau_func(cur_iter=n_iter), dataset, lap_report)
    print("all done!")
    return model


def finish(args, model, cano_pc, pc_list, sample, save_dir, tau, dataset=None, lap_report=None):
    from reart_amd import tail
    from reart_amd.utils.kinematic_utils import edge_index2edges
    from reart_amd.utils.model_utils import compute_pc_transform

    device = cano_pc.device
    with torch.no_grad():
        _, seg_part, trans_list = model(cano_pc)
    trans_list = trans_list.detach()
    if isinstance(model, KinematicModel):
        from reart_amd.utils.graph_utils import denoise_seg_label

        seg_part = denoise_seg_label(seg_part.clone(), cano_pc, KNN(k=1, transpose_mode=True), min_num=20)
        conn = torch.tensor(edge_index2edges(model.edge_index), dtype=torch.long, device=device)
        from reart_amd.utils.kinematic_utils import extract_kinematic

        seg_part, trans_list, conn = extract_kinematic(seg_part, trans_list, conn)
    else:
        seg_part, trans_list, conn = tail.extract_structure(
            seg_part, trans_list, cano_pc, merge_thr=args.merge_thr, merge_it=args.merge_it,
            cano_dist_thr=args.cano_dist_thr, lambda_joint=args.lambda_joint)
    conn_list = conn.cpu().numpy().tolist()
    print("parts:", trans_list.shape[1], "| joint connection:", conn_list)
    metrics = tail.snapshot_metrics(cano_pc, pc_list, seg_part, trans_list, args.cano_idx, sample)
    if "epe" in metrics:
        print(f"Flow eval: EPE: {metrics['epe']:.3f} | Acc 5: {metrics['acc5']:.3f} | Acc 10: {metrics['acc10']:.3f} | "
              f"Angle: {metrics['angle']:.3f}")
    if "ri" in metrics:
        print(f"Seg eval: RI: {metrics['ri']:.3f}")
    if "recon_err" in metrics:
        print(f"Recon eval: recon: {metrics['recon_err']:.3f}")
    report = {"parts": int(trans_list.shape[1]), "joint_connection": conn_list,
              "cd_err": float(metrics["cd_err"]) if "cd_err" in metrics else None}
    retarget_err = 9999
    if isinstance(model, KinematicModel) and dataset is not None and len(dataset.novel_pose_list):
        from reart_amd.utils.kinematic_utils import ik

        retarget_err = ik(dataset, model, device, verbose=False, vis=False, fused=bool(getattr(args, "fused_ik", False)))
    print("Retarget error: {:.3f}".format(retarget_err))
    with open(os.path.join(save_dir, "result.txt"), "w") as f_result:
        f_result.write(f"retarget_err: {retarget_err:.3f}\n")
        for k in ("recon_err", "epe", "acc5", "acc10", "angle", "ri", "cd_err"):
            if k in metrics:
                f_result.write(f"{k}: {metrics[k]:.3f}\n")
        if not args.evaluate:
            energy = tail.energy_terms(cano_pc, pc_list, seg_part, trans_list, conn, args.cano_idx)
            report.update({k: float(energy[k]) for k in ("ass_err", "screw_err", "group_err", "total_err")})
            print(f"Energy eval: total: {energy['total_err']:.3f}")
            for k in ("ass_err", "screw_err", "group_err", "total_err"):
                print(f"{k}: {energy[k]:.3f}")
                f_result.write(f"{k}: {energy[k]:.3f}\n")
            print(f"cd_err: {metrics['cd_err']:.3f}")
        if lap_report is not None:
            for k in ("assign_refreshes", "lap_fallbacks"):
                f_result.write(f"{k}: {lap_report[k]}\n")
    if args.evaluate:
        return report
    save_dict = {"pred_cano_part": seg_part.cpu().numpy(), "pred_pose_list": trans_list.cpu().numpy(),
                 "cano_idx": args.cano_idx, "joint_connection": conn_list}
    save_dict.update(sample)
    with open(os.path.join(save_dir, "result.pkl"), "wb") as f:
        pickle.dump(save_dict, f)
    model_dict = {"state_dict": model.state_dict(), "tau": tau, "cano_idx": args.cano_idx}
    if isinstance(model, KinematicModel):
        model_dict.update(seg_part=model.seg_part, cano_pc=model.cano_pc, edge_index=model.edge_index,
                          paths_to_base=model.paths_to_base, reverse_topo=model.reverse_topo)
    torch.save(model_dict, os.path.join(save_dir, "model.pth.tar"))
    print("saved", os.path.join(save_dir, "result.pkl"), "and", os.path.join(save_dir, "model.pth.tar"))
    return report


def build_parser():
    p = argparse.ArgumentParser(description="Robot (reart_amd)")
    p.add_argument("--manual_seed", default=2, type=int)
    p.add_argument("--resume", type=str, nargs="+", metavar="PATH")
    p.add_argument("--evaluate", dest="evaluate", action="store_true")
    p.add_argument("--snapshot_gap", default=100, type=int)
    p.add_argument("--use_cuda", default=1, type=int)
    p.add_argument("--cano_idx", default=0, type=int)
    p.add_argument("--num_points", default=4096, type=int)
    p.add_argument("--seq_path", default="data/robot/nao", type=str)
    p.add_argument("--normalize_file", default="data/category_normalize_scale.pkl", type=str)
    p.add_argument("--start_tau", default=5, type=float)
    p.add_argument("--end_tau", default=1, type=float)
    p.add_argument("--seg_lr", default=1e-3, type=float)
    p.add_argument("--trans_lr", default=1e-2, type=float)
    p.add_argument("--weight_decay", default=0, type=float)
    p.add_argument("--n_iter", default=15000, type=int)
    p.add_argument("--assign_iter", default=5000, type=int)
    p.add_argument("--num_parts", default=20, type=int)
    p.add_argument("--model", default="base", type=str, choices=["base", "kinematic"])
    p.add_argument("--base_result_path", default=None, type=str)
    p.add_argument("--corr_model_path", default="pretrained/corr_model.pth.tar")
    p.add_argument("--use_flow_loss", action="store_true")
    p.add_argument("--use_robust_loss", action="store_true")
    p.add_argument("--use_assign_loss", action="store_true")
    p.add_argument("--use_nproc", action="store_true")
    p.add_argument("--downsample", default=4, type=int)
    p.add_argument("--assign_gap", default=5, type=int)
    p.add_argument("--lambda_assign", default=3e-1, type=float)
    p.add_argument("--lambda_flow", default=1, type=float)
    p.add_argument("--lambda_joint", default=100, type=float)
    p.add_argument("--cano_dist_thr", default=1e-2, type=float)
    p.add_argument("--merge_thr", default=3e-2, type=float)
    p.add_argument("--merge_it", default=2, type=int)
    p.add_argument("--save_root", default="exp", type=str)
    p.add_argument("--synthetic", action="store_true", help="generated articulated sequence instead of --seq_path")
    p.add_argument("--synthetic_frames", default=20, type=int)
    p.add_argument("--deterministic", dest="deterministic", action="store_true", default=True,
                   help="(default) the assignment refreshes return a function of the cost matrix alone, like the reference's scipy "
                        "call (run_robot.py:172-176): when several assignments are optimal the raced GPU solvers return whichever "
                        "finished first, so every solve is checked for ties (reart_lap_ties) and a tied problem takes the "
                        "lexicographically smallest optimum -- two runs under one --manual_seed are the same run (run_robot.py:37-49)")
    p.add_argument("--no_deterministic", dest="deterministic", action="store_false",
                   help="skip the tie check (about 2 %% of a projection iteration): tied optima are settled by whichever racer wins")
    p.add_argument("--fused_ik", action="store_true",
                   help="retarget error of a kinematic model: fit all novel poses in one launch (kinematic_utils.ik_batch) instead of "
                        "one Adam loop per pose; same optimum, not bit-equal to the default")
    p.add_argument("--fused_losses", action="store_true",
                   help="operator loop (the base model outside the fused engine): the Chamfer term as one warm-started call with a "
                        "fused backward, the T-1 flow blends as one call; same losses up to the summation order of the Chamfer sum")
# ... 12 lines not shown
```

Baseline: 13320 iterations/s.

## Publish pose/weight shared-memory image from Adam finalize to skip forward rebuild

The backward finalize kernel now writes the updated parameters directly into a precomputed shared-memory image (rotation-translation table plus transposed W1/b1/W2) in the workspace, and tags it with the next iteration number. The forward kernel checks the tag and, when it is fresh, bulk-copies the image into LDS instead of recomputing 6D-to-matrix conversions and transposing weights in every block. Block 0 also writes trans_list from the image. Python invalidates the tag on capture, eager steps and peeks, and run_robot captures multi-step graphs. The price is extra global writes in finalize, an ordering dependency on the ticket, and more register use in the forward kernel for the vector preload.

```diff
diff --git a/include/reart_hip.h b/include/reart_hip.h
--- a/include/reart_hip.h
+++ b/include/reart_hip.h
@@ -150,6 +150,7 @@
     int tune_xcd;
     int profile;
     int tune_share;
+    int tune_fwd_images;
     int tune_long;
 } reart_relax_config;
 
@@ -176,6 +177,7 @@
 size_t reart_relax_workspace_bytes(const reart_relax_config *cfg);
 int reart_relax_prepare(const reart_relax_config *cfg, const reart_relax_buffers *bufs,
                         void *workspace, size_t workspace_bytes, void *stream);
+int reart_relax_images_invalidate(void *workspace, size_t workspace_bytes, void *stream);
 int reart_relax_forward(const reart_relax_config *cfg, const reart_relax_buffers *bufs,
                         void *workspace, size_t workspace_bytes, void *stream);
 int reart_relax_step(const reart_relax_config *cfg, const reart_relax_buffers *bufs,
diff --git a/reart_amd/_lib.py b/reart_amd/_lib.py
--- a/reart_amd/_lib.py
+++ b/reart_amd/_lib.py
@@ -121,6 +121,7 @@
     "reart_group_temporal_err": (c_int, [P, c_int, c_int, P, P, c_int, P, P, P]),
     "reart_relax_workspace_bytes": (c_size_t, None),
     "reart_relax_prepare": (c_int, None),
+    "reart_relax_images_invalidate": (c_int, [P, c_size_t, P]),
     "reart_relax_step": (c_int, None),
     "reart_relax_step_batch": (c_int, None),
     "reart_relax_forward": (c_int, None),
diff --git a/reart_amd/csrc/internal.h b/reart_amd/csrc/internal.h
--- a/reart_amd/csrc/internal.h
+++ b/reart_amd/csrc/internal.h
@@ -20,6 +20,8 @@
     float *rt_table;
     float *boxes;
     int pts;
+    const float *img;
+    const int64_t *img_tag;
 };
 
 struct BaseBwdArgs {
@@ -61,6 +63,7 @@
     float weight_decay;
     const int64_t *step_ptr;
     const double *bias_corr;
+    float *img;
 };
 
 struct StepBook {
@@ -69,6 +72,7 @@
     const double *flow_part; int n_flow_part;
     int64_t *iter; float *tau; float *losses; double *bias_corr;
     unsigned int *ticket;
+    int64_t *img_tag;
     int ring, n_iter;
     float lambda_flow, fixed_tau, end_tau, start_tau, beta1, beta2;
 };
diff --git a/reart_amd/csrc/model.hip b/reart_amd/csrc/model.hip
--- a/reart_amd/csrc/model.hip
+++ b/reart_amd/csrc/model.hip
@@ -44,6 +44,33 @@
     PHASE_TS(0, 0);
     const int P = (PP > 0) ? PP : a.P;
     const int nRT = a.B * a.P;
+    const int n = blockIdx.x * PTS + pl;
+    const bool live = n < a.N;
+    const int nc = live ? n : a.N - 1;
+    const int nimg = 12 * nRT + a.H * (4 + PMAX);
+    const bool img_vec = (a.H & 3) == 0;
+    constexpr int UI = (((19 * 12 + 128) * PMAX + 4 * 128) / 4 + BS - 1) / BS;
+    typedef float img4 __attribute__((ext_vector_type(4)));
+    img4 vi[UI];
+    if (a.img && img_vec) {
+#pragma unroll
+        for (int u = 0; u < UI; ++u)
+            if (tid + u * BS < (nimg >> 2)) vi[u] = ((const img4 *)a.img)[tid + u * BS];
+    }
+    const uint64_t it = a.iter_ptr ? (uint64_t)a.iter_ptr[0] : 0ull;
+    const bool fresh = a.img && a.iter_ptr && (uint64_t)a.img_tag[0] == it;
+    const float x0 = a.cano[3 * (size_t)nc], x1 = a.cano[3 * (size_t)nc + 1], x2 = a.cano[3 * (size_t)nc + 2];
+    const float tau = a.tau_ptr ? a.tau_ptr[0] : a.tau;
+    if (fresh) {
+        if (img_vec) {
+#pragma unroll
+            for (int u = 0; u < UI; ++u)
+                if (tid + u * BS < (nimg >> 2)) ((img4 *)smem)[tid + u * BS] = vi[u];
+            for (int e = tid + UI * BS; e < (nimg >> 2); e += BS) ((img4 *)smem)[e] = ((const img4 *)a.img)[e];
+        } else {
+            for (int e = tid; e < nimg; e += BS) smem[e] = a.img[e];
+        }
+    } else {
     auto put_rt = [&](int e, const float (&d6)[6], const float (&tv)[3]) {
         float R[9];
         r6d_to_matrix(d6, R);
@@ -103,20 +130,15 @@
     }
     for (int j = tid + BS; j < a.H; j += BS)
         for (int p = 0; p < PMAX; ++p) s_w2T[((p >> 1) * a.H + j) * 2 + (p & 1)] = p < P ? a.W2[(size_t)p * a.H + j] : 0.f;
-
-    const int n = blockIdx.x * PTS + pl;
-    const bool live = n < a.N;
-    const int nc = live ? n : a.N - 1;
-    const float x0 = a.cano[3 * (size_t)nc], x1 = a.cano[3 * (size_t)nc + 1], x2 = a.cano[3 * (size_t)nc + 2];
+    }
+
     const int p0 = sid * FW_PG;
     const bool has1 = p0 + 1 < P;
-    const float tau = a.tau_ptr ? a.tau_ptr[0] : a.tau;
     float g0, g1 = 0.f;
     if (a.gumbel) {
         g0 = a.gumbel[(size_t)nc * P + (p0 < P ? p0 : 0)];
         if (has1) g1 = a.gumbel[(size_t)nc * P + p0 + 1];
     } else {
-        const uint64_t it = a.iter_ptr ? (uint64_t)a.iter_ptr[0] : 0ull;
         uint32_t r[4];
         philox4x32((uint32_t)n, (uint32_t)(p0 >> 2), (uint32_t)it, (uint32_t)(it >> 32), (uint32_t)a.seed,
                    (uint32_t)(a.seed >> 32), r);
@@ -232,6 +254,19 @@
                 float *o = a.boxes + ((size_t)t * (a.Npad / NN_BOX) + pos / NN_BOX) * 8;
                 o[0] = lo[0]; o[1] = lo[1]; o[2] = lo[2]; o[3] = hi[0]; o[4] = hi[1]; o[5] = hi[2];
             }
+        }
+    }
+    if (fresh && blockIdx.x == 0 && a.trans_list) {
+        for (int e = tid; e < nRT; e += BS) {
+            const float *Rt = s_rt + 12 * e;
+            float *T = a.trans_list + 16 * (size_t)e;
+#pragma unroll
+            for (int r = 0; r < 3; ++r) {
+#pragma unroll
+                for (int c = 0; c < 3; ++c) T[4 * r + c] = Rt[3 * r + c];
+                T[4 * r + 3] = Rt[9 + r];
+            }
+            T[12] = 0.f; T[13] = 0.f; T[14] = 0.f; T[15] = 1.f;
         }
     }
     PHASE_TS(0, 5);
@@ -714,7 +749,7 @@
     r.p = *p; r.m = *m; r.v = *v;
     return r;
 }
-__device__ __forceinline__ void adam_update(float *p, float g, float *m, float *v, const AdamLoaded &ld, float lr,
+__device__ __forceinline__ float adam_update(float *p, float g, float *m, float *v, const AdamLoaded &ld, float lr,
                                             float step_size_base, float bc2s, float beta1, float beta2,
                                             float eps, float weight_decay = 0.f) {
     (void)lr;
@@ -724,24 +759,50 @@
     vv = vv * beta2 + ((1.0f - beta2) * g) * g;
     const float denom = sqrtf(vv) / bc2s + eps;
     *m = mm; *v = vv;
-    *p = ld.p - step_size_base * (mm / denom);
-}
-
-__device__ __forceinline__ void base_bwd_finalize_body(const BaseBwdArgs &a, const FinalizeAdam &ad) {
+    const float pn = ld.p - step_size_base * (mm / denom);
+    *p = pn;
+    return pn;
+}
+
+struct PosePub { float pn; int e, c, on; };
+
+__device__ __forceinline__ void finalize_publish_pose(const FinalizeAdam &ad, const PosePub &pb) {
+    if (!pb.on) return;
+    const int lane0 = (threadIdx.x & 63) & ~15;
+    float nv[9], R[9];
+#pragma unroll
+    for (int u = 0; u < 9; ++u) nv[u] = __shfl(pb.pn, lane0 + u, 64);
+    r6d_to_matrix(nv, R);
+    float val = R[0];
+#pragma unroll
+    for (int u = 1; u < 9; ++u) val = (pb.c == u) ? R[u] : val;
+#pragma unroll
+    for (int u = 0; u < 3; ++u) val = (pb.c == 9 + u) ? nv[6 + u] : val;
+    ad.img[12 * (size_t)pb.e + pb.c] = val;
+}
+
+__device__ __forceinline__ PosePub base_bwd_finalize_body(const BaseBwdArgs &a, const FinalizeAdam &ad) {
+    PosePub pub = {0.f, 0, 0, 0};
     const int og = blockIdx.x * 256 + threadIdx.x;
     const int nWr = a.P * a.H + 4 * a.H;
     const int nW = (4 * nWr + 63) & ~63;
     const int RQ = (a.nchunk + 3) >> 2;
     const int o = og >> 2;
     const int no = n_out(a.P, a.H, a.B);
+    float *const img = ad.enabled ? ad.img : nullptr;
     double bc1 = 1.0, bc2 = 1.0;
     if (ad.enabled) { bc1 = ad.bias_corr[0]; bc2 = ad.bias_corr[1]; }
     if (og < nW) {
-        if (o >= nWr) return;
+        if (o >= nWr) return pub;
         const int nW2 = a.P * a.H, nW1 = 3 * a.H;
         const int kind = o < nW2 ? 0 : (o < nW2 + nW1 ? 1 : 2);
         const int q = kind == 0 ? o : (kind == 1 ? o - nW2 : o - nW2 - nW1);
         const int mo = kind == 0 ? nW1 + a.H + q : (kind == 1 ? q : nW1 + q);
+        int io = 12 * a.B * a.P;
+        if (kind == 0) {
+            const int p = (unsigned)q / (unsigned)a.H, j = q - p * a.H;
+            io += 4 * a.H + ((p >> 1) * a.H + j) * 2 + (p & 1);
+        } else io += kind == 1 ? 4 * (q / 3) + q % 3 : 4 * q + 3;
         AdamLoaded ld = {0.f, 0.f, 0.f};
         if (ad.enabled) {
             if (kind == 0) ld.p = ad.W2[q];
@@ -769,17 +830,26 @@
         for (; c < cend; ++c) acc += a.partial[(size_t)c * no + o];
         acc = acc + __shfl_xor(acc, 1, 64);
         acc = acc + __shfl_xor(acc, 2, 64);
-        if (og & 3) return;
+        if (og & 3) return pub;
         const float ss_seg = (float)((double)ad.seg_lr / bc1), bc2s = (float)bc2;
         if (kind == 0) {
             a.gW2[q] = acc;
-            if (ad.enabled) adam_update(ad.W2 + q, acc, ad.m + mo, ad.v + mo, ld, ad.seg_lr, ss_seg, bc2s, ad.beta1, ad.beta2, ad.eps, ad.weight_decay);
+            if (ad.enabled) {
+                const float pn = adam_update(ad.W2 + q, acc, ad.m + mo, ad.v + mo, ld, ad.seg_lr, ss_seg, bc2s, ad.beta1, ad.beta2, ad.eps, ad.weight_decay);
+                if (img) img[io] = pn;
+            }
         } else if (kind == 1) {
             a.gW1[q] = acc;
-            if (ad.enabled) adam_update(ad.W1 + q, acc, ad.m + mo, ad.v + mo, ld, ad.seg_lr, ss_seg, bc2s, ad.beta1, ad.beta2, ad.eps, ad.weight_decay);
+            if (ad.enabled) {
+                const float pn = adam_update(ad.W1 + q, acc, ad.m + mo, ad.v + mo, ld, ad.seg_lr, ss_seg, bc2s, ad.beta1, ad.beta2, ad.eps, ad.weight_decay);
+                if (img) img[io] = pn;
+            }
         } else {
             a.gb1[q] = acc;
-            if (ad.enabled) adam_update(ad.b1 + q, acc, ad.m + mo, ad.v + mo, ld, ad.seg_lr, ss_seg, bc2s, ad.beta1, ad.beta2, ad.eps, ad.weight_decay);
+            if (ad.enabled) {
+                const float pn = adam_update(ad.b1 + q, acc, ad.m + mo, ad.v + mo, ld, ad.seg_lr, ss_seg, bc2s, ad.beta1, ad.beta2, ad.eps, ad.weight_decay);
+                if (img) img[io] = pn;
+            }
         }
     } else if (og < nW + 64 * a.B * a.P) {
         const int q = og - nW, e = q >> 6, tq = (q >> 4) & 3, c = q & 15;
@@ -812,22 +882,26 @@
         const int lane0 = (threadIdx.x & 63) & ~15;
 #pragma unroll
         for (int u = 0; u < 12; ++u) gRt[u] = __shfl(acc, lane0 + u, 64);
-        if (c >= 9 || tq != 0) return;
-        float g6[6];
-        r6d_backward(d6, gRt, g6);
-        const float ss_tr = (float)((double)ad.trans_lr / bc1), bc2s = (float)bc2;
-        float g;
-        if (c < 6) {
-            g = g6[0];
-#pragma unroll
-            for (int u = 1; u < 6; ++u) g = (c == u) ? g6[u] : g;
-            a.g6d[6 * (size_t)e + c] = g;
-        } else {
-            g = k == 0 ? gRt[9] : (k == 1 ? gRt[10] : gRt[11]);
-            a.gt[3 * (size_t)e + k] = g;
-        }
-        if (ad.enabled) adam_update(pp, g, ad.m + mo, ad.v + mo, ld, ad.trans_lr, ss_tr, bc2s, ad.beta1, ad.beta2, ad.eps, ad.weight_decay);
-    }
+        if (tq != 0 || c >= (img ? 12 : 9)) return pub;
+        pub.e = e; pub.c = c; pub.on = img != nullptr;
+        if (c < 9) {
+            float g6[6];
+            r6d_backward(d6, gRt, g6);
+            const float ss_tr = (float)((double)ad.trans_lr / bc1), bc2s = (float)bc2;
+            float g;
+            if (c < 6) {
+                g = g6[0];
+#pragma unroll
+                for (int u = 1; u < 6; ++u) g = (c == u) ? g6[u] : g;
+                a.g6d[6 * (size_t)e + c] = g;
+            } else {
+                g = k == 0 ? gRt[9] : (k == 1 ? gRt[10] : gRt[11]);
+                a.gt[3 * (size_t)e + k] = g;
+            }
+            if (ad.enabled) pub.pn = adam_update(pp, g, ad.m + mo, ad.v + mo, ld, ad.trans_lr, ss_tr, bc2s, ad.beta1, ad.beta2, ad.eps, ad.weight_decay);
+        }
+    }
+    return pub;
 }
 
 template <bool BATCH>
@@ -840,6 +914,7 @@
     __shared__ float s_tau;
     __shared__ long s_it;
     const int tid = threadIdx.x;
+    PosePub pub = {0.f, 0, 0, 0};
 #ifdef REART_PHASE_CLOCK
     if (blockIdx.x == 1 && blockIdx.y == 0 && threadIdx.x == 0) { g_phase_ts[0][14] = __builtin_amdgcn_s_memtime(); g_phase_ts[0][8] = g_phase_ts[0][14]; }
 #endif
@@ -861,13 +936,16 @@
         recon = reart_wave_sum_d(recon);
         flow = reart_wave_sum_d(flow);
         if (l == 0) { s_book[0] = recon; s_book[1] = flow * (double)bk.lambda_flow; }
-    } else base_bwd_finalize_body(a, ad);
+    } else pub = base_bwd_finalize_body(a, ad);
 #ifdef REART_PHASE_CLOCK
     if (blockIdx.x == 1 && blockIdx.y == 0 && threadIdx.x == 0) g_phase_ts[0][9] = __builtin_amdgcn_s_memtime();
 #endif
-    if (!bk.enabled) return;
+    if (!bk.enabled) { finalize_publish_pose(ad, pub); return; }
     __syncthreads();
-    if (tid == 0) s_last = (atomicAdd(bk.ticket, 1u) == gridDim.x - 1) ? 1 : 0;
+    unsigned int turn = 0u;
+    if (tid == 0) turn = atomicAdd(bk.ticket, 1u);
+    finalize_publish_pose(ad, pub);
+    if (tid == 0) s_last = (turn == gridDim.x - 1) ? 1 : 0;
     __syncthreads();
 #ifdef REART_PHASE_CLOCK
     if (blockIdx.x == 1 && blockIdx.y == 0 && threadIdx.x == 0) g_phase_ts[0][10] = __builtin_amdgcn_s_memtime();
@@ -882,6 +960,7 @@
     bk.bias_corr[0] = s_book[2];
     bk.bias_corr[1] = s_book[3];
     bk.tau[0] = s_tau;
+    if (bk.img_tag) bk.img_tag[0] = it + 1;
     *bk.ticket = 0u;
 }
 
diff --git a/reart_amd/csrc/step.hip b/reart_amd/csrc/step.hip
--- a/reart_amd/csrc/step.hip
+++ b/reart_amd/csrc/step.hip
@@ -10,6 +10,7 @@
     int nchunk, nparams;
     size_t o_ysoa, o_xsoa, o_rsoa, o_rlen, o_qmap;
     size_t o_pd0, o_pi0, o_pd1, o_pi1, o_pd3, o_pi3;
+    size_t o_imgtag;
     size_t o_yT, o_hT, o_hard, o_rt, o_G, o_gpf, o_fx, o_floss, o_fpart, o_grads, o_bwd;
     size_t o_bc;
     size_t o_ticket;
@@ -59,6 +60,7 @@
     p->nparams = 3 * c->H + c->H + c->P * c->H + 6 * c->B * c->P + 3 * c->B * c->P;
     size_t off = 0;
     const size_t BN = (size_t)c->B * c->N;
+    p->o_imgtag = take(off, sizeof(int64_t));
     p->o_ysoa = take(off, sizeof(float) * 3 * c->B * (size_t)p->Npad);
     p->o_xsoa = take(off, sizeof(float) * 3 * c->B * (size_t)p->Npad);
     p->o_rsoa = take(off, sizeof(float) * 3 * c->B * (size_t)p->Mpad);
@@ -73,7 +75,7 @@
     p->o_yT = take(off, sizeof(float) * (size_t)c->P * c->N);
     p->o_hT = take(off, sizeof(float) * (size_t)c->H * c->N);
     p->o_hard = take(off, sizeof(int) * (size_t)c->N);
-    p->o_rt = take(off, sizeof(float) * 12 * (size_t)c->B * c->P);
+    p->o_rt = take(off, sizeof(float) * (12 * (size_t)c->B * c->P + (size_t)c->H * (4 + 32)));
     p->o_G = take(off, sizeof(float) * 3 * BN);
     p->o_gpf = take(off, sizeof(float) * 3 * BN);
     p->o_fx = take(off, sizeof(double));
@@ -163,6 +165,12 @@
     d[j] = x; d[Mpad + j] = y; d[2 * (size_t)Mpad + j] = z;
 }
 
+extern "C" int reart_relax_images_invalidate(void *workspace, size_t workspace_bytes, void *stream) {
+    if (!workspace || workspace_bytes < sizeof(int64_t)) return REART_ERR_INVALID_ARG;
+    if (hipMemsetAsync(workspace, 0xff, sizeof(int64_t), (hipStream_t)stream) != hipSuccess) return REART_ERR_LAUNCH;
+    return REART_OK;
+}
+
 extern "C" int reart_relax_prepare(const reart_relax_config *cfg, const reart_relax_buffers *bufs,
                                    void *workspace, size_t workspace_bytes, void *stream) {
     StepPlan p;
@@ -188,6 +196,9 @@
                        (int *)(ws + p.o_fx), (double *)(ws + p.o_bc),
                        (p.pruned && cfg->use_flow) ? (int *)(ws + p.o_seed3) : nullptr, (int *)(ws + p.o_border));
     if (hipMemsetAsync(ws + p.o_ticket, 0, 4 * sizeof(unsigned int), st) != hipSuccess) return REART_ERR_LAUNCH;
+    if (hipMemsetAsync(ws + p.o_rt, 0, sizeof(float) * (12 * (size_t)cfg->B * cfg->P + (size_t)cfg->H * (4 + 32)), st) != hipSuccess) return REART_ERR_LAUNCH;
+    rc = reart_relax_images_invalidate(workspace, workspace_bytes, stream);
+    if (rc != REART_OK) return rc;
     if (hipMemsetAsync(ws + p.o_prof_acc, 0, 4 * sizeof(unsigned long long), st) != hipSuccess) return REART_ERR_LAUNCH;
     if (p.pruned) {
         if (hipMemsetAsync(ws + p.o_pi0, 0, sizeof(int) * (size_t)cfg->B * cfg->N, st) != hipSuccess) return REART_ERR_LAUNCH;
@@ -684,6 +695,8 @@
     fa.rt_table = (float *)(ws + p.o_rt);
     fa.boxes = c.use_boxes ? (float *)(ws + p.o_boxX) : nullptr;
     fa.pts = c.tune_fwd_pts;
+    const bool images = c.tune_fwd_images >= 0 && c.tune_long <= 0 && reart_base_path(P, B, H, 0) == 0;
+    if (images) { fa.img = fa.rt_table; fa.img_tag = (const int64_t *)(ws + p.o_imgtag); }
     if (forward_only) return REART_OK;
     if (c.use_assign && !bufs->assign_map) return REART_ERR_INVALID_ARG;
 
@@ -827,11 +840,13 @@
     ad.beta1 = c.beta1; ad.beta2 = c.beta2; ad.eps = c.eps; ad.step_ptr = bufs->iter;
     ad.weight_decay = c.weight_decay;
     ad.bias_corr = (const double *)(ws + p.o_bc);
+    ad.img = images ? fa.rt_table : nullptr;
     StepBook &bk = L.bk;
     bk.enabled = 1; bk.frame_loss = (const double *)(ws + p.o_floss); bk.n_frame_part = B * g.ncg;
     bk.flow_part = (const double *)(ws + p.o_fpart); bk.n_flow_part = nfp;
     bk.iter = bufs->iter; bk.tau = bufs->tau; bk.losses = bufs->losses; bk.bias_corr = (double *)(ws + p.o_bc);
     bk.ticket = (unsigned int *)(ws + p.o_ticket);
+    bk.img_tag = images ? (int64_t *)(ws + p.o_imgtag) : nullptr;
     bk.ring = c.ring; bk.n_iter = c.n_iter; bk.lambda_flow = c.lambda_flow; bk.fixed_tau = c.fixed_tau;
     bk.end_tau = c.end_tau; bk.start_tau = c.start_tau; bk.beta1 = c.beta1; bk.beta2 = c.beta2;
     L.ws_bwd = ws + p.o_bwd; L.bwd_bytes = p.bwd_bytes;
diff --git a/reart_amd/relax.py b/reart_amd/relax.py
--- a/reart_amd/relax.py
+++ b/reart_amd/relax.py
@@ -18,7 +18,7 @@
                                                                                  ("weight_decay", c_float)] + \
                [(n, c_int) for n in ("search_mode", "tune_slices", "tune_slices_flow", "tune_sparse", "tune_fwd_pts",
                                      "tune_bwd_pts", "tune_reorder", "tune_cloud", "tune_xcd", "profile", "tune_share",
-                                     "tune_long")]
+                                     "tune_fwd_images", "tune_long")]
 
 
 def tuning_from_env(env=None):
@@ -41,6 +41,8 @@
         t["tune_xcd"] = 1
     if env.get("REART_LONG") == "1":
         t["tune_long"] = 1
+    if env.get("REART_FWD_IMAGES") == "0":
+        t["tune_fwd_images"] = -1
     if env.get("REART_SHARE") in ("0", "1"):
         t["tune_share"] = -1 if env["REART_SHARE"] == "0" else 1
     return t
@@ -236,6 +238,10 @@
         inv_f.scatter_(1, self._perm_frames, torch.arange(N, device=self.device).expand(B, N))
         return self.cano[self._inv], torch.gather(self.pc_list, 1, inv_f[..., None].expand(-1, -1, 3))
 
+    def _invalidate_images(self):
+        rc = _lib.lib().reart_relax_images_invalidate(_lib.ptr(self.workspace), self.workspace.numel(), _lib.stream())
+        _lib.check(rc, "reart_relax_images_invalidate")
+
     def set_gumbel(self, noise):
         assert self._graph is None, "noise injection is an eager-mode (test) feature"
         if noise is not None and self._perm is not None:
@@ -244,6 +250,7 @@
         self._refresh_buffers()
 
     def peek_forward(self):
+        self._invalidate_images()
         rc = _lib_fns().reart_relax_forward(ctypes.byref(self.cfg), ctypes.byref(self._bufs), _lib.ptr(self.workspace),
                                             self.workspace.numel(), _lib.stream())
         _lib.check(rc, "reart_relax_forward")
@@ -277,10 +284,12 @@
         _lib.check(rc, "reart_relax_step")
 
     def capture(self, steps_per_graph=1):
+        self._invalidate_images()
         self._enqueue()
         torch.cuda.synchronize()
         g = torch.cuda.CUDAGraph()
         with torch.cuda.graph(g, capture_error_mode="thread_local"):
+            self._invalidate_images()
             for _ in range(steps_per_graph):
                 self._enqueue()
         self._graph, self._steps_per_graph = g, steps_per_graph
@@ -292,6 +301,8 @@
                 self._graph.replay()
             self.graph_replays += n // self._steps_per_graph
             n %= self._steps_per_graph
+        if n > 0:
+            self._invalidate_images()
         for _ in range(n):
             self._enqueue()
         self.eager_steps += n
@@ -300,6 +311,7 @@
 
     def step_timed(self, n=1):
         acc = (c_float * len(self.PHASES))()
+        self._invalidate_images()
         for _ in range(n):
             rc = _lib_fns().reart_relax_step_timed(ctypes.byref(self.cfg), ctypes.byref(self._bufs),
                                                    _lib.ptr(self.workspace), self.workspace.numel(), _lib.stream(), acc)
@@ -349,13 +361,17 @@
 
     SAME = ("N", "P", "B", "H", "M_max", "use_flow", "robust", "euclidean", "flow_k", "use_grid", "use_boxes", "use_assign",
             "search_mode", "tune_slices", "tune_slices_flow", "tune_sparse", "tune_fwd_pts", "tune_bwd_pts", "tune_reorder",
-            "tune_cloud", "tune_xcd", "tune_share", "tune_long")
+            "tune_cloud", "tune_xcd", "tune_share", "tune_fwd_images", "tune_long")
 
     def _refresh(self):
         K = len(self.engines)
         self._cfgs = (RelaxConfig * K)(*[e.cfg for e in self.engines])
         self._bufs = (RelaxBuffers * K)(*[e._bufs for e in self.engines])
         self._ws = (c_void_p * K)(*[e.workspace.data_ptr() for e in self.engines])
+
+    def _invalidate_images(self):
+        for e in self.engines:
+            e._invalidate_images()
 
     def _enqueue(self):
         if len({(e.cfg.use_assign, e.cfg.use_flow) for e in self.engines}) != 1:
@@ -365,10 +381,12 @@
         _lib.check(rc, "reart_relax_step_batch")
 
     def capture(self, steps_per_graph=1):
+        self._invalidate_images()
         self._enqueue()
         torch.cuda.synchronize()
         g = torch.cuda.CUDAGraph()
         with torch.cuda.graph(g, capture_error_mode="thread_local"):
+            self._invalidate_images()
             for _ in range(steps_per_graph):
                 self._enqueue()
         self._graph, self._steps_per_graph = g, steps_per_graph
@@ -386,6 +404,8 @@
                 self._graph.replay()
             self.graph_replays += n // self._steps_per_graph
             n %= self._steps_per_graph
+        if n > 0:
+            self._invalidate_images()
         for _ in range(n):
             self._enqueue()
         self.eager_steps += n
diff --git a/reart_amd/run_robot.py b/reart_amd/run_robot.py
--- a/reart_amd/run_robot.py
+++ b/reart_amd/run_robot.py
@@ -686,7 +686,7 @@
                           lambda_flow=args.lambda_flow, use_robust_loss=args.use_robust_loss, fixed_tau=fixed_tau,
                           seed=args.manual_seed, weight_decay=args.weight_decay)
         if fused_until > 0:
-            i += eng.capture()
+            i += eng.capture(steps_per_graph=max(1, min(50, args.snapshot_gap, fused_until - 1)))
         while i < fused_until:
             chunk = min(args.snapshot_gap, fused_until - i)
             eng.step(chunk)
```

Result: no change. 13380 iterations/s, median of 6 (+0.5%).
